# justinkay/aldi

Hardware: AMD Instinct MI355X
Metric: images/sec (student+teacher ALDI step), R50-FPN 1333x800 (higher is better)
Workload: dtype bf16

## Files before the change

### aldi_amd/csrc/bneck.hip

```cpp
#include "common.h"
#include "tile_prims.h"
#include <stdio.h>

namespace {

constexpr int MID = 64, CO = 256, TH = 8, TW = 16, HC = TW + 2, NHP = (TH + 2) * HC, CR = 192, A1P = 24;
constexpr int kRegA = 0;
constexpr int kRegB = 32768;
constexpr int kRegC = kRegB + (TH + 2) * A1P * 128;
constexpr int kLdsBytes = kRegC + 16384;
constexpr int kStgRow = CO * 2 + 16;
static_assert(TH * TW * kStgRow <= kLdsBytes && kLdsBytes <= 81920, "two workgroups per CU");

struct BneckDev {
    const bf16_t* x; const bf16_t* res; bf16_t* y;
    const bf16_t* w1; const bf16_t* w2; const bf16_t* w3;
    const float* b1; const float* b2; const float* b3;
    int N, H, W, th, tw, xcd;
    unsigned x_bytes, y_bytes;
};

__device__ __forceinline__ void lds_write_b64(unsigned addr, uint2 v) {
    asm volatile("ds_write_b64 %0, %1" ::"v"(addr), "v"(v) : "memory");
}
template <int N, int STEP, int I = 0>
__device__ __forceinline__ void stg_read_all(u32x4_t* f, unsigned addr) {
    if constexpr (I < N) {
        f[I] = frag_read<I * STEP>(addr);
        stg_read_all<N, STEP, I + 1>(f, addr);
    }
}
__device__ __forceinline__ uint2 relu_pack4(f32x4_t a, float4 sh, bool keep) {
    float v0 = fmaxf(a[0] + sh.x, 0.f), v1 = fmaxf(a[1] + sh.y, 0.f), v2 = fmaxf(a[2] + sh.z, 0.f), v3 = fmaxf(a[3] + sh.w, 0.f);
    uint2 t;
    t.x = keep ? pack2_bf16(v0, v1) : 0u;
    t.y = keep ? pack2_bf16(v2, v3) : 0u;
    return t;
}

template <int CX>
__global__ __launch_bounds__(256, 2) void bneck_kernel(BneckDev p) {
    static_assert(CX % 32 == 0, "x slabs of 32 channels");
    __shared__ __attribute__((aligned(128))) uint4 lds[kLdsBytes / 16];
    const int tid = threadIdx.x, lane = tid & 63, wave = __builtin_amdgcn_readfirstlane(tid >> 6);
    const int fr = lane & 15, fq = lane >> 4;
    int bid = blockIdx.x;
    if (p.xcd) {
        const int total = gridDim.x, q = total >> 3, r = total & 7, xcd = bid & 7, idx = bid >> 3;
        bid = (xcd < r ? xcd * (q + 1) : r * (q + 1) + (xcd - r) * q) + idx;
    }
    const int per_img = p.th * p.tw;
    const int n = bid / per_img, rem = bid - n * per_img;
    const int ty = rem / p.tw, tx = rem - ty * p.tw;
    const int h0 = ty * TH, w0 = tx * TW;
    constexpr unsigned OOB = 0x80000000u;
    const __amdgpu_buffer_rsrc_t rx = __builtin_amdgcn_make_buffer_rsrc(const_cast<bf16_t*>(p.x), 0, p.x_bytes, 0x00020000);
    const __amdgpu_buffer_rsrc_t rw1 = __builtin_amdgcn_make_buffer_rsrc(const_cast<bf16_t*>(p.w1), 0, MID * CX * 2, 0x00020000);
    const __amdgpu_buffer_rsrc_t rw2 = __builtin_amdgcn_make_buffer_rsrc(const_cast<bf16_t*>(p.w2), 0, MID * 9 * MID * 2, 0x00020000);
    const __amdgpu_buffer_rsrc_t rw3 = __builtin_amdgcn_make_buffer_rsrc(const_cast<bf16_t*>(p.w3), 0, CO * MID * 2, 0x00020000);
    const int wbase = __builtin_amdgcn_readfirstlane(tid & ~63);
    const unsigned lbase = lds_addr(&lds[0]);
    const long img_pix = (long)n * p.H * p.W;
    float4 sh1[4], sh2[4], sh3[4];
#pragma unroll
    for (int j = 0; j < 4; ++j) {
        sh1[j] = *reinterpret_cast<const float4*>(p.b1 + j * 16 + fq * 4);
        sh2[j] = *reinterpret_cast<const float4*>(p.b2 + j * 16 + fq * 4);
        sh3[j] = *reinterpret_cast<const float4*>(p.b3 + (wave * 4 + j) * 16 + fq * 4);
    }

    unsigned xoff[3];
#pragma unroll
    for (int it = 0; it < 3; ++it) {
        const int cr = (tid >> 2) + it * 64, kce = swz<4>(cr, tid & 3);
        const int hr = cr / HC, hc = cr - hr * HC;
        const int gh = h0 - 1 + hr, gw = w0 - 1 + hc;
        const bool ok = cr < NHP && (unsigned)gh < (unsigned)p.H && (unsigned)gw < (unsigned)p.W;
        xoff[it] = ok ? (unsigned)(((img_pix + (long)gh * p.W + gw) * CX + kce * 8) * 2) : OOB;
    }
    const unsigned w1off = (unsigned)(((tid >> 2) * CX + swz<4>(tid >> 2, tid & 3) * 8) * 2);
    constexpr int kStage1 = CR * 64 + MID * 64;
    auto issue1 = [&](int s) {
        const int st = s & 3;
#pragma unroll
        for (int it = 0; it < 3; ++it) glds16(rx, &lds[st * (kStage1 / 16) + wbase + it * 256], xoff[it] == OOB ? OOB : xoff[it] + (unsigned)(s * 64));
        glds16(rw1, &lds[st * (kStage1 / 16) + CR * 4 + wbase], w1off + (unsigned)(s * 64));
    };
    f32x4_t acc1[3][4];
#pragma unroll
    for (int i = 0; i < 3; ++i)
#pragma unroll
        for (int j = 0; j < 4; ++j) acc1[i][j] = f32x4_t{0.f, 0.f, 0.f, 0.f};
    {
        const int xrow = wave * 48 + fr;
        const unsigned x_rd = lbase + (unsigned)(xrow * 4 + swz<4>(xrow, fq)) * 16u;
        const unsigned w_rd = lbase + CR * 64 + (unsigned)(fr * 4 + swz<4>(fr, fq)) * 16u;
        constexpr int S = CX / 32;
#pragma unroll
        for (int s = 0; s < 3 && s < S; ++s) issue1(s);
#pragma unroll
        for (int s = 0; s < S; ++s) {
            constexpr int kPieces = 4;
            const int younger = (S - 1 - s < 2 ? S - 1 - s : 2) * kPieces;
            if (younger == 8) asm volatile("s_waitcnt vmcnt(8)" ::: "memory");
            else if (younger == 4) asm volatile("s_waitcnt vmcnt(4)" ::: "memory");
            else asm volatile("s_waitcnt vmcnt(0)" ::: "memory");
            __builtin_amdgcn_s_barrier();
            __builtin_amdgcn_sched_barrier(0);
            if (s + 3 < S) issue1(s + 3);
            u32x4_t xf[3], wf[4];
            frag_read_all<3, 64>(xf, x_rd + (unsigned)((s & 3) * kStage1));
            frag_read_all<4, 64>(wf, w_rd + (unsigned)((s & 3) * kStage1));
            frag_wait<3, 4>(xf, wf);
#pragma unroll
            for (int i = 0; i < 3; ++i)
#pragma unroll
                for (int j = 0; j < 4; ++j) acc1[i][j] = Mma<bf16_t>::run(wf[j], xf[i], acc1[i][j]);
        }
    }
    __builtin_amdgcn_s_barrier();
    __builtin_amdgcn_sched_barrier(0);
    unsigned w2off[2];
#pragma unroll
    for (int it = 0; it < 2; ++it) {
        const int c = tid + it * 256, row = c >> 3, q = c & 7;
        w2off[it] = (unsigned)(((row * 9) * MID + (q ^ ((row >> 1) & 7)) * 8) * 2);
    }
    auto issue_tap = [&](int t) {
#pragma unroll
        for (int it = 0; it < 2; ++it) glds16(rw2, &lds[kRegA / 16 + (t & 3) * 512 + wbase + it * 256], w2off[it] + (unsigned)(t * MID * 2));
    };
    issue_tap(0); issue_tap(1); issue_tap(2);
#pragma unroll
    for (int i = 0; i < 3; ++i) {
        const int cr = (wave * 3 + i) * 16 + fr;
        const int hr = cr / HC, hc = cr - hr * HC;
        const int gh = h0 - 1 + hr, gw = w0 - 1 + hc;
        const bool inside = (unsigned)gh < (unsigned)p.H && (unsigned)gw < (unsigned)p.W;
        const int ar = hr * A1P + hc;
        if (cr < NHP) {
#pragma unroll
            for (int j = 0; j < 4; ++j) {
                const int chunk = (j * 2 + (fq >> 1)) ^ ((ar >> 1) & 7);
                lds_write_b64(lbase + kRegB + (unsigned)(ar * 128 + chunk * 16 + (fq & 1) * 8), relu_pack4(acc1[i][j], sh1[j], inside));
            }
        }
    }
    f32x4_t acc2[2][4];
#pragma unroll
    for (int i = 0; i < 2; ++i)
#pragma unroll
        for (int j = 0; j < 4; ++j) acc2[i][j] = f32x4_t{0.f, 0.f, 0.f, 0.f};
    {
        unsigned a1b[2][3][2];
#pragma unroll
        for (int par = 0; par < 2; ++par)
#pragma unroll
            for (int kw = 0; kw < 3; ++kw)
#pragma unroll
                for (int ks = 0; ks < 2; ++ks) {
                    const int row = par * 8 + kw + fr;
                    a1b[par][kw][ks] = lbase + kRegB + (unsigned)(wave * 2 * A1P * 128) + (unsigned)(row * 128 + (((ks * 4 + fq) ^ ((row >> 1) & 7)) << 4));
                }
        unsigned wb[2];
#pragma unroll
        for (int ks = 0; ks < 2; ++ks) wb[ks] = lbase + kRegA + (unsigned)((fr * 8 + ((ks * 4 + fq) ^ ((fr >> 1) & 7))) * 16);
        asm volatile("s_waitcnt lgkmcnt(0)" ::: "memory");
#pragma unroll
        for (int t = 0; t < 9; ++t) {
            const int kh = t / 3, kw = t - kh * 3;
            if (t <= 6) asm volatile("s_waitcnt vmcnt(4)" ::: "memory");
            else if (t == 7) asm volatile("s_waitcnt vmcnt(2)" ::: "memory");
            else asm volatile("s_waitcnt vmcnt(0)" ::: "memory");
            __builtin_amdgcn_s_barrier();
            __builtin_amdgcn_sched_barrier(0);
            if (t + 3 < 9) issue_tap(t + 3);
            u32x4_t af[2][2], wf[2][4];
#pragma unroll
            for (int ks = 0; ks < 2; ++ks) {
                af[ks][0] = kh == 0 ? frag_read<0>(a1b[0][kw][ks]) : kh == 1 ? frag_read<16 * 128>(a1b[1][kw][ks]) : frag_read<48 * 128>(a1b[0][kw][ks]);
                af[ks][1] = kh == 0 ? frag_read<16 * 128>(a1b[1][kw][ks]) : kh == 1 ? frag_read<48 * 128>(a1b[0][kw][ks]) : frag_read<64 * 128>(a1b[1][kw][ks]);
                frag_read_all<4, 128>(wf[ks], wb[ks] + (unsigned)((t & 3) * 8192));
            }
            frag_wait<2, 4>(af[0], wf[0]);
            frag_wait<2, 4>(af[1], wf[1]);
#pragma unroll
            for (int ks = 0; ks < 2; ++ks)
#pragma unroll
                for (int i = 0; i < 2; ++i)
#pragma unroll
                    for (int j = 0; j < 4; ++j) acc2[i][j] = Mma<bf16_t>::run(wf[ks][j], af[ks][i], acc2[i][j]);
        }
    }
    __builtin_amdgcn_s_barrier();
    __builtin_amdgcn_sched_barrier(0);
#pragma unroll
    for (int it = 0; it < 8; ++it) {
        const int c = tid + it * 256, row = c >> 3, q = c & 7;
        glds16(rw3, &lds[kRegA / 16 + wbase + it * 256], (unsigned)((row * MID + (q ^ ((row >> 1) & 7)) * 8) * 2));
    }
#pragma unroll
    for (int i = 0; i < 2; ++i) {
        const int row = (wave * 2 + i) * 16 + fr;
#pragma unroll
        for (int j = 0; j < 4; ++j) {
            const int chunk = (j * 2 + (fq >> 1)) ^ ((row >> 1) & 7);
            lds_write_b64(lbase + kRegC + (unsigned)(row * 128 + chunk * 16 + (fq & 1) * 8), relu_pack4(acc2[i][j], sh2[j], true));
        }
    }
    asm volatile("s_waitcnt vmcnt(0) lgkmcnt(0)" ::: "memory");
    __builtin_amdgcn_s_barrier();
    __builtin_amdgcn_sched_barrier(0);
    f32x4_t acc3[8][4];
#pragma unroll
    for (int i = 0; i < 8; ++i)
#pragma unroll
        for (int j = 0; j < 4; ++j) acc3[i][j] = f32x4_t{0.f, 0.f, 0.f, 0.f};
#pragma unroll
    for (int ks = 0; ks < 2; ++ks) {
        const int sw = (ks * 4 + fq) ^ ((fr >> 1) & 7);
        const unsigned ab = lbase + kRegC + (unsigned)((fr * 8 + sw) * 16);
        const unsigned w3b = lbase + kRegA + (unsigned)(((wave * 64 + fr) * 8 + sw) * 16);
        u32x4_t af[8], wf[4];
        frag_read_all<8, 128>(af, ab);
        frag_read_all<4, 128>(wf, w3b);
        frag_wait<8, 4>(af, wf);
#pragma unroll
        for (int i = 0; i < 8; ++i)
#pragma unroll
            for (int j = 0; j < 4; ++j) acc3[i][j] = Mma<bf16_t>::run(wf[j], af[i], acc3[i][j]);
    }
    __builtin_amdgcn_s_barrier();
    __builtin_amdgcn_sched_barrier(0);
#pragma unroll
    for (int j = 0; j < 4; ++j) {
        const int co = (wave * 4 + j) * 16 + fq * 4;
        const float4 sh = sh3[j];
#pragma unroll
        for (int i = 0; i < 8; ++i) {
            uint2 t;
            t.x = pack2_bf16(acc3[i][j][0] + sh.x, acc3[i][j][1] + sh.y);
            t.y = pack2_bf16(acc3[i][j][2] + sh.z, acc3[i][j][3] + sh.w);
            lds_write_b64(lbase + (unsigned)((i * 16 + fr) * kStgRow + co * 2), t);
        }
    }
    asm volatile("s_waitcnt lgkmcnt(0)" ::: "memory");
    __builtin_amdgcn_s_barrier();
    __builtin_amdgcn_sched_barrier(0);
    {
        const __amdgpu_buffer_rsrc_t rr = make_rsrc_uniform(p.res, p.y_bytes);
        const __amdgpu_buffer_rsrc_t ry = make_rsrc_uniform(p.y, p.y_bytes);
        constexpr int NI = TH * TW * (CO / 8) / 256;
        unsigned goff[NI];
        u32x4_t rres[NI];
#pragma unroll
        for (int it = 0; it < NI; ++it) {
            const int c = tid + it * 256, row = c >> 5, ch = c & 31;
            const int gh = h0 + (row >> 4), gw = w0 + (row & 15);
            const bool ok = gh < p.H && gw < p.W;
            goff[it] = ok ? (unsigned)(((img_pix + (long)gh * p.W + gw) * CO + ch * 8) * 2) : OOB;
        }
#pragma unroll
        for (int it = 0; it < NI; ++it) rres[it] = __builtin_amdgcn_raw_buffer_load_b128(rr, goff[it], 0, 0);
        u32x4_t sv[NI];
        stg_read_all<NI, 8 * kStgRow>(sv, lbase + (unsigned)((tid >> 5) * kStgRow + (tid & 31) * 16));
        asm volatile("s_waitcnt lgkmcnt(0)" ::: "memory");
#pragma unroll
        for (int it = 0; it < NI; ++it) asm volatile("" : "+v"(sv[it]));
#pragma unroll
        for (int it = 0; it < NI; ++it) {
            u32x4_t ov;
#pragma unroll
            for (int q = 0; q < 4; ++q) {
                const float lo = fmaxf(__uint_as_float(sv[it][q] << 16) + __uint_as_float(rres[it][q] << 16), 0.f);
                const float hi = fmaxf(__uint_as_float(sv[it][q] & 0xffff0000u) + __uint_as_float(rres[it][q] & 0xffff0000u), 0.f);
                ov[q] = pack2_bf16(lo, hi);
            }
            __builtin_amdgcn_raw_buffer_store_b128(ov, ry, goff[it], 0, 0);
        }
    }
}

struct FoldItem { const float* w; const float* scale; bf16_t* out; int rows, cols, chunk_begin, reserved; };
__global__ __launch_bounds__(256) void fold_weights_kernel(const FoldItem* __restrict__ items, int n_items, int total_chunks) {
    const int c = blockIdx.x * blockDim.x + threadIdx.x;
    if (c >= total_chunks) return;
    int k = 0;
    for (int i = 1; i < n_items; ++i)
        if (c >= items[i].chunk_begin) k = i;
    const FoldItem it = items[k];
    const long e0 = (long)(c - it.chunk_begin) * 8;
    const int r = (int)(e0 / it.cols);
    const float s = it.scale ? it.scale[r] : 1.f;
    const float4 a = *reinterpret_cast<const float4*>(it.w + e0), b = *reinterpret_cast<const float4*>(it.w + e0 + 4);
    uint4 o;
    o.x = pack2_bf16(a.x * s, a.y * s); o.y = pack2_bf16(a.z * s, a.w * s);
    o.z = pack2_bf16(b.x * s, b.y * s); o.w = pack2_bf16(b.z * s, b.w * s);
    *reinterpret_cast<uint4*>(it.out + e0) = o;
}

}

extern "C" int aldi_fold_weights_batch(const aldi_fold_item* items, int n_items, int total_chunks, aldi_stream_t stream) {
    static_assert(sizeof(aldi_fold_item) == sizeof(FoldItem), "descriptor layout");
    if (!items || n_items < 1 || total_chunks < 1) return aldi_set_error_msg(ALDI_ERR_ARG, "fold_weights_batch: bad args");
    hipLaunchKernelGGL(fold_weights_kernel, dim3(cdiv(total_chunks, 256)), dim3(256), 0, static_cast<hipStream_t>(stream),
                       reinterpret_cast<const FoldItem*>(items), n_items, total_chunks);
    ALDI_CHECK_LAUNCH();
    return ALDI_OK;
}

extern "C" int aldi_bottleneck_fused(const aldi_bottleneck_args* a, aldi_stream_t stream) {
    if (!a || !a->x || !a->res || !a->y || !a->w1 || !a->w2 || !a->w3 || !a->b1 || !a->b2 || !a->b3)
        return aldi_set_error_msg(ALDI_ERR_ARG, "bottleneck_fused: null pointer");
    if (a->mid != MID || a->Cout != CO || (a->Cin != 64 && a->Cin != 256) || a->N < 1 || a->H < 1 || a->W < 1)
        return aldi_set_error_msg(ALDI_ERR_ARG, "bottleneck_fused: built for Cin in {64, 256}, 64 mid channels, 256 output channels (res2)");
    const size_t xb = (size_t)a->N * a->H * a->W * a->Cin * 2, yb = (size_t)a->N * a->H * a->W * CO * 2;
    if (xb >= 0x80000000ull || yb >= 0x80000000ull) return aldi_set_error_msg(ALDI_ERR_ARG, "bottleneck_fused: operand larger than 2 GiB (32-bit buffer offsets)");
    BneckDev d;
    d.x = static_cast<const bf16_t*>(a->x); d.res = static_cast<const bf16_t*>(a->res); d.y = static_cast<bf16_t*>(a->y);
    d.w1 = static_cast<const bf16_t*>(a->w1); d.w2 = static_cast<const bf16_t*>(a->w2); d.w3 = static_cast<const bf16_t*>(a->w3);
    d.b1 = a->b1; d.b2 = a->b2; d.b3 = a->b3;
    d.N = a->N; d.H = a->H; d.W = a->W; d.th = cdiv(a->H, TH); d.tw = cdiv(a->W, TW);
    d.xcd = aldi_tuning().igemm_xcd;
    d.x_bytes = (unsigned)xb; d.y_bytes = (unsigned)yb;
    const int tiles = a->N * d.th * d.tw;
    hipStream_t st = static_cast<hipStream_t>(stream);
    if (a->Cin == 64) hipLaunchKernelGGL(bneck_kernel<64>, dim3(tiles), dim3(256), 0, st, d);
    else hipLaunchKernelGGL(bneck_kernel<256>, dim3(tiles), dim3(256), 0, st, d);
    ALDI_CHECK_LAUNCH();
    char name[64];
    snprintf(name, sizeof(name), "bottleneck_fused<bf16,%d,64,256>", a->Cin);
    aldi_note_dispatch(name);
    return ALDI_OK;
}
```

### aldi_amd/csrc/elementwise.hip

```cpp
#include "common.h"
#include <stdlib.h>

namespace {

template <typename T>
__global__ void dgrad_weights_kernel(const float* __restrict__ w, const float* __restrict__ scale, T* __restrict__ wt,
                                     int Cout, int KH, int KW, int Cin) {
    long total = (long)Cout * KH * KW * Cin;
    for (long i = blockIdx.x * (long)blockDim.x + threadIdx.x; i < total; i += (long)gridDim.x * blockDim.x) {
        int co = (int)(i % Cout);
        long r = i / Cout;
        int kw = (int)(r % KW); r /= KW;
        int kh = (int)(r % KH);
        int ci = (int)(r / KH);
        float v = w[(((long)co * KH + (KH - 1 - kh)) * KW + (KW - 1 - kw)) * Cin + ci];
        if (scale) v *= scale[co];
        Elem<T>::st(wt + i, v);
    }
}

template <typename T>
__global__ __launch_bounds__(256) void dgrad_weights_batch_kernel(const aldi_dgw_item* __restrict__ items, int n_items) {
    __shared__ float tl[32][33];
    const int tile = blockIdx.x;
    int it = 0, hi = n_items - 1;
    while (it < hi) {
        const int mid = (it + hi + 1) >> 1;
        if (items[mid].tile_begin <= tile) it = mid;
        else hi = mid - 1;
    }
    const aldi_dgw_item d = items[it];
    const int Cout = d.Cout, KH = d.KH, KW = d.KW, Cin = d.Cin, T_ = KH * KW;
    const int nci = (Cin + 31) >> 5, nco = (Cout + 31) >> 5;
    int t = tile - d.tile_begin;
    const int cit = t % nci; t /= nci;
    const int cot = t % nco;
    const int tap = t / nco;
    const int kh = tap / KW, kw = tap - kh * KW;
    const int stap = (KH - 1 - kh) * KW + (KW - 1 - kw);
    const int tx = threadIdx.x & 31, ty = threadIdx.x >> 5;
#pragma unroll
    for (int k = 0; k < 4; ++k) {
        const int co = cot * 32 + ty + k * 8, ci = cit * 32 + tx;
        float v = 0.f;
        if (co < Cout && ci < Cin) {
            v = d.w_master[((long)co * T_ + stap) * Cin + ci];
            if (d.scale) v *= d.scale[co];
        }
        tl[ty + k * 8][tx] = v;
    }
    __syncthreads();
    T* __restrict__ wt = static_cast<T*>(d.wt);
#pragma unroll
    for (int k = 0; k < 4; ++k) {
        const int ci = cit * 32 + ty + k * 8, co = cot * 32 + tx;
        if (co < Cout && ci < Cin) Elem<T>::st(wt + ((long)ci * T_ + tap) * Cout + co, tl[tx][ty + k * 8]);
    }
}

struct StemDev {
    const uint8_t* img;
    const float* w;
    const float* scale; const float* shift;
    void* y;
    int N, Hs, Ws, Hc, Wc;
    int h[ALDI_MAX_IMAGES], wd[ALDI_MAX_IMAGES];
    float mean[3], inv_std[3];
};

template <typename T>
__global__ __launch_bounds__(256) void stem_kernel(StemDev p) {
    constexpr int TI = 16 * 2 + 5;
    __shared__ float ws[147 * 64];
    __shared__ float tile[3 * TI * TI];
    const int n = blockIdx.z;
    const int oy0 = blockIdx.y * 16, ox0 = blockIdx.x * 16;
    for (int i = threadIdx.x; i < 147 * 64; i += 256) {
        int co = i & 63, tap = i >> 6;
        ws[i] = p.w[co * 147 + tap];
    }
    const int iy0 = oy0 * 2 - 3, ix0 = ox0 * 2 - 3;
    const int h = p.h[n], w = p.wd[n];
    for (int i = threadIdx.x; i < 3 * TI * TI; i += 256) {
        int c = i / (TI * TI), r = i - c * TI * TI;
        int yy = r / TI, xx = r - yy * TI;
        int iy = iy0 + yy, ix = ix0 + xx;
        float v = 0.f;
        if (iy >= 0 && iy < h && ix >= 0 && ix < w)
            v = ((float)p.img[(((long)n * 3 + c) * p.Hs + iy) * p.Ws + ix] - p.mean[c]) * p.inv_std[c];
        tile[i] = v;
    }
    __syncthreads();
    const int ty = threadIdx.x >> 4, tx = threadIdx.x & 15;
    const int oy = oy0 + ty, ox = ox0 + tx;
    float acc[64];
#pragma unroll
    for (int i = 0; i < 64; ++i) acc[i] = 0.f;
    for (int kh = 0; kh < 7; ++kh)
        for (int kw = 0; kw < 7; ++kw)
#pragma unroll
            for (int c = 0; c < 3; ++c) {
                float xv = tile[(c * TI + ty * 2 + kh) * TI + tx * 2 + kw];
                const float4* wr = reinterpret_cast<const float4*>(&ws[((kh * 7 + kw) * 3 + c) * 64]);
#pragma unroll
                for (int q = 0; q < 16; ++q) {
                    float4 wv = wr[q];
                    acc[q * 4 + 0] = fmaf(xv, wv.x, acc[q * 4 + 0]);
                    acc[q * 4 + 1] = fmaf(xv, wv.y, acc[q * 4 + 1]);
                    acc[q * 4 + 2] = fmaf(xv, wv.z, acc[q * 4 + 2]);
                    acc[q * 4 + 3] = fmaf(xv, wv.w, acc[q * 4 + 3]);
                }
            }
    if (oy < p.Hc && ox < p.Wc) {
        T* out = static_cast<T*>(p.y) + (((long)n * p.Hc + oy) * p.Wc + ox) * 64;
#pragma unroll
        for (int q = 0; q < 16; ++q) {
            float v[4];
#pragma unroll
            for (int r = 0; r < 4; ++r) {
                float t = acc[q * 4 + r] * p.scale[q * 4 + r] + p.shift[q * 4 + r];
                v[r] = t > 0.f ? t : 0.f;
            }
            store4(out + q * 4, v);
        }
    }
}

__global__ __launch_bounds__(256) void stem_mfma_kernel(StemDev p) {
    constexpr int TH = 37, TW = 40, WK = 200;
    __shared__ __attribute__((aligned(16))) bf16_t wl[64 * WK];
    __shared__ __attribute__((aligned(16))) bf16_t tile[3 * TH * TW];
    const int n = blockIdx.z;
    const int oy0 = blockIdx.y * 16, ox0 = blockIdx.x * 16;
    for (int i = threadIdx.x; i < 64 * 192; i += 256) {
        const int co = i / 192, k = i - co * 192;
        const int idx = k >> 3, kw = k & 7;
        float v = 0.f;
        if (idx < 21 && kw < 7) {
            const int c = idx / 7, kh = idx - c * 7;
            v = p.w[co * 147 + (kh * 7 + kw) * 3 + c];
        }
        wl[co * WK + k] = f32_to_bf16(v);
    }
    const int iy0 = oy0 * 2 - 3, ix0 = ox0 * 2 - 3;
    const int h = p.h[n], w = p.wd[n];
    for (int i = threadIdx.x; i < 3 * TH * TW; i += 256) {
        const int c = i / (TH * TW), r = i - c * TH * TW;
        const int yy = r / TW, xx = r - yy * TW;
        const int iy = iy0 + yy, ix = ix0 + xx;
        float v = 0.f;
        if (xx < TH && iy >= 0 && iy < h && ix >= 0 && ix < w)
            v = ((float)p.img[(((long)n * 3 + c) * p.Hs + iy) * p.Ws + ix] - p.mean[c]) * p.inv_std[c];
        tile[i] = f32_to_bf16(v);
    }
    __syncthreads();
    const int lane = threadIdx.x & 63, wave = threadIdx.x >> 6;
    const int fr = lane & 15, fq = lane >> 4;
    f32x4_t acc[4][4];
#pragma unroll
    for (int i = 0; i < 4; ++i)
#pragma unroll
        for (int j = 0; j < 4; ++j) acc[i][j] = f32x4_t{0.f, 0.f, 0.f, 0.f};
    const uint32_t* tile32 = reinterpret_cast<const uint32_t*>(tile);
    const uint4* wl16 = reinterpret_cast<const uint4*>(wl);
#pragma unroll
    for (int s = 0; s < 6; ++s) {
        int idx = s * 4 + fq;
        idx = idx < 21 ? idx : 20;
        const int c = idx / 7, kh = idx - c * 7;
        uint4 xf[4], wf[4];
#pragma unroll
        for (int i = 0; i < 4; ++i) {
            const int ty = wave * 4 + i;
            const int e = ((c * TH + ty * 2 + kh) * TW + fr * 2) >> 1;
            xf[i] = make_uint4(tile32[e], tile32[e + 1], tile32[e + 2], tile32[e + 3]);
        }
#pragma unroll
        for (int j = 0; j < 4; ++j) wf[j] = wl16[((j * 16 + fr) * WK + (s * 4 + fq) * 8) >> 3];
#pragma unroll
        for (int i = 0; i < 4; ++i)
#pragma unroll
            for (int j = 0; j < 4; ++j)
                acc[i][j] = __builtin_amdgcn_mfma_f32_16x16x32_bf16(*reinterpret_cast<bf16x8_t*>(&wf[j]), *reinterpret_cast<bf16x8_t*>(&xf[i]),
                                                                     acc[i][j], 0, 0, 0);
    }
    bf16_t* Y = static_cast<bf16_t*>(p.y);
#pragma unroll
    for (int j = 0; j < 4; ++j) {
        const int ch = j * 16 + fq * 4;
        const float4 sc = *reinterpret_cast<const float4*>(p.scale + ch), sh = *reinterpret_cast<const float4*>(p.shift + ch);
#pragma unroll
        for (int i = 0; i < 4; ++i) {
            const int oy = oy0 + wave * 4 + i, ox = ox0 + fr;
            if (oy < p.Hc && ox < p.Wc) {
                uint2 o;
                o.x = pack2_bf16(fmaxf(acc[i][j][0] * sc.x + sh.x, 0.f), fmaxf(acc[i][j][1] * sc.y + sh.y, 0.f));
                o.y = pack2_bf16(fmaxf(acc[i][j][2] * sc.z + sh.z, 0.f), fmaxf(acc[i][j][3] * sc.w + sh.w, 0.f));
                *reinterpret_cast<uint2*>(Y + (((long)n * p.Hc + oy) * p.Wc + ox) * 64 + ch) = o;
            }
        }
    }
}

constexpr int kStemWK = 200;
__global__ void stem_pack_kernel(const float* __restrict__ w, bf16_t* __restrict__ wpk) {
    const int i = blockIdx.x * blockDim.x + threadIdx.x;
    if (i >= 64 * kStemWK) return;
    const int co = i / kStemWK, k = i - co * kStemWK;
    const int idx = k >> 3, kw = k & 7;
    float v = 0.f;
    if (k < 192 && idx < 21 && kw < 7) {
        const int c = idx / 7, kh = idx - c * 7;
        v = w[co * 147 + (kh * 7 + kw) * 3 + c];
    }
    wpk[i] = f32_to_bf16(v);
}

struct StemPoolDev {
    StemDev s;
    const bf16_t* wpk;
    bf16_t* yp;
    int Hp, Wp;
};

__global__ __launch_bounds__(256) void stem_pool_mfma_kernel(StemPoolDev q) {
    const StemDev& p = q.s;
    constexpr int TH = 37, TW = 40, WK = kStemWK, PT = 7, CS = 144;
    constexpr int kWlBytes = 64 * WK * 2, kTileBytes = 3 * TH * TW * 2, kCtBytes = 256 * CS;
    __shared__ __attribute__((aligned(16))) unsigned char smem[(kWlBytes + kTileBytes) > kCtBytes ? (kWlBytes + kTileBytes) : kCtBytes];
    bf16_t* wl = reinterpret_cast<bf16_t*>(smem);
    bf16_t* tile = reinterpret_cast<bf16_t*>(smem + kWlBytes);
    const int n = blockIdx.z;
    const int py0 = blockIdx.y * PT, px0 = blockIdx.x * PT;
    const int cy0 = 2 * py0 - 1, cx0 = 2 * px0 - 1;
    {
        const uint4* src = reinterpret_cast<const uint4*>(q.wpk);
        uint4* dst = reinterpret_cast<uint4*>(wl);
        for (int i = threadIdx.x; i < 64 * WK / 8; i += 256) dst[i] = src[i];
    }
    const int iy0 = cy0 * 2 - 3, ix0 = cx0 * 2 - 3;
    const int h = p.h[n], w = p.wd[n];
    {
        const int r = threadIdx.x >> 1, half = threadIdx.x & 1;
        if (r < 3 * TH) {
            const int c = r / TH, yy = r - c * TH;
            const int iy = iy0 + yy;
            const bool rok = iy >= 0 && iy < h;
            const uint8_t* row = p.img + (((long)n * 3 + c) * p.Hs + (rok ? iy : 0)) * p.Ws;
            const float mean = p.mean[c], inv = p.inv_std[c];
#pragma unroll
            for (int k = 0; k < 20; ++k) {
                const int xx = half * 20 + k, ix = ix0 + xx;
                float v = 0.f;
                if (rok && xx < TH && ix >= 0 && ix < w) v = ((float)row[ix] - mean) * inv;
                tile[(c * TH + yy) * TW + xx] = f32_to_bf16(v);
            }
        }
    }
    __syncthreads();
    const int lane = threadIdx.x & 63, wave = threadIdx.x >> 6;
    const int fr = lane & 15, fq = lane >> 4;
    f32x4_t acc[4][4];
#pragma unroll
    for (int i = 0; i < 4; ++i)
#pragma unroll
        for (int j = 0; j < 4; ++j) acc[i][j] = f32x4_t{0.f, 0.f, 0.f, 0.f};
    {
        const uint32_t* tile32 = reinterpret_cast<const uint32_t*>(tile);
        const uint4* wl16 = reinterpret_cast<const uint4*>(wl);
#pragma unroll
        for (int s = 0; s < 6; ++s) {
            int idx = s * 4 + fq;
            idx = idx < 21 ? idx : 20;
            const int c = idx / 7, kh = idx - c * 7;
            uint4 xf[4], wf[4];
#pragma unroll
            for (int i = 0; i < 4; ++i) {
                const int ty = wave * 4 + i;
                const int e = ((c * TH + ty * 2 + kh) * TW + fr * 2) >> 1;
                xf[i] = make_uint4(tile32[e], tile32[e + 1], tile32[e + 2], tile32[e + 3]);
            }
#pragma unroll
            for (int j = 0; j < 4; ++j) wf[j] = wl16[((j * 16 + fr) * WK + (s * 4 + fq) * 8) >> 3];
#pragma unroll
            for (int i = 0; i < 4; ++i)
#pragma unroll
                for (int j = 0; j < 4; ++j)
                    acc[i][j] = __builtin_amdgcn_mfma_f32_16x16x32_bf16(*reinterpret_cast<bf16x8_t*>(&wf[j]), *reinterpret_cast<bf16x8_t*>(&xf[i]),
                                                                         acc[i][j], 0, 0, 0);
        }
    }
    __syncthreads();
#pragma unroll
    for (int j = 0; j < 4; ++j) {
        const int ch = j * 16 + fq * 4;
        const float4 sc = *reinterpret_cast<const float4*>(p.scale + ch), sh = *reinterpret_cast<const float4*>(p.shift + ch);
#pragma unroll
        for (int i = 0; i < 4; ++i) {
            const int ry = wave * 4 + i, cy = cy0 + ry, cx = cx0 + fr;
            uint2 o;
            if (cy >= 0 && cy < p.Hc && cx >= 0 && cx < p.Wc) {
                o.x = pack2_bf16(fmaxf(acc[i][j][0] * sc.x + sh.x, 0.f), fmaxf(acc[i][j][1] * sc.y + sh.y, 0.f));
                o.y = pack2_bf16(fmaxf(acc[i][j][2] * sc.z + sh.z, 0.f), fmaxf(acc[i][j][3] * sc.w + sh.w, 0.f));
            } else {
                o.x = o.y = 0xff80ff80u;
            }
            *reinterpret_cast<uint2*>(smem + (ry * 16 + fr) * CS + ch * 2) = o;
        }
    }
    __syncthreads();
    typedef short s16x8_t __attribute__((ext_vector_type(8)));
    for (int item = threadIdx.x; item < PT * PT * 8; item += 256) {
        const int chunk = item & 7, pp = item >> 3;
        const int pi = pp / PT, pj = pp - pi * PT;
        const int py = py0 + pi, px = px0 + pj;
        if (py >= q.Hp || px >= q.Wp) continue;
        s16x8_t m = *reinterpret_cast<const s16x8_t*>(smem + ((2 * pi) * 16 + 2 * pj) * CS + chunk * 16);
#pragma unroll
        for (int d = 1; d < 9; ++d) {
            const s16x8_t v = *reinterpret_cast<const s16x8_t*>(smem + ((2 * pi + d / 3) * 16 + 2 * pj + d % 3) * CS + chunk * 16);
            m = __builtin_elementwise_max(m, v);
        }
        *reinterpret_cast<s16x8_t*>(q.yp + (((long)n * q.Hp + py) * q.Wp + px) * 64 + chunk * 8) = m;
    }
}

template <typename T>
__global__ void maxpool3s2_kernel(const T* __restrict__ x, T* __restrict__ y, int N, int H, int W, int C, int Ho, int Wo) {
    long total = (long)N * Ho * Wo * (C / 4);
    for (long i = blockIdx.x * (long)blockDim.x + threadIdx.x; i < total; i += (long)gridDim.x * blockDim.x) {
        int c4 = (int)(i % (C / 4));
        long r = i / (C / 4);
        int wo = (int)(r % Wo); r /= Wo;
        int ho = (int)(r % Ho);
        int n = (int)(r / Ho);
        float m[4] = {-INFINITY, -INFINITY, -INFINITY, -INFINITY};
        for (int dy = 0; dy < 3; ++dy) {
            int hi = ho * 2 - 1 + dy;
            if (hi < 0 || hi >= H) continue;
            for (int dx = 0; dx < 3; ++dx) {
                int wi = wo * 2 - 1 + dx;
                if (wi < 0 || wi >= W) continue;
                float v[4];
                load4(x + (((long)n * H + hi) * W + wi) * C + c4 * 4, v);
#pragma unroll
                for (int k = 0; k < 4; ++k) m[k] = fmaxf(m[k], v[k]);
            }
        }
        store4(y + i * 4, m);
    }
}

template <typename T>
__global__ void subsample2_kernel(const T* __restrict__ x, T* __restrict__ y, int N, int H, int W, int C, int Ho, int Wo) {
    long total = (long)N * Ho * Wo * (C / 4);
    for (long i = blockIdx.x * (long)blockDim.x + threadIdx.x; i < total; i += (long)gridDim.x * blockDim.x) {
        int c4 = (int)(i % (C / 4));
        long r = i / (C / 4);
        int wo = (int)(r % Wo); r /= Wo;
        int ho = (int)(r % Ho);
        int n = (int)(r / Ho);
        float v[4];
        load4(x + (((long)n * H + ho * 2) * W + wo * 2) * C + c4 * 4, v);
        store4(y + i * 4, v);
    }
}

template <typename T>
__global__ void subsample2_bwd_kernel(const T* __restrict__ gy, T* __restrict__ gx, int N, int H, int W, int C, int Ho, int Wo) {
    long total = (long)N * Ho * Wo * (C / 4);
    for (long i = blockIdx.x * (long)blockDim.x + threadIdx.x; i < total; i += (long)gridDim.x * blockDim.x) {
        int c4 = (int)(i % (C / 4));
        long r = i / (C / 4);
        int wo = (int)(r % Wo); r /= Wo;
        int ho = (int)(r % Ho);
        int n = (int)(r / Ho);
        float a[4], b[4];
        load4(gy + i * 4, a);
        T* dst = gx + (((long)n * H + ho * 2) * W + wo * 2) * C + c4 * 4;
        load4(dst, b);
#pragma unroll
        for (int k = 0; k < 4; ++k) b[k] += a[k];
        store4(dst, b);
    }
}

template <typename T>
__global__ void upsample2_bwd_kernel(const T* __restrict__ g, T* __restrict__ out, int N, int Hc, int Wc, int C, int accumulate) {
    long total = (long)N * Hc * Wc * (C / 4);
    const int H = Hc * 2, W = Wc * 2;
    for (long i = blockIdx.x * (long)blockDim.x + threadIdx.x; i < total; i += (long)gridDim.x * blockDim.x) {
        int c4 = (int)(i % (C / 4));
        long r = i / (C / 4);
        int w = (int)(r % Wc); r /= Wc;
        int h = (int)(r % Hc);
        int n = (int)(r / Hc);
        float s[4] = {0, 0, 0, 0};
#pragma unroll
        for (int dy = 0; dy < 2; ++dy)
#pragma unroll
            for (int dx = 0; dx < 2; ++dx) {
                float v[4];
                load4(g + (((long)n * H + h * 2 + dy) * W + w * 2 + dx) * C + c4 * 4, v);
#pragma unroll
                for (int k = 0; k < 4; ++k) s[k] += v[k];
            }
        if (accumulate) {
            float o[4];
            load4(out + i * 4, o);
#pragma unroll
            for (int k = 0; k < 4; ++k) s[k] += o[k];
        }
        store4(out + i * 4, s);
    }
}

template <typename T> __device__ __forceinline__ void through_storage(float v[4]);
template <> __device__ __forceinline__ void through_storage<float>(float v[4]) {}
template <> __device__ __forceinline__ void through_storage<bf16_t>(float v[4]) {
    bf16_t t[4];
    store4(t, v);
    load4(t, v);
}
template <typename T>
__global__ void upsample2_bwd_chain_kernel(const T* __restrict__ g2, T* __restrict__ o3, T* __restrict__ o4, T* __restrict__ o5, int N, int H5, int W5, int C) {
    const long total = (long)N * H5 * W5 * (C / 4);
    const int H4 = H5 * 2, W4 = W5 * 2, H3 = H5 * 4, W3 = W5 * 4, H2 = H5 * 8, W2 = W5 * 8;
    for (long i = blockIdx.x * (long)blockDim.x + threadIdx.x; i < total; i += (long)gridDim.x * blockDim.x) {
        const int c4 = (int)(i % (C / 4));
        long r = i / (C / 4);
        const int w5 = (int)(r % W5); r /= W5;
        const int h5 = (int)(r % H5);
        const int n = (int)(r / H5);
        float s5[4] = {0, 0, 0, 0};
        for (int a = 0; a < 4; ++a) {
            const int h4 = h5 * 2 + (a >> 1), w4 = w5 * 2 + (a & 1);
            float s4[4] = {0, 0, 0, 0};
            for (int b = 0; b < 4; ++b) {
                const int h3 = h4 * 2 + (b >> 1), w3 = w4 * 2 + (b & 1);
                float s3[4] = {0, 0, 0, 0};
#pragma unroll
                for (int dy = 0; dy < 2; ++dy)
#pragma unroll
                    for (int dx = 0; dx < 2; ++dx) {
                        float v[4];
                        load4(g2 + (((long)n * H2 + h3 * 2 + dy) * W2 + w3 * 2 + dx) * C + c4 * 4, v);
#pragma unroll
                        for (int k = 0; k < 4; ++k) s3[k] += v[k];
                    }
                T* p3 = o3 + (((long)n * H3 + h3) * W3 + w3) * C + c4 * 4;
                float o[4];
                load4(p3, o);
#pragma unroll
                for (int k = 0; k < 4; ++k) s3[k] += o[k];
                store4(p3, s3);
                through_storage<T>(s3);
#pragma unroll
                for (int k = 0; k < 4; ++k) s4[k] += s3[k];
            }
            T* p4 = o4 + (((long)n * H4 + h4) * W4 + w4) * C + c4 * 4;
            float o[4];
            load4(p4, o);
#pragma unroll
            for (int k = 0; k < 4; ++k) s4[k] += o[k];
            store4(p4, s4);
            through_storage<T>(s4);
#pragma unroll
            for (int k = 0; k < 4; ++k) s5[k] += s4[k];
        }
        T* p5 = o5 + i * 4;
        float o[4];
        load4(p5, o);
#pragma unroll
        for (int k = 0; k < 4; ++k) s5[k] += o[k];
        store4(p5, s5);
    }
}

template <typename T>
__global__ void add_f32_kernel(const T* __restrict__ a, const float* __restrict__ b, const T* __restrict__ relu_src, T* __restrict__ out, long n4) {
    for (long i = blockIdx.x * (long)blockDim.x + threadIdx.x; i < n4; i += (long)gridDim.x * blockDim.x) {
        float v[4] = {0, 0, 0, 0};
        if (a) load4(a + i * 4, v);
        if (b) {
            float4 t = *reinterpret_cast<const float4*>(b + i * 4);
            v[0] += t.x; v[1] += t.y; v[2] += t.z; v[3] += t.w;
        }
        if (relu_src) {
            float m[4];
            load4(relu_src + i * 4, m);
#pragma unroll
            for (int k = 0; k < 4; ++k) v[k] = m[k] > 0.f ? v[k] : 0.f;
        }
        store4(out + i * 4, v);
    }
}

template <typename T>
__global__ void cast_from_f32_kernel(const float* __restrict__ src, T* __restrict__ dst, long n) {
    for (long i = blockIdx.x * (long)blockDim.x + threadIdx.x; i < n; i += (long)gridDim.x * blockDim.x) Elem<T>::st(dst + i, src[i]);
}

template <typename T>
__global__ void sgd_kernel(float* __restrict__ p, const float* __restrict__ g, float* __restrict__ buf, T* __restrict__ pc,
                           long n, float lr, float mu, float wd, float gscale, int first) {
    for (long i = blockIdx.x * (long)blockDim.x + threadIdx.x; i < n; i += (long)gridDim.x * blockDim.x) {
        float w = p[i];
        float d = g[i] * gscale + wd * w;
        float b = first ? d : mu * buf[i] + d;
        buf[i] = b;
        w = w - lr * b;
        p[i] = w;
        if (pc) Elem<T>::st(pc + i, w);
    }
}

template <typename T>
__global__ void sgd_dev_kernel(float* __restrict__ p, const float* __restrict__ g, float* __restrict__ buf, T* __restrict__ pc,
                               long n, const float* __restrict__ hyper) {
    const float lr = hyper[0], mu = hyper[1], wd = hyper[2], gscale = hyper[3];
    for (long i = blockIdx.x * (long)blockDim.x + threadIdx.x; i < n; i += (long)gridDim.x * blockDim.x) {
        float w = p[i];
        const float d = g[i] * gscale + wd * w;
        const float b = mu * buf[i] + d;
        buf[i] = b;
        w = w - lr * b;
        p[i] = w;
        if (pc) Elem<T>::st(pc + i, w);
    }
}

template <typename T>
__global__ void ema_kernel(float* __restrict__ t, const float* __restrict__ s, T* __restrict__ tc, long n, long nc, float one_minus_alpha, float alpha,
                           int copy_only) {
    const long n4 = ((reinterpret_cast<uintptr_t>(t) | reinterpret_cast<uintptr_t>(s)) & 15) == 0 ? n >> 2 : 0;
    for (long q = blockIdx.x * (long)blockDim.x + threadIdx.x; q < n4; q += (long)gridDim.x * blockDim.x) {
        const float4 sv = reinterpret_cast<const float4*>(s)[q];
        float4 v = sv;
        if (!copy_only) {
            const float4 tv = reinterpret_cast<const float4*>(t)[q];
            v.x = sv.x * one_minus_alpha + tv.x * alpha; v.y = sv.y * one_minus_alpha + tv.y * alpha;
            v.z = sv.z * one_minus_alpha + tv.z * alpha; v.w = sv.w * one_minus_alpha + tv.w * alpha;
        }
        reinterpret_cast<float4*>(t)[q] = v;
        if (tc) {
            const long i = q << 2;
            if (i < nc) Elem<T>::st(tc + i, v.x);
            if (i + 1 < nc) Elem<T>::st(tc + i + 1, v.y);
            if (i + 2 < nc) Elem<T>::st(tc + i + 2, v.z);
            if (i + 3 < nc) Elem<T>::st(tc + i + 3, v.w);
        }
    }
    for (long i = (n4 << 2) + blockIdx.x * (long)blockDim.x + threadIdx.x; i < n; i += (long)gridDim.x * blockDim.x) {
        float v = copy_only ? s[i] : s[i] * one_minus_alpha + t[i] * alpha;
        t[i] = v;
        if (tc && i < nc) Elem<T>::st(tc + i, v);
    }
}

__global__ void bn_fold_kernel(const float* __restrict__ w, const float* __restrict__ b, const float* __restrict__ mean,
                               const float* __restrict__ var, float* __restrict__ scale, float* __restrict__ shift, int C, float eps) {
    int i = blockIdx.x * blockDim.x + threadIdx.x;
    if (i < C) {
        float sc = w[i] * (1.0f / sqrtf(var[i] + eps));
        scale[i] = sc;
        shift[i] = b[i] - mean[i] * sc;
    }
}

static inline int nblocks(long n, int per = 256, int cap = 16384) {
    long b = (n + per - 1) / per;
    return (int)(b < 1 ? 1 : (b > cap ? cap : b));
}

}

#define DISPATCH_T(dtype, KERNEL, grid, block, st, ...)                                              \
    do {                                                                                             \
        if ((dtype) == ALDI_BF16) hipLaunchKernelGGL(KERNEL<bf16_t>, grid, block, 0, st, __VA_ARGS__); \
        else if ((dtype) == ALDI_F32) hipLaunchKernelGGL(KERNEL<float>, grid, block, 0, st, __VA_ARGS__); \
        else return aldi_set_error_msg(ALDI_ERR_ARG, #KERNEL ": bad dtype");                         \
        ALDI_CHECK_LAUNCH();                                                                         \
    } while (0)

extern "C" int aldi_stem_forward(const aldi_stem_args* a, aldi_stream_t stream) {
    if (!a || !a->img || !a->w || !a->y || a->N < 1 || a->N > ALDI_MAX_IMAGES) return aldi_set_error_msg(ALDI_ERR_ARG, "stem_forward: bad args");
    StemDev d;
    d.img = a->img; d.w = a->w; d.scale = a->scale; d.shift = a->shift; d.y = a->y;
    d.N = a->N; d.Hs = a->Hs; d.Ws = a->Ws; d.Hc = a->Hc; d.Wc = a->Wc;
    for (int i = 0; i < a->N; ++i) { d.h[i] = a->h[i]; d.wd[i] = a->w_img[i]; }
    for (int c = 0; c < 3; ++c) { d.mean[c] = a->mean[c]; d.inv_std[c] = 1.0f / a->std[c]; }
    dim3 grid(cdiv(a->Wc, 16), cdiv(a->Hc, 16), a->N);
    hipStream_t st = static_cast<hipStream_t>(stream);
    const int mfma_env = aldi_tuning().stem_mfma;
    if (a->dtype == ALDI_BF16 && mfma_env && a->scale && a->shift) {
        hipLaunchKernelGGL(stem_mfma_kernel, grid, dim3(256), 0, st, d);
        ALDI_CHECK_LAUNCH();
        return ALDI_OK;
    }
    DISPATCH_T(a->dtype, stem_kernel, grid, dim3(256), st, d);
    return ALDI_OK;
}

extern "C" int aldi_stem_pack_weights(const float* w, void* w_packed, aldi_stream_t stream) {
    if (!w || !w_packed) return aldi_set_error_msg(ALDI_ERR_ARG, "stem_pack_weights: null pointer");
    hipLaunchKernelGGL(stem_pack_kernel, dim3(cdiv(64 * kStemWK, 256)), dim3(256), 0, static_cast<hipStream_t>(stream), w, (bf16_t*)w_packed);
    ALDI_CHECK_LAUNCH();
    return ALDI_OK;
}

extern "C" int aldi_stem_pool_forward(const aldi_stem_args* a, const void* w_packed, void* y_pool, aldi_stream_t stream) {
    if (!a || !a->img || !w_packed || !y_pool || !a->scale || !a->shift || a->N < 1 || a->N > ALDI_MAX_IMAGES || a->dtype != ALDI_BF16)
        return aldi_set_error_msg(ALDI_ERR_ARG, "stem_pool_forward: bad args (bf16 only)");
    StemPoolDev q;
    StemDev& d = q.s;
    d.img = a->img; d.w = a->w; d.scale = a->scale; d.shift = a->shift; d.y = nullptr;
    d.N = a->N; d.Hs = a->Hs; d.Ws = a->Ws; d.Hc = a->Hc; d.Wc = a->Wc;
    for (int i = 0; i < a->N; ++i) { d.h[i] = a->h[i]; d.wd[i] = a->w_img[i]; }
    for (int c = 0; c < 3; ++c) { d.mean[c] = a->mean[c]; d.inv_std[c] = 1.0f / a->std[c]; }
    q.wpk = static_cast<const bf16_t*>(w_packed);
    q.yp = static_cast<bf16_t*>(y_pool);
    q.Hp = (a->Hc - 1) / 2 + 1; q.Wp = (a->Wc - 1) / 2 + 1;
    dim3 grid(cdiv(q.Wp, 7), cdiv(q.Hp, 7), a->N);
    hipLaunchKernelGGL(stem_pool_mfma_kernel, grid, dim3(256), 0, static_cast<hipStream_t>(stream), q);
    ALDI_CHECK_LAUNCH();
    return ALDI_OK;
}

extern "C" int aldi_maxpool3s2(const void* x, void* y, int N, int H, int W, int C, int dtype, aldi_stream_t stream) {
    int Ho = (H + 2 - 3) / 2 + 1, Wo = (W + 2 - 3) / 2 + 1;
    long total = (long)N * Ho * Wo * (C / 4);
    hipStream_t st = static_cast<hipStream_t>(stream);
    if (dtype == ALDI_BF16) hipLaunchKernelGGL(maxpool3s2_kernel<bf16_t>, dim3(nblocks(total)), dim3(256), 0, st, (const bf16_t*)x, (bf16_t*)y, N, H, W, C, Ho, Wo);
    else hipLaunchKernelGGL(maxpool3s2_kernel<float>, dim3(nblocks(total)), dim3(256), 0, st, (const float*)x, (float*)y, N, H, W, C, Ho, Wo);
    ALDI_CHECK_LAUNCH();
    return ALDI_OK;
}

constexpr int kMaxStage = 16;
struct StageDev { const unsigned char* src[kMaxStage]; int h[kMaxStage], w[kMaxStage]; int n, C, Hs, Ws; };
__global__ __launch_bounds__(256) void stage_images_kernel(StageDev p, unsigned char* __restrict__ dst) {
    const int i = blockIdx.z, c = blockIdx.y;
    const int h = p.h[i], w = p.w[i];
    const unsigned char* s = p.src[i] + (long)c * h * w;
    unsigned char* d = dst + ((long)i * p.C + c) * p.Hs * p.Ws;
    for (int row = blockIdx.x; row < h; row += gridDim.x) {
        const unsigned char* sr = s + (long)row * w;
        unsigned char* dr = d + (long)row * p.Ws;
        if ((((uintptr_t)sr | (uintptr_t)dr) & 3) == 0) {
            const int w4 = w >> 2;
            for (int x = threadIdx.x; x < w4; x += blockDim.x) reinterpret_cast<unsigned*>(dr)[x] = reinterpret_cast<const unsigned*>(sr)[x];
            for (int x = (w4 << 2) + threadIdx.x; x < w; x += blockDim.x) dr[x] = sr[x];
        } else {
            for (int x = threadIdx.x; x < w; x += blockDim.x) dr[x] = sr[x];
        }
    }
}

extern "C" int aldi_stage_images(const void* const* images, const int* heights, const int* widths, int n, int C, int Hs, int Ws, void* batch,
                                 aldi_stream_t stream) {
    if (!images || !heights || !widths || !batch || n < 1 || n > kMaxStage || C < 1) return aldi_set_error_msg(ALDI_ERR_ARG, "stage_images: bad args (1..16 images)");
    StageDev p;
    p.n = n; p.C = C; p.Hs = Hs; p.Ws = Ws;
    int hmax = 1;
    for (int i = 0; i < kMaxStage; ++i) {
        p.src[i] = i < n ? static_cast<const unsigned char*>(images[i]) : nullptr;
        p.h[i] = i < n ? heights[i] : 0; p.w[i] = i < n ? widths[i] : 0;
        if (i < n && (!images[i] || heights[i] < 0 || widths[i] < 0 || heights[i] > Hs || widths[i] > Ws)) return aldi_set_error_msg(ALDI_ERR_ARG, "stage_images: image larger than the batch");
        if (p.h[i] > hmax) hmax = p.h[i];
    }
    hipLaunchKernelGGL(stage_images_kernel, dim3(hmax < 256 ? hmax : 256, C, n), dim3(256), 0, static_cast<hipStream_t>(stream), p, static_cast<unsigned char*>(batch));
    ALDI_CHECK_LAUNCH();
    return ALDI_OK;
}

extern "C" int aldi_subsample2(const void* x, void* y, int N, int H, int W, int C, int backward, int dtype, aldi_stream_t stream) {
    int Ho = (H - 1) / 2 + 1, Wo = (W - 1) / 2 + 1;
    long total = (long)N * Ho * Wo * (C / 4);
    hipStream_t st = static_cast<hipStream_t>(stream);
    if (!backward) {
        if (dtype == ALDI_BF16) hipLaunchKernelGGL(subsample2_kernel<bf16_t>, dim3(nblocks(total)), dim3(256), 0, st, (const bf16_t*)x, (bf16_t*)y, N, H, W, C, Ho, Wo);
        else hipLaunchKernelGGL(subsample2_kernel<float>, dim3(nblocks(total)), dim3(256), 0, st, (const float*)x, (float*)y, N, H, W, C, Ho, Wo);
    } else {
        if (dtype == ALDI_BF16) hipLaunchKernelGGL(subsample2_bwd_kernel<bf16_t>, dim3(nblocks(total)), dim3(256), 0, st, (const bf16_t*)x, (bf16_t*)y, N, H, W, C, Ho, Wo);
        else hipLaunchKernelGGL(subsample2_bwd_kernel<float>, dim3(nblocks(total)), dim3(256), 0, st, (const float*)x, (float*)y, N, H, W, C, Ho, Wo);
    }
    ALDI_CHECK_LAUNCH();
    return ALDI_OK;
}

extern "C" int aldi_upsample2_bwd(const void* g, void* out, int N, int Hc, int Wc, int C, int accumulate, int dtype, aldi_stream_t stream) {
    long total = (long)N * Hc * Wc * (C / 4);
    hipStream_t st = static_cast<hipStream_t>(stream);
    if (dtype == ALDI_BF16) hipLaunchKernelGGL(upsample2_bwd_kernel<bf16_t>, dim3(nblocks(total)), dim3(256), 0, st, (const bf16_t*)g, (bf16_t*)out, N, Hc, Wc, C, accumulate);
    else hipLaunchKernelGGL(upsample2_bwd_kernel<float>, dim3(nblocks(total)), dim3(256), 0, st, (const float*)g, (float*)out, N, Hc, Wc, C, accumulate);
    ALDI_CHECK_LAUNCH();
    return ALDI_OK;
}

extern "C" int aldi_upsample2_bwd_chain(const void* g2, void* o3, void* o4, void* o5, int N, int H5, int W5, int C, int dtype, aldi_stream_t stream) {
    if (!g2 || !o3 || !o4 || !o5 || N < 1 || H5 < 1 || W5 < 1 || (C & 3)) return aldi_set_error_msg(ALDI_ERR_ARG, "upsample2_bwd_chain: bad args");
    const long total = (long)N * H5 * W5 * (C / 4);
    hipStream_t st = static_cast<hipStream_t>(stream);
    if (dtype == ALDI_BF16) hipLaunchKernelGGL(upsample2_bwd_chain_kernel<bf16_t>, dim3(cdiv(total, 256)), dim3(256), 0, st, (const bf16_t*)g2, (bf16_t*)o3, (bf16_t*)o4, (bf16_t*)o5, N, H5, W5, C);
    else hipLaunchKernelGGL(upsample2_bwd_chain_kernel<float>, dim3(cdiv(total, 256)), dim3(256), 0, st, (const float*)g2, (float*)o3, (float*)o4, (float*)o5, N, H5, W5, C);
    ALDI_CHECK_LAUNCH();
    return ALDI_OK;
}

extern "C" int aldi_add_f32(const void* a, const float* b, const void* relu_src, void* out, long n, int dtype, aldi_stream_t stream) {
    if (n % 4) return aldi_set_error_msg(ALDI_ERR_ARG, "add_f32: n must be a multiple of 4");
    hipStream_t st = static_cast<hipStream_t>(stream);
    if (dtype == ALDI_BF16) hipLaunchKernelGGL(add_f32_kernel<bf16_t>, dim3(nblocks(n / 4)), dim3(256), 0, st, (const bf16_t*)a, b, (const bf16_t*)relu_src, (bf16_t*)out, n / 4);
    else hipLaunchKernelGGL(add_f32_kernel<float>, dim3(nblocks(n / 4)), dim3(256), 0, st, (const float*)a, b, (const float*)relu_src, (float*)out, n / 4);
    ALDI_CHECK_LAUNCH();
    return ALDI_OK;
}

extern "C" int aldi_cast_from_f32(const float* src, void* dst, long n, int dtype, aldi_stream_t stream) {
    hipStream_t st = static_cast<hipStream_t>(stream);
    if (dtype == ALDI_BF16) hipLaunchKernelGGL(cast_from_f32_kernel<bf16_t>, dim3(nblocks(n)), dim3(256), 0, st, src, (bf16_t*)dst, n);
    else hipLaunchKernelGGL(cast_from_f32_kernel<float>, dim3(nblocks(n)), dim3(256), 0, st, src, (float*)dst, n);
    ALDI_CHECK_LAUNCH();
    return ALDI_OK;
}

extern "C" int aldi_sgd_step(float* p, const float* g, float* buf, void* p_compute, long n, float lr, float momentum, float weight_decay,
                             float grad_scale, int first_step, int dtype, aldi_stream_t stream) {
    if (!p || !g || !buf) return aldi_set_error_msg(ALDI_ERR_ARG, "sgd_step: null pointer");
    hipStream_t st = static_cast<hipStream_t>(stream);
    if (dtype == ALDI_BF16) hipLaunchKernelGGL(sgd_kernel<bf16_t>, dim3(nblocks(n)), dim3(256), 0, st, p, g, buf, (bf16_t*)p_compute, n, lr, momentum, weight_decay, grad_scale, first_step);
    else hipLaunchKernelGGL(sgd_kernel<float>, dim3(nblocks(n)), dim3(256), 0, st, p, g, buf, (float*)nullptr, n, lr, momentum, weight_decay, grad_scale, first_step);
    ALDI_CHECK_LAUNCH();
    return ALDI_OK;
}

extern "C" int aldi_sgd_step_dev(float* p, const float* g, float* buf, void* p_compute, long n, const float* hyper, int dtype, aldi_stream_t stream) {
    if (!p || !g || !buf || !hyper || n <= 0) return aldi_set_error_msg(ALDI_ERR_ARG, "sgd_step_dev: bad args");
    hipStream_t st = static_cast<hipStream_t>(stream);
    if (dtype == ALDI_BF16) hipLaunchKernelGGL(sgd_dev_kernel<bf16_t>, dim3(nblocks(n)), dim3(256), 0, st, p, g, buf, (bf16_t*)p_compute, n, hyper);
    else hipLaunchKernelGGL(sgd_dev_kernel<float>, dim3(nblocks(n)), dim3(256), 0, st, p, g, buf, (float*)nullptr, n, hyper);
    ALDI_CHECK_LAUNCH();
    return ALDI_OK;
}

extern "C" int aldi_ema_update(float* teacher, const float* student, void* teacher_compute, long n, long n_compute, double alpha, int copy_only, int dtype,
                               aldi_stream_t stream) {
    if (!teacher || !student) return aldi_set_error_msg(ALDI_ERR_ARG, "ema_update: null pointer");
    hipStream_t st = static_cast<hipStream_t>(stream);
    const float oma = (float)(1.0 - alpha);
    const float alpha_f = (float)alpha;
    const long nc = teacher_compute ? (n_compute < n ? n_compute : n) : 0;
    const int cap = aldi_tuning().ema_blocks > 0 ? aldi_tuning().ema_blocks : 16384;
    if (dtype == ALDI_BF16) hipLaunchKernelGGL(ema_kernel<bf16_t>, dim3(nblocks(n / 4 + 1, 256, cap)), dim3(256), 0, st, teacher, student, (bf16_t*)teacher_compute, n, nc, oma, alpha_f, copy_only);
    else hipLaunchKernelGGL(ema_kernel<float>, dim3(nblocks(n / 4 + 1, 256, cap)), dim3(256), 0, st, teacher, student, (float*)nullptr, n, 0L, oma, alpha_f, copy_only);
    ALDI_CHECK_LAUNCH();
    return ALDI_OK;
}

extern "C" int aldi_bn_fold(const float* w, const float* b, const float* mean, const float* var, float* scale, float* shift, int C, aldi_stream_t stream) {
    hipLaunchKernelGGL(bn_fold_kernel, dim3(cdiv(C, 256)), dim3(256), 0, static_cast<hipStream_t>(stream), w, b, mean, var, scale, shift, C, 1e-5f);
    ALDI_CHECK_LAUNCH();
    return ALDI_OK;
}

extern "C" int aldi_dgrad_weights_batch(const aldi_dgw_item* items, int n_items, int total_tiles, int dtype, aldi_stream_t stream) {
    if (!items || n_items <= 0 || total_tiles <= 0) return aldi_set_error_msg(ALDI_ERR_ARG, "dgrad_weights_batch: bad args");
    hipStream_t st = static_cast<hipStream_t>(stream);
    if (dtype == ALDI_BF16) hipLaunchKernelGGL(dgrad_weights_batch_kernel<bf16_t>, dim3(total_tiles), dim3(256), 0, st, items, n_items);
    else if (dtype == ALDI_F32) hipLaunchKernelGGL(dgrad_weights_batch_kernel<float>, dim3(total_tiles), dim3(256), 0, st, items, n_items);
    else return aldi_set_error_msg(ALDI_ERR_ARG, "dgrad_weights_batch: bad dtype");
    ALDI_CHECK_LAUNCH();
    return ALDI_OK;
}

extern "C" int aldi_dgrad_weights(const float* w_master, const float* scale, void* wt, int Cout, int KH, int KW, int Cin,
                                  int dtype, aldi_stream_t stream) {
    if (!w_master || !wt) return aldi_set_error_msg(ALDI_ERR_ARG, "dgrad_weights: null pointer");
    long total = (long)Cout * KH * KW * Cin;
    int blocks = (int)((total + 255) / 256);
    if (blocks > 8192) blocks = 8192;
    hipStream_t st = static_cast<hipStream_t>(stream);
    if (dtype == ALDI_BF16) hipLaunchKernelGGL(dgrad_weights_kernel<bf16_t>, dim3(blocks), dim3(256), 0, st, w_master, scale, (bf16_t*)wt, Cout, KH, KW, Cin);
    else hipLaunchKernelGGL(dgrad_weights_kernel<float>, dim3(blocks), dim3(256), 0, st, w_master, scale, (float*)wt, Cout, KH, KW, Cin);
    ALDI_CHECK_LAUNCH();
    return ALDI_OK;
}
```

### aldi_amd/csrc/host.h

```cpp
#pragma once
#include "../../include/aldi_hip.h"

int aldi_set_error_msg(int code, const char* msg);

typedef uint16_t bf16_t;

#define ALDI_KNOBS(X) \
    X(igemm_xcd, 1) X(igemm_tile, 0) X(igemm_dbg, 0) X(igemm_bigtile_min, 1024) X(igemm_bigtile, 64) X(igemm_bigtile_k, 768) X(igemm_lintile_min, 768) \
    X(igemm_halo, 1) X(igemm_force, 0) X(igemm_k64_min, 1024) X(igemm_group, 1) X(igemm_narrow_k, 512) X(igemm_splitk_tile, 2) X(igemm_halo_f32, 0) \
    X(igemm_f32_tile64_max, 4096) X(igemm_direct, 15) X(igemm_lean, 1) X(igemm_halo64_mid, 0) X(igemm_ws, 1) X(igemm_ws_wgs, 512) X(igemm_ws_min, 40000) \
    X(wgrad_lean, 1) X(wgrad_big_min, 28) X(wgrad_big_slots, 256) X(wgrad_slots, 384) X(wgrad_xcd, 1) \
    X(igemm_halo_ilv, 1) X(igemm_halo_small, 0) X(igemm_halo96, 0) \
    X(wgrad_dma, 0) X(wgrad_dbg, 0) X(wgrad_group_slots, 0) X(wgrad_group_epi, 24) X(wgrad_db, 0) X(wgrad_ordered, 1) X(wgrad_big_group, 1) X(wgrad_big_epi, 12) \
    X(wgrad_big_group_min, 64) X(wgrad_lds_pad_kb, 0) X(wgrad_f32_tile128, 1) X(wgrad_dma64, 3) X(wgrad_ilv, 0) \
    X(msda_gather, 7) X(msda_gather_list, 1500) X(msda_bin, 1) X(msda_bin_list, 512) X(roialign_sep, 1) X(roialign_bwd_rows, 2) \
    X(colsum_blocks, 256) X(colsum_minrows, 16) X(colsum_nt, 1024) X(colsum_block_kb, 384) \
    X(stem_mfma, 1) X(sab_blocks, 512) X(ln_bwd_blocks, 512) X(ln_bwd_blocks_narrow, 1024) X(rpn_topk_fused, 1) X(ema_blocks, 2048) X(nms_mask_tri, 1) X(match_wave, 1)

struct AldiTuning {
#define ALDI_KNOB_FIELD(name, dflt) int name;
    ALDI_KNOBS(ALDI_KNOB_FIELD)
#undef ALDI_KNOB_FIELD
};
AldiTuning& aldi_tuning();
void aldi_note_dispatch(const char* kernel);

static inline int cdiv(long a, long b) { return (int)((a + b - 1) / b); }
```

### aldi_amd/engine.py

```python
from __future__ import annotations

import contextlib
import dataclasses
import inspect
import math
import os
from collections import OrderedDict
from typing import Dict, List, Optional, Sequence, Tuple

import torch

from . import ops
from .arch import FC_DIM, FPN_C, NUM_ANCHORS, POOL, STAGE_BLOCKS, Packed, ParamLayout, pad_to

PIXEL_MEAN = (103.530, 116.280, 123.675)
PIXEL_STD = (1.0, 1.0, 1.0)
ANCHOR_SIZES = (32, 64, 128, 256, 512)
ANCHOR_RATIOS = (0.5, 1.0, 2.0)
STRIDES = (4, 8, 16, 32, 64)
GMAX = 128
RPN_BATCH, RPN_POS_FRAC = 256, 0.5
ROI_BATCH, ROI_POS_FRAC = 512, 0.25
RPN_PRE = (2000, 1000)
RPN_POST = (1000, 1000)
# ... 42 lines not shown
        self.bn_shift = torch.zeros(max(L.bn_channels, 1), dtype=torch.float32, device=device)
        self._grad = None
        self._mom = None
        self.first_step = True
        self._wt: Dict[str, torch.Tensor] = {}
        self._wt_keys: List[str] = []
        self._wt_plan = None
        self.wt_epoch = 0
        self._neg1: Dict[int, torch.Tensor] = {}
        self._stem_pk, self._stem_name = None, None
        self.lazy_wt = False
        self._wt_dirty = False
        self._fold_names: List[str] = []
        self._fold_plan = None

    @property
    def grad(self) -> torch.Tensor:
        if self._grad is None:
            self._grad = torch.zeros(self.layout.n_train, dtype=torch.float32, device=self.device)
        return self._grad

    @property
    def mom(self) -> torch.Tensor:
        if self._mom is None:
            self._mom = torch.zeros(self.layout.n_train, dtype=torch.float32, device=self.device)
        return self._mom

    def w(self, name: str) -> torch.Tensor:
        p = self.layout.t[name]
        n = p.rows * p.kk * p.kk * p.cin
        return self.compute[p.w_off: p.w_off + n].view(p.wshape)

    def w_master(self, name: str) -> torch.Tensor:
        p = self.layout.t[name]
        n = p.rows * p.kk * p.kk * p.cin
        return self.master[p.w_off: p.w_off + n].view(p.wshape)

    def b(self, name: str) -> Optional[torch.Tensor]:
        p = self.layout.t[name]
        return self.master[p.b_off: p.b_off + p.rows] if p.bias else None

    def scale(self, name: str) -> Optional[torch.Tensor]:
        p = self.layout.t[name]
        return self.bn_scale[p.bn_off: p.bn_off + p.rows] if p.bn else None

    def shift(self, name: str) -> Optional[torch.Tensor]:
        p = self.layout.t[name]
        return self.bn_shift[p.bn_off: p.bn_off + p.rows] if p.bn else self.b(name)

    def gw(self, name: str) -> torch.Tensor:
        p = self.layout.t[name]
        n = p.rows * p.kk * p.kk * p.cin
        return self.grad[p.w_off: p.w_off + n]

    def gb(self, name: str) -> torch.Tensor:
        p = self.layout.t[name]
        return self.grad[p.b_off: p.b_off + p.rows]

    def wt(self, name: str, negate: bool = False) -> torch.Tensor:
        key = name + ("-" if negate else "")
        if self._wt_dirty:
            self._refresh_wt()
        if key not in self._wt:
            self._wt[key] = ops.dgrad_weights(*self._wt_source(key), self.dtype)
            if key not in self._wt_keys:
                self._wt_keys.append(key)
                if self._wt_plan is not None:
                    self.wt_epoch += 1
                self._wt_plan = None
        return self._wt[key]

    def wt_flat(self, name: str) -> torch.Tensor:
        return self.wt(name + "@flat")

    def folded(self, names: Sequence[str]) -> List[torch.Tensor]:
        if self._fold_plan is None:
            self._fold_names = list(names) if not self._fold_names else self._fold_names
            self._fold_plan = ops.FoldWeightsPlan([(self.w_master(n), self.scale(n)) for n in self._fold_names])
            self._fold_plan.run()
        idx = [self._fold_names.index(n) for n in names]
        return [self._fold_plan.out[i] for i in idx]

    def stem_packed(self, name: str) -> torch.Tensor:
        if self._stem_pk is None:
            self._stem_pk = ops.stem_pack_weights(self.w_master(name))
            self._stem_name = name
        return self._stem_pk

    def _wt_source(self, key: str):
        neg = key.endswith("-")
        key = key[:-1] if neg else key
        flat = key.endswith("@flat")
        name = key[:-len("@flat")] if flat else key
        w = self.w_master(name)
        if flat:
            w = w.view(w.shape[0], 1, 1, -1)
        return w, self._wt_scale(name, neg)

    def _wt_scale(self, name: str, negate: bool):
        if not negate:
            return self.scale(name)
        rows = self.layout.t[name].rows
        if rows not in self._neg1:
            self._neg1[rows] = torch.full((rows,), -1.0, dtype=torch.float32, device=self.device)
        return self._neg1[rows]

    def _refresh_wt(self):
        self._wt_dirty = False
        self._wt.clear()
        if not self._wt_keys:
            return
        if self._wt_plan is None:
            self._wt_plan = ops.DgradWeightsPlan([self._wt_source(key) for key in self._wt_keys], self.dtype)
        self._wt_plan.run()
        for key, o in zip(self._wt_keys, self._wt_plan.out):
            self._wt[key] = o

    def load_state_dict(self, sd: Dict[str, torch.Tensor]):
        missing = [k for k in self.layout.state_dict_keys() if k not in sd]
        if missing:
            raise KeyError(f"missing keys in state_dict: {missing[:5]}{'...' if len(missing) > 5 else ''}")
        self.master.copy_(self.layout.pack(sd).to(self.device))
        self.refresh()

    def state_dict(self) -> "OrderedDict[str, torch.Tensor]":
        return self.layout.unpack(self.master)

    def refresh(self, cast: bool = True):
        L = self.layout
        if L.bn_channels:
            b = L.bn_base
            c = L.bn_channels
            ops.bn_fold(self.master[b:b + c], self.master[b + c:b + 2 * c], self.master[b + 2 * c:b + 3 * c],
                        self.master[b + 3 * c:b + 4 * c], self.bn_scale, self.bn_shift, c)
        if self.dtype != torch.float32 and cast:
            ops.cast_from_f32(self.master[:L.n_weights], self.dtype, out=self.compute)
        if self._stem_pk is not None:
            ops.stem_pack_weights(self.w_master(self._stem_name), out=self._stem_pk)
        if self._fold_plan is not None:
            self._fold_plan.run()
        self._refresh_wt()

    def zero_grad(self):
        self.grad.zero_()
        self._gscale = 1.0

    def scale_grad(self, f: float):
        self._gscale = getattr(self, "_gscale", 1.0) * f

    def sgd_step(self, lr: float, momentum: float = 0.9, weight_decay: float = 1e-4, grad_scale: float = 1.0):
        n = self.layout.n_train
        ops.sgd_step(self.master, self.grad, self.mom, self.compute if self.dtype != torch.float32 else None, n, lr, momentum,
                     weight_decay, grad_scale * getattr(self, "_gscale", 1.0), self.first_step, self.dtype)
        self._after_sgd()

    def _after_sgd(self):
        self.first_step = False
        if self.lazy_wt:
            self._wt_dirty = True
        else:
            self._refresh_wt()

    def sgd_range_dev(self, lo: int, hi: int, hyper: torch.Tensor):
        hi = min(hi, self.layout.n_train)
        if hi > lo:
            ops.sgd_step_dev(self.master, self.grad, self.mom, self.compute if self.dtype != torch.float32 else None, lo, hi, hyper, self.dtype)

    def ema_from(self, student: "Weights", alpha: float, copy_only: bool):
        n = self.layout.n_total
        if self.dtype == torch.bfloat16:
            ops.ema_update(self.master, student.master, self.compute, n, alpha, copy_only, self.dtype, n_compute=self.layout.n_weights)
            self.refresh(cast=False)
        else:
            ops.ema_update(self.master, student.master, None, n, alpha, copy_only, torch.float32)
            self.refresh()


def make_anchors(shapes: Sequence[Tuple[int, int]], device, sizes: Sequence[float] = ANCHOR_SIZES) -> torch.Tensor:
    out = []
    for (h, w), size, stride in zip(shapes, sizes, STRIDES):
        cell = []
        for r in ANCHOR_RATIOS:
            area = size ** 2.0
            aw = math.sqrt(area / r)
            ah = r * aw
            cell.append([-aw / 2.0, -ah / 2.0, aw / 2.0, ah / 2.0])
        cell = torch.tensor(cell, dtype=torch.float32)
        sx = torch.arange(0, w * stride, step=stride, dtype=torch.float32)
        sy = torch.arange(0, h * stride, step=stride, dtype=torch.float32)
        yy, xx = torch.meshgrid(sy, sx, indexing="ij")
        shifts = torch.stack((xx.reshape(-1), yy.reshape(-1), xx.reshape(-1), yy.reshape(-1)), dim=1)
        out.append((shifts.view(-1, 1, 4) + cell.view(1, -1, 4)).reshape(-1, 4))
    return torch.cat(out).contiguous().to(device)


@dataclasses.dataclass(frozen=True)
class D2Params:
    pixel_mean: Tuple[float, ...] = PIXEL_MEAN
    pixel_std: Tuple[float, ...] = PIXEL_STD
    anchor_sizes: Tuple[float, ...] = ANCHOR_SIZES
    rpn_batch: int = RPN_BATCH
    rpn_pos_frac: float = RPN_POS_FRAC
    rpn_iou: Tuple[float, float] = (0.3, 0.7)
    rpn_pre: Tuple[int, int] = RPN_PRE
    rpn_post: Tuple[int, int] = RPN_POST
    rpn_nms: float = RPN_NMS
    roi_batch: int = ROI_BATCH
    roi_pos_frac: float = ROI_POS_FRAC
    roi_iou: float = 0.5
    roi_weights: Tuple[float, float, float, float] = ROI_WEIGHTS
    score_thresh: float = SCORE_THRESH
    nms_test: float = NMS_TEST
    dets: int = DETS

    @classmethod
    def from_cfg(cls, cfg) -> "D2Params":
        M = cfg.MODEL

        def get(node, key, default):
            return node.get(key, default) if hasattr(node, "get") else getattr(node, key, default)

        def need(cond, what):
            if not cond:
                raise ValueError(f"aldi_amd R50-FPN engine: unsupported config value: {what}")
        rpn, roi, box, ag = M.RPN, M.ROI_HEADS, get(M, "ROI_BOX_HEAD", {}), M.ANCHOR_GENERATOR
        sizes = [list(s_) for s_ in ag.SIZES]
        need(len(sizes) == 5 and all(len(s_) == 1 for s_ in sizes), f"ANCHOR_GENERATOR.SIZES {sizes} (one size per level p2..p6)")
        ratios = [list(r_) for r_ in ag.ASPECT_RATIOS]
        need(all(tuple(float(v) for v in r_) == ANCHOR_RATIOS for r_ in ratios), f"ANCHOR_GENERATOR.ASPECT_RATIOS {ratios} (kernels: {ANCHOR_RATIOS})")
        need(len(M.PIXEL_MEAN) == 3 and len(M.PIXEL_STD) == 3, "PIXEL_MEAN / PIXEL_STD must have 3 entries")
        need(list(get(rpn, "IN_FEATURES", ["p2", "p3", "p4", "p5", "p6"])) == ["p2", "p3", "p4", "p5", "p6"], "RPN.IN_FEATURES")
        need(list(get(roi, "IN_FEATURES", ["p2", "p3", "p4", "p5"])) == ["p2", "p3", "p4", "p5"], "ROI_HEADS.IN_FEATURES")
        need(tuple(get(rpn, "BBOX_REG_WEIGHTS", (1.0, 1.0, 1.0, 1.0))) == (1.0, 1.0, 1.0, 1.0), "RPN.BBOX_REG_WEIGHTS != (1, 1, 1, 1)")
        need(float(get(rpn, "SMOOTH_L1_BETA", 0.0)) == 0.0 and float(get(box, "SMOOTH_L1_BETA", 0.0)) == 0.0, "SMOOTH_L1_BETA != 0 (the losses are pure L1)")
        need(get(rpn, "BBOX_REG_LOSS_TYPE", "smooth_l1") == "smooth_l1" and get(box, "BBOX_REG_LOSS_TYPE", "smooth_l1") == "smooth_l1", "BBOX_REG_LOSS_TYPE")
        need(float(get(rpn, "LOSS_WEIGHT", 1.0)) == 1.0 and float(get(rpn, "BBOX_REG_LOSS_WEIGHT", 1.0)) == 1.0, "RPN loss weights != 1")
        need(int(get(box, "POOLER_RESOLUTION", POOL)) == POOL and int(get(box, "POOLER_SAMPLING_RATIO", 0)) == 0 and
             get(box, "POOLER_TYPE", "ROIAlignV2") == "ROIAlignV2", "ROI_BOX_HEAD pooler (kernels: ROIAlignV2, 7x7, adaptive sampling)")
        need(not get(box, "CLS_AGNOSTIC_BBOX_REG", False), "CLS_AGNOSTIC_BBOX_REG")
        need(get(roi, "PROPOSAL_APPEND_GT", True), "ROI_HEADS.PROPOSAL_APPEND_GT False")
        need(len(rpn.IOU_THRESHOLDS) == 2 and len(roi.IOU_THRESHOLDS) == 1, "IOU_THRESHOLDS (RPN: two, ROI heads: one)")
        pre = (int(rpn.PRE_NMS_TOPK_TRAIN), int(rpn.PRE_NMS_TOPK_TEST))
        post = (int(rpn.POST_NMS_TOPK_TRAIN), int(rpn.POST_NMS_TOPK_TEST))
        need(max(pre) <= 2048 and min(pre + post) >= 1, f"RPN.PRE_NMS_TOPK {pre} (the NMS workspace holds 2048 boxes per level and image)")
        dets = int(get(get(cfg, "TEST", {}), "DETECTIONS_PER_IMAGE", DETS))
        need(1 <= dets <= GMAX, f"TEST.DETECTIONS_PER_IMAGE {dets} (<= {GMAX}: pseudo-label rows)")
        need(int(rpn.BATCH_SIZE_PER_IMAGE) >= 1 and int(roi.BATCH_SIZE_PER_IMAGE) >= 1, "BATCH_SIZE_PER_IMAGE")
        return cls(pixel_mean=tuple(float(v) for v in M.PIXEL_MEAN), pixel_std=tuple(float(v) for v in M.PIXEL_STD),
                   anchor_sizes=tuple(float(s_[0]) for s_ in sizes), rpn_batch=int(rpn.BATCH_SIZE_PER_IMAGE), rpn_pos_frac=float(rpn.POSITIVE_FRACTION),
                   rpn_iou=(float(rpn.IOU_THRESHOLDS[0]), float(rpn.IOU_THRESHOLDS[1])), rpn_pre=pre, rpn_post=post, rpn_nms=float(rpn.NMS_THRESH),
                   roi_batch=int(roi.BATCH_SIZE_PER_IMAGE), roi_pos_frac=float(roi.POSITIVE_FRACTION), roi_iou=float(roi.IOU_THRESHOLDS[0]),
                   roi_weights=tuple(float(v) for v in get(box, "BBOX_REG_WEIGHTS", ROI_WEIGHTS)), score_thresh=float(roi.SCORE_THRESH_TEST),
                   nms_test=float(roi.NMS_THRESH_TEST), dets=dets)


def raise_on_error(code: int, who: str = "engine"):
    if code & 1:
        raise FloatingPointError(f"{who}: predicted boxes or scores contain Inf/NaN. Training has diverged.")
    if code & 2:
        raise RuntimeError(f"{who}: sparse RPN-head backward: more active pixels than (2 * BATCH_SIZE_PER_IMAGE + 4 * positives) per image; "
                           "the excess was dropped, gradients of this step are wrong -- or, from the detection post-processing: a row of class "
                           "scores contains Inf/NaN; the row was dropped")
    if code & 4:
        raise RuntimeError(f"{who}: detection post-processing: more than 8192 candidates above SCORE_THRESH_TEST in one image; the excess was dropped")
    if code & 8:
        raise RuntimeError(f"{who}: RPN top-k: the group barrier of `topk_fused_kernel` timed out (its workgroups were not co-resident); the candidates "
                           "of this step are wrong.  Set ALDI_RPN_TOPK_FUSED=0 for the five-launch path")
    if code:
        raise RuntimeError(f"{who}: device error word {code}")


class Ctx(dict):
    __getattr__ = dict.__getitem__
    __setattr__ = dict.__setitem__


class RCNN:
    p = D2Params()

    def __init__(self, weights: Weights, num_classes: int, params: Optional[D2Params] = None):
        self.wts = weights
        if params is not None:
            self.p = params
        self.K = num_classes
        self.device, self.dtype = weights.device, weights.dtype
        self.Cp = weights.layout.t["box_pred"].rows
        self.Ch = weights.layout.t["rpn_head_out"].rows
        self._anchor_cache: Dict[tuple, tuple] = {}
        self._ws: Dict[str, torch.Tensor] = {}
        self.err = torch.zeros(1, dtype=torch.int32, device=self.device)
        torch.set_num_threads(1)
        idx = lambda n: int(n.rsplit(".", 1)[1])
        names = list(getattr(weights.layout, "t", {}))
        self.img_da_layers = sorted((n for n in names if n.startswith("img_align.model.")), key=idx)
        self.ins_da_layers = sorted((n for n in names if n.startswith("ins_align.model.")), key=idx)
        self.has_img_da, self.has_ins_da = bool(self.img_da_layers), bool(self.ins_da_layers)
        self.fused_stem = os.environ.get("ALDI_FUSED_STEM", "1") == "1"
        self.wgrad_tail_split = int(os.environ.get("ALDI_WGRAD_TAIL_SPLIT", "2"))
        self.group_wgrad = os.environ.get("ALDI_WGRAD_GROUP", "1") == "1"
        self.mask_bits = os.environ.get("ALDI_MASK_BITS", "1") == "1"
        self.mask_bits_inner = os.environ.get("ALDI_MASK_BITS_INNER", "1") == "1"
        self.level_groups = os.environ.get("ALDI_LEVEL_GROUPS", "1") == "1"
        self.fused_res2 = os.environ.get("ALDI_FUSED_RES2", "1") == "1"
        self._wg_queue: list = []
        self.sparse_rpn_backward = os.environ.get("ALDI_RPN_SPARSE_BWD", "1") == "1"
        spec = getattr(weights.layout, "img_da", None)
        self.img_da_level = ("p2", "p3", "p4", "p5", "p6").index(spec["layer"]) if spec else 0

    def stage_images(self, images: Sequence[torch.Tensor]):
        sizes = [(int(im.shape[1]), int(im.shape[2])) for im in images]
        Hs = pad_to(max(s[0] for s in sizes), 32)
        Ws = pad_to(max(s[1] for s in sizes), 32)
        N = len(images)
        if all(im.is_cuda for im in images):
            st = torch.zeros((N, 3, Hs, Ws), dtype=torch.uint8, device=self.device)
            for i, im in enumerate(images):
                st[i, :, : sizes[i][0], : sizes[i][1]] = im
        else:
            host = torch.zeros((N, 3, Hs, Ws), dtype=torch.uint8).pin_memory()
            for i, im in enumerate(images):
                host[i, :, : sizes[i][0], : sizes[i][1]] = im
            st = host.to(self.device, non_blocking=True)
        hw = torch.tensor(sizes, dtype=torch.int32).to(self.device)
        return st, sizes, hw

    def stage_gt(self, instances: Sequence[dict]):
        N = len(instances)
        gb = torch.zeros((N, GMAX, 4), dtype=torch.float32)
        gc = torch.zeros((N, GMAX), dtype=torch.int32)
        cnt = torch.zeros((N,), dtype=torch.int32)
        on_dev = []
        for i, inst in enumerate(instances):
            b = inst["gt_boxes"]
            b = b.tensor if hasattr(b, "tensor") else b
            g = int(b.shape[0])
            if g > GMAX:
                raise ValueError(f"more than {GMAX} GT boxes in one image")
            if g:
                if b.is_cuda:
                    on_dev.append((i, g, b, inst["gt_classes"]))
                else:
                    gb[i, :g] = b.reshape(-1, 4).to(torch.float32)
                    gc[i, :g] = inst["gt_classes"].to(torch.int32)
            cnt[i] = g
        gbd, gcd, cntd = ops.upload_packed([gb, gc, cnt], self.device)
        for i, g, b, cl in on_dev:
            gbd[i, :g] = b.reshape(-1, 4).to(torch.float32)
            gcd[i, :g] = cl.to(torch.int32)
        return {"boxes": gbd, "classes": gcd, "count": cntd, "host_count": cnt.tolist()}

    def geometry(self, Hs: int, Ws: int):
        key = (Hs, Ws)
        if key not in self._anchor_cache:
            shapes = []
            h, w = Hs // 4, Ws // 4
            for l in range(4):
                shapes.append((h, w))
                if l < 3:
                    h, w = h // 2, w // 2
            shapes.append(((shapes[3][0] - 1) // 2 + 1, (shapes[3][1] - 1) // 2 + 1))
            geom = ops.make_geom(shapes, NUM_ANCHORS, self.Ch)
            anchors = make_anchors(shapes, self.device, getattr(self, "anchor_sizes", self.p.anchor_sizes))
            self._anchor_cache[key] = (shapes, geom, anchors)
            while len(self._anchor_cache) > 16:
                self._anchor_cache.pop(next(iter(self._anchor_cache)))
        else:
            self._anchor_cache[key] = self._anchor_cache.pop(key)
        return self._anchor_cache[key]

    def workspace(self, name: str, nbytes: int) -> torch.Tensor:
        t = self._ws.get(name)
        if t is None or t.numel() < nbytes:
            t = torch.empty(nbytes, dtype=torch.uint8, device=self.device)
            self._ws[name] = t
        return t

    def _conv_call(self, x, name, *, relu=False, res=None, res_mode=0, want_f32=False, out=None, bits_out=None):
        W = self.wts
        p = W.layout.t[name]
        return x, W.w(name), dict(stride=p.stride, pad=p.pad, scale=W.scale(name), shift=W.shift(name), res=res, res_mode=res_mode, relu=relu,
                                  want_f32=want_f32, out=out, bits_out=bits_out)

    def conv(self, x, name, **kw):
        x, w, kw = self._conv_call(x, name, **kw)
        return ops.conv2d(x, w, **kw)

    def _serve(self, req):
        if isinstance(req, list):
            return ops.conv2d_group([self._conv_call(r[0], r[1], **r[2]) for r in req])
        return self.conv(req[0], req[1], **req[2])

    def _drive(self, gen):
        try:
            req = next(gen)
            while True:
                req = gen.send(self._serve(req))
        except StopIteration as e:
            return e.value

    @staticmethod
    def drive_pair(eng_a, gen_a, eng_b, gen_b, streams=None):
        res = [None, None]
        ctx_a = torch.cuda.stream(streams[0]) if streams else contextlib.nullcontext()
        ctx_b = torch.cuda.stream(streams[1]) if streams else contextlib.nullcontext()
        try:
            with ctx_a:
                ra = next(gen_a)
        except StopIteration as e:
            ra, res[0] = None, e.value
        try:
            with ctx_b:
                rb = next(gen_b)
        except StopIteration as e:
            rb, res[1] = None, e.value
        while ra is not None or rb is not None:
            if streams:
                if ra is not None:
                    with ctx_a:
                        ya = eng_a._serve(ra)
                        try:
                            ra = gen_a.send(ya)
                        except StopIteration as e:
                            ra, res[0] = None, e.value
                if rb is not None:
                    with ctx_b:
                        yb = eng_b._serve(rb)
                        try:
                            rb = gen_b.send(yb)
                        except StopIteration as e:
                            rb, res[1] = None, e.value
                continue
            if ra is not None and rb is not None:
                la, lb = (ra if isinstance(ra, list) else [ra]), (rb if isinstance(rb, list) else [rb])
                ys = ops.conv2d_group([eng_a._conv_call(r[0], r[1], **r[2]) for r in la] + [eng_b._conv_call(r[0], r[1], **r[2]) for r in lb])
                ya = ys[:len(la)] if isinstance(ra, list) else ys[0]
                yb = ys[len(la):] if isinstance(rb, list) else ys[len(la)]
            elif ra is not None:
                ya = eng_a._serve(ra)
            else:
                yb = eng_b._serve(rb)
            if ra is not None:
                try:
                    ra = gen_a.send(ya)
                except StopIteration as e:
                    ra, res[0] = None, e.value
            if rb is not None:
                try:
                    rb = gen_b.send(yb)
                except StopIteration as e:
                    rb, res[1] = None, e.value
        return res[0], res[1]

    def trunk(self, st_u8: torch.Tensor, sizes, save: bool) -> Ctx:
        return self._drive(self.trunk_steps(st_u8, sizes, save))

    def prefix_pipelinable(self) -> bool:
        return type(self) is RCNN and self.dtype == torch.bfloat16 and self.fused_stem and self.fused_res2

    def trunk_steps(self, st_u8: torch.Tensor, sizes, save: bool, fpn: bool = True, pre: Optional[torch.Tensor] = None,
                    prefix_out: Optional[torch.Tensor] = None):
        W = self.wts
        c = Ctx()
        bu = "backbone.bottom_up."
        if pre is not None:
            x = pre
        elif self.dtype == torch.bfloat16 and self.fused_stem:
            x = ops.stem_pool_forward(st_u8, sizes, W.stem_packed(bu + "stem.conv1"), W.scale(bu + "stem.conv1"), W.shift(bu + "stem.conv1"),
                                      self.p.pixel_mean, self.p.pixel_std)
        else:
            stem = ops.stem_forward(st_u8, sizes, W.w_master(bu + "stem.conv1"), W.scale(bu + "stem.conv1"), W.shift(bu + "stem.conv1"),
                                    self.p.pixel_mean, self.p.pixel_std, self.dtype)
            x = ops.maxpool3s2(stem)
            del stem
        blocks = []
        cs = []
        out_bits = {}
        fuse2 = self.dtype == torch.bfloat16 and self.fused_res2
        if fuse2:
            res2 = [f"{bu}res2.{b}.conv{k}" for b in range(STAGE_BLOCKS[0]) for k in (1, 2, 3)]
            fw = dict(zip(res2, W.folded(res2)))
        assert prefix_out is None or (fuse2 and pre is None)
        for si, nb in enumerate(STAGE_BLOCKS):
            if si == 0 and pre is not None:
                cs.append(x)
                continue
            for b in range(nb):
                p = f"{bu}res{si + 2}.{b}."
                sc = (yield x, p + "shortcut", {}) if b == 0 else x
                if si == 0 and fuse2:
                    x = ops.bottleneck_fused(x, sc, fw[p + "conv1"], fw[p + "conv2"], fw[p + "conv3"], W.shift(p + "conv1"), W.shift(p + "conv2"),
                                             W.shift(p + "conv3"), out=prefix_out if (prefix_out is not None and b == nb - 1) else None)
                    continue
                want_bits = save and si > 0 and self.mask_bits and self.dtype == torch.bfloat16

                def bits_for(inp, name):
                    if not want_bits:
                        return None
                    lt = W.layout.t[name]
                    ho = (inp.shape[1] + 2 * lt.pad - lt.kk) // lt.stride + 1
                    wo = (inp.shape[2] + 2 * lt.pad - lt.kk) // lt.stride + 1
                    return torch.empty(inp.shape[0] * ho * wo * (lt.wshape[0] // 8), dtype=torch.uint8, device=self.device)
                b1 = bits_for(x, p + "conv1") if self.mask_bits_inner else None
                h1 = yield x, p + "conv1", dict(relu=True, bits_out=b1)
                b2 = bits_for(h1, p + "conv2") if self.mask_bits_inner else None
                h2 = yield h1, p + "conv2", dict(relu=True, bits_out=b2)
                bits = bits_for(h2, p + "conv3")
                out = yield h2, p + "conv3", dict(relu=True, res=sc, res_mode=1, bits_out=bits)
                if save and si > 0:
                    blocks.append((p, x, h1, h2, out, b == 0))
                    if bits is not None:
                        out_bits[out.data_ptr()] = bits
                        if b1 is not None:
                            out_bits[h1.data_ptr()], out_bits[h2.data_ptr()] = b1, b2
                x = out
            cs.append(x)
            if prefix_out is not None:
                return x
        if not fpn:
            if save:
                c.blocks, c.cs, c.out_bits = blocks, cs, out_bits
            else:
                c.cs = cs
            return c
        prev = {}
        P = {}
        prev[5] = yield cs[3], "backbone.fpn_lateral5", {}
        if self.level_groups:
            for lvl in (4, 3, 2):
                prev[lvl] = yield cs[lvl - 2], f"backbone.fpn_lateral{lvl}", dict(res=prev[lvl + 1], res_mode=2)
            outs = yield [(prev[lvl], f"backbone.fpn_output{lvl}", {}) for lvl in (2, 3, 4, 5)]
            P.update(zip((2, 3, 4, 5), outs))
        else:
            P[5] = yield prev[5], "backbone.fpn_output5", {}
            for lvl in (4, 3, 2):
                prev[lvl] = yield cs[lvl - 2], f"backbone.fpn_lateral{lvl}", dict(res=prev[lvl + 1], res_mode=2)
                P[lvl] = yield prev[lvl], f"backbone.fpn_output{lvl}", {}
        P[6] = ops.subsample2(P[5])
        c.P = [P[2], P[3], P[4], P[5], P[6]]
        if save:
            c.blocks, c.cs, c.prev, c.out_bits = blocks, cs, prev, out_bits
        return c

    def rpn_head(self, c: Ctx, save: bool):
        self._drive(self.rpn_head_steps(c, save))

    def rpn_head_steps(self, c: Ctx, save: bool):
        px = [f.shape[0] * f.shape[1] * f.shape[2] for f in c.P]
        flat = torch.empty((1, sum(px), 1, FPN_C), dtype=self.dtype, device=self.device)
        ts, o, reqs = [], 0, []
        for f, n in zip(c.P, px):
            view = flat[0, o:o + n, 0].view(f.shape[0], f.shape[1], f.shape[2], FPN_C)
            reqs.append((f, "proposal_generator.rpn_head.conv", dict(relu=True, out=view)))
            o += n
        if self.level_groups:
            ts = yield reqs
        else:
            for r in reqs:
                ts.append((yield r))
        hf = yield flat, "rpn_head_out", dict(want_f32=True)
        heads, o = [], 0
        for f, n in zip(c.P, px):
            heads.append(hf[0, o:o + n, 0].view(f.shape[0], f.shape[1], f.shape[2], hf.shape[3]))
            o += n
        c.head, c.head_flat = heads, hf
        if save:
            c.rpn_t = ts

    def box_head(self, pooled: torch.Tensor, c: Optional[Ctx] = None):
        R = pooled.shape[0]
        x = pooled.view(R, 1, 1, POOL * POOL * FPN_C)
        fc1 = self.conv(x, "roi_heads.box_head.fc1", relu=True)
        bits2 = None
        if c is not None and self.mask_bits and self.dtype == torch.bfloat16 and R > 0 and os.environ.get("ALDI_MASK_BITS_FC", "1") == "1":
            bits2 = torch.empty(R * (FC_DIM // 8), dtype=torch.uint8, device=self.device)
        fc2 = self.conv(fc1, "roi_heads.box_head.fc2", relu=True, bits_out=bits2)
        pred = self.conv(fc2, "box_pred", want_f32=True).view(R, self.Cp)
        if c is not None:
            c.pooled, c.fc1, c.fc2 = pooled, fc1, fc2
            if bits2 is not None:
                if c.get("out_bits") is None:
                    c.out_bits = {}
                c.out_bits[fc2.data_ptr()] = bits2
        return pred, fc2

    def roi_feats(self, c: Ctx, grads=None):
        return ops.make_roi_feats(c.P[:4], grads, [1.0 / s for s in STRIDES[:4]])

    def _sample_host(self, counts: List[List[int]], batch: int, frac: float):
        N = len(counts)
        S = batch
        sel = torch.zeros((N, 2, S), dtype=torch.int32)
        nsel = torch.zeros((N, 2), dtype=torch.int32)
        for n, (npos, nneg) in enumerate(counts):
            num_pos = min(npos, int(batch * frac))
            num_neg = min(nneg, batch - num_pos)
            perm1 = randperm_prefix(npos, num_pos)
            perm2 = randperm_prefix(nneg, num_neg)
            sel[n, 0, :num_pos] = perm1.to(torch.int32)
            sel[n, 1, :num_neg] = perm2.to(torch.int32)
            nsel[n, 0], nsel[n, 1] = num_pos, num_neg
        return sel, nsel, nsel.tolist()

    def _sample(self, counts: List[List[int]], batch: int, frac: float):
        sel, nsel, h = self._sample_host(counts, batch, frac)
        sel_d, nsel_d = ops.upload_packed([sel, nsel], self.device)
        return sel_d, nsel_d, h

    def rpn_match(self, geom, anchors, gt, N):
        sumA = anchors.shape[0]
        dev = self.device
        best_iou = torch.empty((N, sumA), dtype=torch.float32, device=dev)
        best_idx = torch.empty((N, sumA), dtype=torch.int32, device=dev)
        labels = torch.empty((N, sumA), dtype=torch.int32, device=dev)
        scratch = ops.box_match_scratch(N, GMAX, dev)
        ops.box_match(anchors, 0, None, sumA, gt["boxes"], gt["count"], GMAX, N, self.p.rpn_iou[0], self.p.rpn_iou[1], True, best_iou, best_idx, scratch, labels)
        lists = torch.empty((N, 2, sumA), dtype=torch.int32, device=dev)
        counts = torch.empty((N, 2), dtype=torch.int32, device=dev)
        ops.compact_labels(labels, sumA, N, 0, lists, counts)
        return labels, best_idx, lists, counts

    def rpn_sample(self, lists, counts, N, host_counts=None):
        if host_counts is None:
            both = torch.cat([counts.view(-1), self.err.view(-1)]).cpu().tolist()
            raise_on_error(both[-1])
            host_counts = [both[2 * i: 2 * i + 2] for i in range(N)]
        lists = lists.contiguous()
        sel, nsel, nsel_h = self._sample(host_counts, self.p.rpn_batch, self.p.rpn_pos_frac)
        L_ = lists.shape[2]
        labels = torch.empty((N, L_), dtype=torch.int32, device=self.device)
        ops.rpn_apply_sample(labels, L_, N, lists, sel, nsel, self.p.rpn_batch)
        n_fg = sum(a for a, _ in nsel_h)
        n_valid = sum(a + b for a, b in nsel_h)
        return labels, n_valid, n_fg, host_counts

    def proposals(self, c: Ctx, geom, anchors, hw, N, training: bool):
        nl = 5
        ws = self.workspace("rpn", ops.rpn_proposals_workspace(N, nl))
        post = self.p.rpn_post[0 if training else 1]
        boxes = torch.empty((N, post, 4), dtype=torch.float32, device=self.device)
        scores = torch.empty((N, post), dtype=torch.float32, device=self.device)
        count = torch.empty((N,), dtype=torch.int32, device=self.device)
        ops.rpn_proposals(geom, c.head, anchors, hw, N, self.p.rpn_pre[0 if training else 1], post, self.p.rpn_nms, ws, boxes, scores, count, self.err)
        return boxes, scores, count

    def forward_train(self, images, instances, *, roi_seed: Optional[int] = None, pre_roi_hook=None,
                      gt_dev: Optional[dict] = None, do_align: bool = False, labeled: bool = True,
                      da_weights: Tuple[float, float] = (0.0, 0.0)) -> Ctx:
        N = len(images)
        st, sizes, hw = self.stage_images(images)
        shapes, geom, anchors = self.geometry(st.shape[2], st.shape[3])
        gt = gt_dev if gt_dev is not None else self.stage_gt(instances)
        c = self.trunk(st, sizes, save=True)
        c.N, c.sizes, c.hw, c.geom, c.anchors, c.gt, c.shapes = N, sizes, hw, geom, anchors, gt, shapes
        self.rpn_head(c, save=True)
        dev = self.device
        _, matched, lists, counts = self.rpn_match(geom, anchors, gt, N)
        labels, _, _, c.rpn_host_counts = self.rpn_sample(lists, counts, N)
        c.rpn_labels, c.rpn_matched, c.rpn_lists, c.rpn_counts = labels, matched, lists, counts
        c.loss_rpn = torch.zeros(2, dtype=torch.float32, device=dev)
        ops.rpn_loss(geom, c.head, None, anchors, labels, matched, gt["boxes"], gt["count"], GMAX, N, 1.0 / (self.p.rpn_batch * N), 0.0, 0.0, c.loss_rpn)
        c.props, c.prop_scores, c.prop_count = self.proposals(c, geom, anchors, hw, N, training=True)
        if pre_roi_hook is not None:
            pre_roi_hook()
        if roi_seed is not None:
            torch.manual_seed(roi_seed)
        self.roi_sample(c, c.props, c.prop_count, gt, N)
        self.roi_forward(c)
        c.loss_box = torch.zeros(2, dtype=torch.float32, device=dev)
        ops.box_loss(c.pred, self.Cp, self.K, c.R, c.rois, c.r_cls, c.r_gt, self.p.roi_weights, 0.0, 0.0, None, c.loss_box)
        c.align = {}
        c.distill = None
        c.labeled, c.da_weights = labeled, da_weights
        if do_align:
            self.align_forward(c, labeled, da_weights)
        return c

    def forward_train_fused(self, specs: List[dict]) -> Ctx:
        dev = self.device
        images = [im for sp in specs for im in sp["images"]]
        N = len(images)
        st, sizes, hw = self.stage_images(images)
        shapes, geom, anchors = self.geometry(st.shape[2], st.shape[3])
        c = self.trunk(st, sizes, save=True)
        c.N, c.sizes, c.hw, c.geom, c.anchors, c.shapes = N, sizes, hw, geom, anchors, shapes
        self.rpn_head(c, save=True)
        side = self._wgrad_stream()
        if side is not None:
            side.wait_stream(torch.cuda.current_stream())
            with torch.cuda.stream(side):
                c.props, c.prop_scores, c.prop_count = self.proposals(c, geom, anchors, hw, N, training=True)
        else:
            c.props, c.prop_scores, c.prop_count = self.proposals(c, geom, anchors, hw, N, training=True)
        for sp in specs:
            if sp.get("gt_lazy") is not None:
                sp["gt_dev"] = sp["gt_lazy"]()
        for sp in specs:
            if sp.get("gt_wait") is not None:
                sp["gt_wait"]()
        gts = [sp["gt_dev"] if sp.get("gt_dev") is not None else self.stage_gt(sp["instances"]) for sp in specs]
        gt = {k: torch.cat([g[k] for g in gts]) for k in ("boxes", "classes", "count")}
        c.gt = gt
        _, matched, lists, counts = self.rpn_match(geom, anchors, gt, N)
        if side is not None:
            torch.cuda.current_stream().wait_stream(side)
        prep = self._roi_prepare(c.props, c.prop_count, gt, N)
        both = torch.cat([counts.view(-1), prep["counts"].view(-1), self.err.view(-1)]).cpu().tolist()
        raise_on_error(both[-1], "student")
        rpn_counts = [both[2 * i: 2 * i + 2] for i in range(N)]
        roi_counts = [both[2 * N + 2 * i: 2 * N + 2 * i + 2] for i in range(N)]
        rsel, rnsel, rh, osel, onsel, oh = [], [], [], [], [], []
        n0 = 0
        chunks = []
        for sp in specs:
            n1 = n0 + len(sp["images"])
            if sp.get("pre_rpn"):
                sp["pre_rpn"]()
            a, b, h_ = self._sample_host(rpn_counts[n0:n1], self.p.rpn_batch, self.p.rpn_pos_frac)
            rsel.append(a); rnsel.append(b); rh += h_
            if sp.get("pre_roi"):
                sp["pre_roi"]()
            a, b, h2 = self._sample_host(roi_counts[n0:n1], self.p.roi_batch, self.p.roi_pos_frac)
            osel.append(a); onsel.append(b); oh += h2
            chunks.append(dict(n0=n0, n1=n1, labeled=sp.get("labeled", True), do_align=sp.get("do_align", False),
                               da_weights=sp.get("da_weights", (0.0, 0.0)), rpn_counts=rpn_counts[n0:n1], roi_counts=roi_counts[n0:n1]))
            n0 = n1
        labels = torch.empty((N, anchors.shape[0]), dtype=torch.int32, device=dev)
        rsel_d, rnsel_d, osel_d, onsel_d = ops.upload_packed([torch.cat(rsel), torch.cat(rnsel), torch.cat(osel), torch.cat(onsel)], dev)
        ops.rpn_apply_sample(labels, anchors.shape[0], N, lists, rsel_d, rnsel_d, self.p.rpn_batch)
        c.rpn_labels, c.rpn_matched, c.rpn_lists, c.rpn_counts = labels, matched, lists, counts
        self._roi_gather(c, prep, osel_d, onsel_d, oh, gt, N)
        r0 = 0
        for ch, sp in zip(chunks, specs):
            r1 = r0 + sum(c.rows[ch["n0"]:ch["n1"]])
            if sp.get("post_rois") is not None:
                sp["post_rois"](c, ch["n0"], r0, r1)
            r0 = r1
        self.roi_forward(c)
        r0 = 0
        for ch in chunks:
            n0, n1 = ch["n0"], ch["n1"]
            r1 = r0 + sum(c.rows[n0:n1])
            ch["r0"], ch["r1"] = r0, r1
            ch["loss_rpn"] = torch.zeros(2, dtype=torch.float32, device=dev)
            ch["loss_box"] = torch.zeros(2, dtype=torch.float32, device=dev)
            nc = n1 - n0
            ops.rpn_loss(geom, [h[n0:n1] for h in c.head], None, anchors, labels[n0:n1], matched[n0:n1], gt["boxes"][n0:n1], gt["count"][n0:n1],
                         GMAX, nc, 1.0 / (self.p.rpn_batch * nc), 0.0, 0.0, ch["loss_rpn"])
            ops.box_loss(c.pred[r0:r1], self.Cp, self.K, r1 - r0, c.rois[r0:r1], c.r_cls[r0:r1], c.r_gt[r0:r1], self.p.roi_weights, 0.0, 0.0, None, ch["loss_box"])
            ch["align"] = {}
            ch["distill"] = None
            if ch["do_align"]:
                self._align_forward_chunk(c, ch)
            r0 = r1
        c.chunks = chunks
        c.align = {}
        c.distill = None
        return c

    def _align_forward_chunk(self, c: Ctx, ch: dict):
        dev = self.device
        label = 1.0 if ch["labeled"] else 0.0
        n0, n1, r0, r1 = ch["n0"], ch["n1"], ch["r0"], ch["r1"]
        if self.has_img_da:
            acts, pooled, logit = self._img_disc_forward(c.P[self.img_da_level][n0:n1])
            ch["loss_da_img"] = torch.zeros(1, dtype=torch.float32, device=dev)
            ops.domain_bce(logit, logit.shape[-1], n1 - n0, label, ch["da_weights"][0], 0.0, None, ch["loss_da_img"])
            ch["align"]["img"] = (acts, pooled, logit)
        if self.has_ins_da and r1 > r0:
            acts, logit = self._ins_disc_forward(c.fc2[r0:r1])
            ch["loss_da_ins"] = torch.zeros(1, dtype=torch.float32, device=dev)
            ops.domain_bce(logit, logit.shape[-1], r1 - r0, label, ch["da_weights"][1], 0.0, None, ch["loss_da_ins"])
            ch["align"]["ins"] = (acts, logit)

    def _img_disc_forward(self, feat: torch.Tensor):
        acts = [feat]
        for name in self.img_da_layers[:-1]:
            acts.append(self.conv(acts[-1], name, relu=True))
        pooled = ops.avgpool(acts[-1])
        return acts, pooled, self.conv(pooled, self.img_da_layers[-1], want_f32=True)

    def _ins_disc_forward(self, feat: torch.Tensor):
        acts = [feat]
        for name in self.ins_da_layers[:-1]:
            acts.append(self.conv(acts[-1], name, relu=True))
        return acts, self.conv(acts[-1], self.ins_da_layers[-1], want_f32=True)

    def distill_forward_chunk(self, c: Ctx, ch: dict, teacher_head, teacher_pred, labels, n_valid, n_fg, values=True, **kw):
        dev = self.device
        n0, n1, r0, r1 = ch["n0"], ch["n1"], ch["r0"], ch["r1"]
        ch["distill"] = dict(t_head=teacher_head, t_pred=teacher_pred, labels=labels, n_valid=n_valid, n_fg=n_fg, **kw)
        if not values:
            return
        ch["loss_dist_rpn"] = torch.zeros(2, dtype=torch.float32, device=dev)
        ch["loss_dist_roi"] = torch.zeros(2, dtype=torch.float32, device=dev)
        ops.rpn_distill_loss(c.geom, [h[n0:n1] for h in c.head], teacher_head, None, labels, n1 - n0, kw["obj_T"], n_valid, n_fg,
# ... 676 lines not shown
```

### aldi_amd/ops.py

```python
from __future__ import annotations

import ctypes as C
import os
from typing import List, Optional, Sequence

import torch

from . import _lib as L


def dtype_code(t: torch.dtype) -> int:
    if t == torch.float32:
        return L.F32
    if t == torch.bfloat16:
        return L.BF16
    raise TypeError(f"unsupported dtype {t}")


def _p(t: Optional[torch.Tensor]):
    return None if t is None else t.data_ptr()


_RAW_STREAM = getattr(torch._C, "_cuda_getCurrentRawStream", None)


def stream_ptr() -> int:
    if _RAW_STREAM is not None:
        return _RAW_STREAM(torch.cuda.current_device())
    return torch.cuda.current_stream().cuda_stream


def upload_packed(tensors, device):
    metas, off = [], 0
    for t in tensors:
        nb = t.numel() * t.element_size()
        metas.append((off, nb))
        off += (nb + 15) // 16 * 16
    host = torch.empty(max(off, 16), dtype=torch.uint8).pin_memory()
    for t, (o, nb) in zip(tensors, metas):
        if nb:
            host[o:o + nb] = t.contiguous().view(-1).view(torch.uint8)
    dev = host.to(device, non_blocking=True)
    return [dev[o:o + nb].view(t.dtype).view(t.shape) for t, (o, nb) in zip(tensors, metas)]


def conv2d(x: torch.Tensor, w: torch.Tensor, *, stride: int = 1, pad: int = 0,
           scale: Optional[torch.Tensor] = None, shift: Optional[torch.Tensor] = None,
           res: Optional[torch.Tensor] = None, res_mode: int = 0, relu: bool = False,
           mask: Optional[torch.Tensor] = None, out: Optional[torch.Tensor] = None,
           out_f32: Optional[torch.Tensor] = None, want_f32: bool = False,
           out_scale: int = 1, out_hw=None, ksplit: Optional[int] = None, mask_bits: Optional[torch.Tensor] = None,
           bits_out: Optional[torch.Tensor] = None) -> torch.Tensor:
    N, H, W_, Cin = x.shape
    Cout, KH, KW, Cin2 = w.shape
    assert Cin == Cin2 and x.is_contiguous() and w.is_contiguous() and x.dtype == w.dtype, (x.shape, w.shape, x.dtype, w.dtype)
    Ho = (H + 2 * pad - KH) // stride + 1
    Wo = (W_ + 2 * pad - KW) // stride + 1
    if out_scale > 1:
        OH, OW = out_hw
        shape = (N, OH, OW, Cout)
    else:
        OH = OW = 0
        shape = (N, Ho, Wo, Cout)
    if out is None and not want_f32:
        out = torch.empty(shape, dtype=x.dtype, device=x.device)
    if want_f32 and out_f32 is None:
        out_f32 = torch.empty(shape, dtype=torch.float32, device=x.device)
    ws = None
    if ksplit is None:
        ksplit = _auto_ksplit(x, N * Ho * Wo, Cout, KH * KW * Cin, KH * KW == 1 and stride == 1 and pad == 0 and res is None and mask is None
                              and not want_f32 and out_f32 is None and out_scale == 1 and mask_bits is None and bits_out is None)
    if ksplit and ksplit > 1:
        ws = torch.empty(ksplit * N * Ho * Wo * Cout, dtype=torch.float32, device=x.device)
    a = L.ConvArgs(_p(x), _p(w), _p(out), _p(out_f32), _p(scale), _p(shift), _p(res), _p(mask),
                   N, H, W_, Cin, Cout, KH, KW, stride, pad, Ho, Wo,
                   int(relu), res_mode, out_scale, OH, OW, dtype_code(x.dtype), _p(ws), int(ksplit or 0), _p(mask_bits), _p(bits_out))
    L.call("aldi_conv_igemm", C.byref(a), stream_ptr())
    return out_f32 if want_f32 and out is None else out


def _auto_ksplit(x, M, Cout, K, plain: bool) -> int:
    if not plain or x.dtype != torch.bfloat16 or K < 4096 or K % 256 or os.environ.get("ALDI_SPLITK", "1") != "1":
        return 0
    tiles = ((M + 127) // 128) * ((Cout + 127) // 128)
    if not (16 <= tiles <= 160) or Cout % 4:
        return 0
    tiles256 = ((M + 255) // 256) * ((Cout + 127) // 128)
    for ks in (2, 4, 7, 8, 14, 16):
        if K % (64 * ks) == 0 and tiles256 * ks >= 216:
            return ks
    return 4 if K % 256 == 0 else 0


def _conv_args(x, w, *, stride=1, pad=0, scale=None, shift=None, res=None, res_mode=0, relu=False, mask=None, out=None, out_f32=None,
               want_f32=False, out_scale=1, out_hw=None, mask_bits=None, bits_out=None):
    N, H, W_, Cin = x.shape
    Cout, KH, KW, Cin2 = w.shape
    assert Cin == Cin2 and x.is_contiguous() and w.is_contiguous() and x.dtype == w.dtype, (x.shape, w.shape, x.dtype, w.dtype)
    Ho = (H + 2 * pad - KH) // stride + 1
    Wo = (W_ + 2 * pad - KW) // stride + 1
    if out_scale > 1:
        OH, OW = out_hw
        shape = (N, OH, OW, Cout)
    else:
        OH = OW = 0
        shape = (N, Ho, Wo, Cout)
    if out is None and not want_f32:
        out = torch.empty(shape, dtype=x.dtype, device=x.device)
    if want_f32 and out_f32 is None:
        out_f32 = torch.empty(shape, dtype=torch.float32, device=x.device)
    a = L.ConvArgs(_p(x), _p(w), _p(out), _p(out_f32), _p(scale), _p(shift), _p(res), _p(mask),
                   N, H, W_, Cin, Cout, KH, KW, stride, pad, Ho, Wo,
                   int(relu), res_mode, out_scale, OH, OW, dtype_code(x.dtype), None, 0, _p(mask_bits), _p(bits_out))
    return a, (out_f32 if want_f32 and out is None else out)


def conv2d_group(calls) -> List[torch.Tensor]:
    arr = (L.ConvArgs * len(calls))()
    outs = []
    for i, (x, w, kw) in enumerate(calls):
        arr[i], y = _conv_args(x, w, **kw)
        outs.append(y)
    L.call("aldi_conv_igemm_group", arr, len(calls), stream_ptr())
    return outs


_WGRAD_WS = {}
WGRAD_WS_EPOCH = 0
WGRAD_ORDERED = os.environ.get("ALDI_WGRAD_ORDERED", "1") != "0"


def _wgrad_workspace(arr, n: int, device) -> None:
    if not WGRAD_ORDERED:
        return
    need = L.lib.aldi_conv_wgrad_group_workspace(arr, n)
    if need < 0:
        raise RuntimeError("aldi_conv_wgrad_group_workspace: " + L.lib.aldi_last_error().decode())
    if need == 0:
        need = 256
    key = (device, stream_ptr())
    buf = _WGRAD_WS.get(key)
    if buf is None or buf.numel() * 4 < need:
        global WGRAD_WS_EPOCH
        if buf is not None:
            WGRAD_WS_EPOCH += 1
            if torch.cuda.is_current_stream_capturing():
                raise RuntimeError("the weight-gradient workspace has to grow during a hipGraph capture: run the new shapes eagerly once first")
        else:
            need = max([need] + [b.numel() * 4 for (d_, _), b in _WGRAD_WS.items() if d_ == device])
        buf = torch.empty((need + (need >> 2) + 3) // 4, dtype=torch.float32, device=device)
        _WGRAD_WS[key] = buf
    arr[0].ws = buf.data_ptr()
    arr[0].ws_bytes = buf.numel() * 4


def conv_wgrad(x: torch.Tensor, g: torch.Tensor, dw: torch.Tensor, *, KH: int, KW: int, stride: int = 1, pad: int = 0,
               scale: Optional[torch.Tensor] = None, db: Optional[torch.Tensor] = None) -> None:
    N, H, W_, Cin = x.shape
    _, Ho, Wo, Cout = g.shape
    assert dw.dtype == torch.float32 and dw.numel() == Cout * KH * KW * Cin and x.dtype == g.dtype, (dw.shape, x.shape, g.shape)
    arr = (L.WgradArgs * 1)()
    arr[0] = L.WgradArgs(_p(x), _p(g), _p(dw), _p(scale), N, H, W_, Cin, Cout, KH, KW, stride, pad, Ho, Wo, dtype_code(x.dtype), _p(db), None, 0)
    if x.dtype == torch.bfloat16:
        _wgrad_workspace(arr, 1, x.device)
    L.call("aldi_conv_wgrad", arr, stream_ptr())


def conv_wgrad_group(problems) -> None:
    arr = (L.WgradArgs * len(problems))()
    for i, (x, g, dw, kw) in enumerate(problems):
        N, H, W_, Cin = x.shape
        _, Ho, Wo, Cout = g.shape
        KH, KW = kw["KH"], kw["KW"]
        assert dw.dtype == torch.float32 and dw.numel() == Cout * KH * KW * Cin and x.dtype == g.dtype, (dw.shape, x.shape, g.shape)
        arr[i] = L.WgradArgs(_p(x), _p(g), _p(dw), _p(kw.get("scale")), N, H, W_, Cin, Cout, KH, KW, kw.get("stride", 1), kw.get("pad", 0), Ho, Wo,
                             dtype_code(x.dtype), _p(kw.get("db")), None, 0)
    _wgrad_workspace(arr, len(problems), problems[0][0].device)
    L.call("aldi_conv_wgrad_group", arr, len(problems), stream_ptr())


def noop() -> None:
    L.call("aldi_noop", stream_ptr())


def bias_grad(g: torch.Tensor, db: torch.Tensor) -> None:
    Cc = g.shape[-1]
    L.call("aldi_bias_grad", _p(g), _p(db), g.numel() // Cc, Cc, dtype_code(g.dtype), stream_ptr())


def dgrad_weights(w_master: torch.Tensor, scale: Optional[torch.Tensor], dtype: torch.dtype,
                  out: Optional[torch.Tensor] = None) -> torch.Tensor:
    Cout, KH, KW, Cin = w_master.shape
    if out is None:
        out = torch.empty((Cin, KH, KW, Cout), dtype=dtype, device=w_master.device)
    L.call("aldi_dgrad_weights", _p(w_master), _p(scale), _p(out), Cout, KH, KW, Cin, dtype_code(dtype), stream_ptr())
    return out


class DgradWeightsPlan:

    def __init__(self, entries, dtype: torch.dtype):
        dev = entries[0][0].device
        self.dtype = dtype
        self.keep = list(entries)
        sizes = [w.numel() for w, _ in entries]
        offs, tot = [], 0
        for n in sizes:
            offs.append(tot)
            tot += (n + 63) // 64 * 64
        self.buf = torch.empty(tot, dtype=dtype, device=dev)
        self.out = []
        items = (L.DgwItem * len(entries))()
        tile = 0
        for i, (w, sc) in enumerate(entries):
            Cout, KH, KW, Cin = w.shape
            o = self.buf[offs[i]:offs[i] + sizes[i]].view(Cin, KH, KW, Cout)
            self.out.append(o)
            it = items[i]
            it.w_master, it.scale, it.wt = w.data_ptr(), (sc.data_ptr() if sc is not None else None), o.data_ptr()
            it.Cout, it.KH, it.KW, it.Cin, it.tile_begin, it.reserved = Cout, KH, KW, Cin, tile, 0
            tile += KH * KW * ((Cout + 31) // 32) * ((Cin + 31) // 32)
        self.total_tiles = tile
        self.n = len(entries)
        raw = torch.frombuffer(bytearray(bytes(items)), dtype=torch.uint8)
        self.items = raw.to(dev)

    def run(self):
        L.call("aldi_dgrad_weights_batch", _p(self.items), self.n, self.total_tiles, dtype_code(self.dtype), stream_ptr())


class FoldWeightsPlan:

    def __init__(self, entries):
        dev = entries[0][0].device
        self.keep = list(entries)
        sizes = [w.numel() for w, _ in entries]
        offs, tot = [], 0
        for n in sizes:
            assert n % 8 == 0
            offs.append(tot)
            tot += (n + 63) // 64 * 64
        self.buf = torch.empty(tot, dtype=torch.bfloat16, device=dev)
        self.out = []
        items = (L.FoldItem * len(entries))()
        chunk = 0
        for i, (w, sc) in enumerate(entries):
            assert w.dtype == torch.float32 and w.is_contiguous() and w.data_ptr() % 16 == 0, "fold_weights: fp32, contiguous, 16-byte aligned"
            o = self.buf[offs[i]:offs[i] + sizes[i]].view(w.shape)
            self.out.append(o)
            it = items[i]
            it.w, it.scale, it.out = w.data_ptr(), (sc.data_ptr() if sc is not None else None), o.data_ptr()
            it.rows, it.cols, it.chunk_begin, it.reserved = w.shape[0], sizes[i] // w.shape[0], chunk, 0
            chunk += sizes[i] // 8
        self.total_chunks, self.n = chunk, len(entries)
        self.items = torch.frombuffer(bytearray(bytes(items)), dtype=torch.uint8).to(dev)

    def run(self):
        L.call("aldi_fold_weights_batch", _p(self.items), self.n, self.total_chunks, stream_ptr())


def bottleneck_fused(x: torch.Tensor, res: torch.Tensor, w1, w2, w3, b1, b2, b3, out: Optional[torch.Tensor] = None) -> torch.Tensor:
    N, H, W_, Cin = x.shape
    mid, Cout = w1.shape[0], w3.shape[0]
    assert x.dtype == torch.bfloat16 and x.is_contiguous() and res.is_contiguous() and res.shape == (N, H, W_, Cout), (x.shape, res.shape)
    assert w1.numel() == mid * Cin and w2.numel() == mid * 9 * mid and w3.numel() == Cout * mid and w1.dtype == torch.bfloat16
    if out is None:
        out = torch.empty((N, H, W_, Cout), dtype=x.dtype, device=x.device)
    a = L.BottleneckArgs(_p(x), _p(res), _p(out), _p(w1), _p(w2), _p(w3), _p(b1), _p(b2), _p(b3), N, H, W_, Cin, mid, Cout)
    L.call("aldi_bottleneck_fused", C.byref(a), stream_ptr())
    return out


def stem_forward(img_u8: torch.Tensor, sizes: Sequence[Sequence[int]], w: torch.Tensor, scale: torch.Tensor, shift: torch.Tensor,
                 mean: Sequence[float], std: Sequence[float], dtype: torch.dtype) -> torch.Tensor:
    N, _, Hs, Ws = img_u8.shape
    Hc, Wc = Hs // 2, Ws // 2
    y = torch.empty((N, Hc, Wc, 64), dtype=dtype, device=img_u8.device)
    a = L.StemArgs()
    a.img, a.w, a.scale, a.shift, a.y = _p(img_u8), _p(w), _p(scale), _p(shift), _p(y)
    a.N, a.Hs, a.Ws, a.Hc, a.Wc = N, Hs, Ws, Hc, Wc
    for i, (h, w_) in enumerate(sizes):
        a.h[i], a.w_img[i] = int(h), int(w_)
    for c in range(3):
        a.mean[c], a.std[c] = float(mean[c]), float(std[c])
    a.dtype = dtype_code(dtype)
    L.call("aldi_stem_forward", C.byref(a), stream_ptr())
    return y


def stem_pack_weights(w: torch.Tensor, out: Optional[torch.Tensor] = None) -> torch.Tensor:
    if out is None:
        out = torch.empty((64, 200), dtype=torch.bfloat16, device=w.device)
    L.call("aldi_stem_pack_weights", _p(w), _p(out), stream_ptr())
    return out


def stem_pool_forward(img_u8: torch.Tensor, sizes: Sequence[Sequence[int]], w_packed: torch.Tensor, scale: torch.Tensor, shift: torch.Tensor,
                      mean: Sequence[float], std: Sequence[float]) -> torch.Tensor:
    N, _, Hs, Ws = img_u8.shape
    Hc, Wc = Hs // 2, Ws // 2
    y = torch.empty((N, (Hc - 1) // 2 + 1, (Wc - 1) // 2 + 1, 64), dtype=torch.bfloat16, device=img_u8.device)
    a = L.StemArgs()
    a.img, a.w, a.scale, a.shift, a.y = _p(img_u8), None, _p(scale), _p(shift), None
    a.N, a.Hs, a.Ws, a.Hc, a.Wc = N, Hs, Ws, Hc, Wc
    for i, (h, w_) in enumerate(sizes):
        a.h[i], a.w_img[i] = int(h), int(w_)
    for c in range(3):
        a.mean[c], a.std[c] = float(mean[c]), float(std[c])
    a.dtype = L.BF16
    L.call("aldi_stem_pool_forward", C.byref(a), _p(w_packed), _p(y), stream_ptr())
    return y


def maxpool3s2(x: torch.Tensor) -> torch.Tensor:
    N, H, W_, Cc = x.shape
    y = torch.empty((N, (H - 1) // 2 + 1, (W_ - 1) // 2 + 1, Cc), dtype=x.dtype, device=x.device)
    L.call("aldi_maxpool3s2", _p(x), _p(y), N, H, W_, Cc, dtype_code(x.dtype), stream_ptr())
    return y


def subsample2(x: torch.Tensor) -> torch.Tensor:
    N, H, W_, Cc = x.shape
    y = torch.empty((N, (H - 1) // 2 + 1, (W_ - 1) // 2 + 1, Cc), dtype=x.dtype, device=x.device)
    L.call("aldi_subsample2", _p(x), _p(y), N, H, W_, Cc, 0, dtype_code(x.dtype), stream_ptr())
    return y


def subsample2_bwd(g_small: torch.Tensor, g_big: torch.Tensor) -> None:
    N, H, W_, Cc = g_big.shape
    L.call("aldi_subsample2", _p(g_small), _p(g_big), N, H, W_, Cc, 1, dtype_code(g_big.dtype), stream_ptr())


def upsample2_bwd(g: torch.Tensor, out: torch.Tensor, accumulate: bool) -> None:
    N, Hc, Wc, Cc = out.shape
    assert g.shape == (N, Hc * 2, Wc * 2, Cc)
    L.call("aldi_upsample2_bwd", _p(g), _p(out), N, Hc, Wc, Cc, int(accumulate), dtype_code(g.dtype), stream_ptr())


def upsample2_bwd_chain(g2: torch.Tensor, o3: torch.Tensor, o4: torch.Tensor, o5: torch.Tensor) -> None:
    N, H5, W5, Cc = o5.shape
    assert o4.shape == (N, H5 * 2, W5 * 2, Cc) and o3.shape == (N, H5 * 4, W5 * 4, Cc) and g2.shape == (N, H5 * 8, W5 * 8, Cc)
    L.call("aldi_upsample2_bwd_chain", _p(g2), _p(o3), _p(o4), _p(o5), N, H5, W5, Cc, dtype_code(g2.dtype), stream_ptr())


def add_f32(a: Optional[torch.Tensor], b: Optional[torch.Tensor], out: torch.Tensor, relu_src: Optional[torch.Tensor] = None) -> torch.Tensor:
    L.call("aldi_add_f32", _p(a), _p(b), _p(relu_src), _p(out), out.numel(), dtype_code(out.dtype), stream_ptr())
    return out


def cast_from_f32(src: torch.Tensor, dtype: torch.dtype, out: Optional[torch.Tensor] = None) -> torch.Tensor:
    if out is None:
        out = torch.empty(src.shape, dtype=dtype, device=src.device)
    L.call("aldi_cast_from_f32", _p(src), _p(out), src.numel(), dtype_code(dtype), stream_ptr())
    return out


def sgd_step(p, g, buf, p_compute, n, lr, momentum, weight_decay, grad_scale, first_step, dtype) -> None:
    L.call("aldi_sgd_step", _p(p), _p(g), _p(buf), _p(p_compute), n, lr, momentum, weight_decay, grad_scale, int(first_step),
           dtype_code(dtype), stream_ptr())


def sgd_step_dev(p, g, buf, p_compute, lo: int, hi: int, hyper: torch.Tensor, dtype) -> None:
    pc = None if p_compute is None else p_compute.data_ptr() + lo * p_compute.element_size()
    L.call("aldi_sgd_step_dev", p.data_ptr() + 4 * lo, g.data_ptr() + 4 * lo, buf.data_ptr() + 4 * lo, pc, hi - lo, _p(hyper), dtype_code(dtype), stream_ptr())


def ema_update(teacher, student, teacher_compute, n, alpha, copy_only, dtype, n_compute=None) -> None:
    nc = 0 if teacher_compute is None else (teacher_compute.numel() if n_compute is None else n_compute)
    L.call("aldi_ema_update", _p(teacher), _p(student), _p(teacher_compute), n, nc, alpha, int(copy_only), dtype_code(dtype), stream_ptr())


def bn_fold(w, b, mean, var, scale, shift, Cc) -> None:
    L.call("aldi_bn_fold", _p(w), _p(b), _p(mean), _p(var), _p(scale), _p(shift), Cc, stream_ptr())


def make_geom(shapes: Sequence[Sequence[int]], A: int, Cc: int) -> L.RpnGeom:
    g = L.RpnGeom()
    g.num_levels, g.A, g.C = len(shapes), A, Cc
    off = 0
    for i, (h, w) in enumerate(shapes):
        g.H[i], g.W[i], g.off[i] = h, w, off
        off += h * w * A
    for i in range(len(shapes), L.MAX_LEVELS + 1):
        g.off[i] = off
    return g


def ptrs(ts: Optional[Sequence[Optional[torch.Tensor]]]):
    if ts is None:
        return None
    arr = L.PtrArray5()
    for i, t in enumerate(ts):
        arr[i] = _p(t)
    return arr


def box_match(boxes, box_stride_n, box_count, Lb, gt_boxes, gt_count, Gmax, N, lo, hi, lowq, best_iou, best_idx, scratch, labels):
    L.call("aldi_box_match", _p(boxes), box_stride_n, _p(box_count), Lb, _p(gt_boxes), _p(gt_count), Gmax, N, lo, hi, int(lowq),
           _p(best_iou), _p(best_idx), _p(scratch), scratch.numel() * scratch.element_size(), _p(labels), stream_ptr())


def box_match_scratch(N: int, Gmax: int, device) -> torch.Tensor:
    return torch.empty((N, Gmax * 32), dtype=torch.int32, device=device)


def stage_images(images, batch: torch.Tensor) -> None:
    n = len(images)
    ptr = (C.c_void_p * n)(*[_p(im) for im in images])
    hs = (C.c_int * n)(*[int(im.shape[1]) for im in images])
    ws = (C.c_int * n)(*[int(im.shape[2]) for im in images])
    L.call("aldi_stage_images", ptr, hs, ws, n, batch.shape[1], batch.shape[2], batch.shape[3], _p(batch), stream_ptr())


def compact_labels(labels, Lb, N, bg, lists, counts):
    ws = torch.empty(max(int(L.lib.aldi_compact_labels_workspace(Lb, N)), 16), dtype=torch.uint8, device=labels.device)
    L.call("aldi_compact_labels", _p(labels), Lb, N, bg, _p(lists), _p(counts), _p(ws), stream_ptr())


def rpn_apply_sample(labels, Lb, N, lists, sel, nsel, S):
    L.call("aldi_rpn_apply_sample", _p(labels), Lb, N, _p(lists), _p(sel), _p(nsel), S, stream_ptr())


def rpn_loss(geom, head, grad, anchors, labels, matched, gt_boxes, gt_count, Gmax, N, inv_norm, gs_cls, gs_loc, loss2):
    L.call("aldi_rpn_loss", C.byref(geom), ptrs(head), ptrs(grad), _p(anchors), _p(labels), _p(matched), _p(gt_boxes), _p(gt_count), Gmax, N,
           inv_norm, gs_cls, gs_loc, _p(loss2), stream_ptr())


def rpn_proposals_workspace(N, nl) -> int:
    return int(L.lib.aldi_rpn_proposals_workspace(N, nl))


def rpn_proposals(geom, head, anchors, img_hw, N, pre, post, thr, workspace, out_boxes, out_scores, out_count, err):
    L.call("aldi_rpn_proposals", C.byref(geom), ptrs(head), _p(anchors), _p(img_hw), N, pre, post, thr, _p(workspace),
           _p(out_boxes), _p(out_scores), _p(out_count), _p(err), stream_ptr())


def rpn_active_pixels_workspace(geom, N) -> int:
    return int(L.lib.aldi_rpn_active_pixels_workspace(C.byref(geom), N))


def rpn_active_pixels(geom, ghead, N, cap, idx, count, workspace, err):
    L.call("aldi_rpn_active_pixels", C.byref(geom), ptrs(ghead), N, cap, _p(idx), _p(count), _p(workspace), _p(err), stream_ptr())


def rpn_sparse_gather(geom, ghead, hidden, feat, N, Cf, cap, idx, count, G, Tm, X9):
    L.call("aldi_rpn_sparse_gather", C.byref(geom), ptrs(ghead), ptrs(hidden), ptrs(feat), N, Cf, cap, _p(idx), _p(count), _p(G), _p(Tm), _p(X9),
           dtype_code(G.dtype), stream_ptr())


def rpn_sparse_scatter(geom, gfeat, Y, N, Cf, cap, idx, count):
    L.call("aldi_rpn_sparse_scatter", C.byref(geom), ptrs(gfeat), _p(Y), N, Cf, cap, _p(idx), _p(count), dtype_code(Y.dtype),
           dtype_code(gfeat[0].dtype), stream_ptr())


def make_roi_feats(feats: Sequence[torch.Tensor], grads: Optional[Sequence[torch.Tensor]], scales: Sequence[float]) -> L.RoiFeats:
    f = L.RoiFeats()
    for i, t in enumerate(feats):
        f.feat[i] = _p(t)
        f.grad[i] = _p(grads[i]) if grads is not None else None
        f.H[i], f.W[i] = t.shape[1], t.shape[2]
        f.scale[i] = scales[i]
    f.C = feats[0].shape[3]
    return f


def roi_prepare(props, pcount, P, gt_boxes, gt_classes, gt_count, Gmax, N, K, thr, cand, ccount, best_iou, best_idx, scratch, labels, cls):
    L.call("aldi_roi_prepare", _p(props), _p(pcount), P, _p(gt_boxes), _p(gt_classes), _p(gt_count), Gmax, N, K, thr, _p(cand), _p(ccount),
           _p(best_iou), _p(best_idx), _p(scratch), _p(labels), _p(cls), stream_ptr())


def roi_prepare_lists(props, pcount, P, gt_boxes, gt_classes, gt_count, Gmax, N, K, thr, cand, ccount, best_iou, best_idx, labels, cls, lists, counts, tickets,
                      tail_a=None, tail_b=None):
    L.call("aldi_roi_prepare_lists", _p(props), _p(pcount), P, _p(gt_boxes), _p(gt_classes), _p(gt_count), Gmax, N, K, thr, _p(cand), _p(ccount),
           _p(best_iou), _p(best_idx), _p(labels), _p(cls), _p(lists), _p(counts), _p(tickets), _p(tail_a), _p(tail_b), stream_ptr())


def roi_gather(cand, cls, best_idx, Lb, lists, sel, nsel, S, row_off, gt_boxes, gt_count, Gmax, N, rois, r_cls, r_gt, r_idx):
    L.call("aldi_roi_gather", _p(cand), _p(cls), _p(best_idx), Lb, _p(lists), _p(sel), _p(nsel), S, _p(row_off), _p(gt_boxes), _p(gt_count),
           Gmax, N, _p(rois), _p(r_cls), _p(r_gt), _p(r_idx), stream_ptr())


def rois_from_proposals(props, pcount, P, N, rois):
    L.call("aldi_rois_from_proposals", _p(props), _p(pcount), P, N, _p(rois), stream_ptr())


def roialign(feats: L.RoiFeats, rois, R, P, pooled, backward: bool):
    L.call("aldi_roialign", C.byref(feats), _p(rois), R, P, _p(pooled), int(backward), dtype_code(pooled.dtype), stream_ptr())


def roialign_backward(feats: L.RoiFeats, rois, R, P, g_pooled, N, rois_sorted: bool = False, grad_dtype=torch.float32):
    L.call("aldi_roialign_backward", C.byref(feats), _p(rois), R, P, _p(g_pooled), N, int(rois_sorted), dtype_code(g_pooled.dtype),
           dtype_code(grad_dtype), stream_ptr())


def box_loss(pred, Cp, K, R, rois, cls, gt_boxes, weights4, gs_cls, gs_box, grad, loss2):
    w = (C.c_float * 4)(*weights4)
    L.call("aldi_box_loss", _p(pred), Cp, K, R, _p(rois), _p(cls), _p(gt_boxes), w, gs_cls, gs_box, _p(grad), _p(loss2), stream_ptr())


def detections_workspace(N) -> int:
    return int(L.lib.aldi_detections_workspace(N))


def detections(pred, Cp, K, props, pcount, P, N, img_hw, weights4, score_thresh, nms_thresh, topk, pl_thresh, workspace,
               det_boxes, det_scores, det_cls, det_count, pl_boxes, pl_cls, pl_scores, pl_count, err):
    w = (C.c_float * 4)(*weights4)
    L.call("aldi_detections", _p(pred), Cp, K, _p(props), _p(pcount), P, N, _p(img_hw), w, score_thresh, nms_thresh, topk, pl_thresh,
           _p(workspace), _p(det_boxes), _p(det_scores), _p(det_cls), _p(det_count), _p(pl_boxes), _p(pl_cls), _p(pl_scores), _p(pl_count),
           pl_boxes.shape[1], _p(err), stream_ptr())


def rpn_distill_loss(geom, s_head, t_head, grad, labels, N, obj_T, n_valid, n_fg, do_obj, do_reg, grad_scale, loss2, counts_dev=None):
    L.call("aldi_rpn_distill_loss", C.byref(geom), ptrs(s_head), ptrs(t_head), ptrs(grad), _p(labels), N, obj_T, int(n_valid), int(n_fg),
           _p(counts_dev), int(do_obj), int(do_reg), grad_scale, _p(loss2), stream_ptr())


def box_losses_fused(pred, Cp, K, rois, cls, gt_boxes, weights4, chunks, grad, grad_lo):
    arr = (L.BoxLossChunk * len(chunks))()
    for i, q in enumerate(chunks):
        arr[i] = L.BoxLossChunk(q["r0"], q["r1"], q["gs_cls"], q["gs_box"], _p(q["loss_box"]), _p(q.get("t_pred")), float(q.get("cls_T", 1.0)),
                                int(bool(q.get("kl"))), int(bool(q.get("do_cls"))), int(bool(q.get("do_reg"))), float(q.get("gs_dcls", 0.0)),
                                float(q.get("gs_dreg", 0.0)), _p(q.get("loss_d")))
    w = (C.c_float * 4)(*weights4)
    L.call("aldi_box_losses_fused", _p(pred), Cp, K, _p(rois), _p(cls), _p(gt_boxes), w, arr, len(chunks), _p(grad), _p(grad_lo), stream_ptr())


def roih_distill_loss(s_pred, t_pred, Cp, K, R, cls_T, kl, do_cls, do_reg, grad_scale, grad, loss2):
    L.call("aldi_roih_distill_loss", _p(s_pred), _p(t_pred), Cp, K, R, cls_T, int(kl), int(do_cls), int(do_reg), grad_scale, _p(grad),
           _p(loss2), stream_ptr())


def domain_bce(pred, ld, R, label, weight, grad_scale, grad, loss):
    L.call("aldi_domain_bce", _p(pred), ld, R, label, weight, grad_scale, _p(grad), _p(loss),
           dtype_code(grad.dtype) if grad is not None else L.F32, stream_ptr())


def avgpool(x: torch.Tensor) -> torch.Tensor:
    N, H, W_, Cc = x.shape
    y = torch.empty((N, 1, 1, Cc), dtype=x.dtype, device=x.device)
    ws = torch.empty(max(int(L.lib.aldi_avgpool_workspace(N, Cc)), 16), dtype=torch.uint8, device=x.device)
    L.call("aldi_avgpool", _p(x), _p(y), N, H * W_, Cc, dtype_code(x.dtype), _p(ws), stream_ptr())
    return y


def avgpool_bwd(gy: torch.Tensor, act: torch.Tensor) -> torch.Tensor:
    N, H, W_, Cc = act.shape
    gx = torch.empty_like(act)
    L.call("aldi_avgpool_bwd", _p(gy), _p(act), _p(gx), N, H * W_, Cc, dtype_code(act.dtype), stream_ptr())
    return gx


POOL_MODES = {"avg": 0, "max": 1}


def _pool_mode(mode: str) -> int:
    if mode not in POOL_MODES:
        raise ValueError(f"pooling must be one of {sorted(POOL_MODES)}, got {mode!r}")
    return POOL_MODES[mode]


def pool_rows(x: torch.Tensor, out: torch.Tensor, mode: str = "avg", row_off: int = 0) -> torch.Tensor:
    rows, S, Cc = x.shape
    assert x.is_contiguous() and out.is_contiguous() and out.dtype == torch.float32 and out.shape[1] == Cc, (x.shape, out.shape, out.dtype)
    L.call("aldi_pool_rows", _p(x), rows, S, Cc, dtype_code(x.dtype), _pool_mode(mode), _p(out), row_off, out.shape[0], stream_ptr())
    return out


def pool_rows_counted(x: torch.Tensor, count: torch.Tensor, out: torch.Tensor, total: torch.Tensor, mode: str = "avg", row_off: int = 0) -> torch.Tensor:
    N, P, S, Cc = x.shape
    assert x.is_contiguous() and out.is_contiguous() and out.dtype == torch.float32 and out.shape[1] == Cc, (x.shape, out.shape, out.dtype)
# ... 34 lines not shown
```

### include/aldi_hip.h

```cpp
#ifndef ALDI_HIP_H
#define ALDI_HIP_H
#include <stddef.h>
#include <stdint.h>

#ifdef __cplusplus
extern "C" {
#endif

typedef void* aldi_stream_t;

enum { ALDI_F32 = 0, ALDI_BF16 = 1 };
enum { ALDI_OK = 0, ALDI_ERR_HIP = -1, ALDI_ERR_ARG = -2 };

const char* aldi_last_error(void);
int aldi_version(void);
int aldi_noop(aldi_stream_t stream);

int aldi_set_tuning(const char* name, int value);
int aldi_get_tuning(const char* name, int* value);
int aldi_reset_tuning(void);
const char* aldi_last_dispatch(void);

typedef struct {
    const void* x;
    const void* w;
    void* y;
    float* y_f32;
    const float* scale;
    const float* shift;
    const void* res;
    const void* mask;
    int N, H, W, Cin;
    int Cout, KH, KW, stride, pad;
    int Ho, Wo;
    int relu;
    int res_mode;
    int out_scale;
    int OH, OW;
    int dtype;
    void* ws;
    int ksplit;
    const void* mask_bits;
    void* bits_out;
} aldi_conv_args;

int aldi_conv_igemm(const aldi_conv_args* a, aldi_stream_t stream);
int aldi_conv_igemm_group(const aldi_conv_args* args, int n, aldi_stream_t stream);
int aldi_conv_igemm_plan(const aldi_conv_args* args, int n, char* name, int cap);

typedef struct {
    const void* x;
    const void* g;
    float* dw;
    const float* scale;
    int N, H, W, Cin, Cout, KH, KW, stride, pad, Ho, Wo;
    int dtype;
    float* db;
    void* ws;
    long ws_bytes;
} aldi_wgrad_args;
int aldi_conv_wgrad(const aldi_wgrad_args* a, aldi_stream_t stream);

int aldi_conv_wgrad_group(const aldi_wgrad_args* args, int n, aldi_stream_t stream);
long aldi_conv_wgrad_group_workspace(const aldi_wgrad_args* args, int n);
int aldi_conv_wgrad_plan(const aldi_wgrad_args* args, int n, int group, char* name, int cap, long* ws_bytes);

int aldi_bias_grad(const void* g, float* db, int M, int C, int dtype, aldi_stream_t stream);

int aldi_dgrad_weights(const float* w_master, const float* scale, void* wt, int Cout, int KH, int KW, int Cin,
                       int dtype, aldi_stream_t stream);

typedef struct aldi_dgw_item {
    const float* w_master;
    const float* scale;
    void* wt;
    int Cout, KH, KW, Cin;
    int tile_begin, reserved;
} aldi_dgw_item;
int aldi_dgrad_weights_batch(const aldi_dgw_item* items, int n_items, int total_tiles, int dtype, aldi_stream_t stream);

typedef struct aldi_bottleneck_args {
    const void* x;
    const void* res;
    void* y;
    const void* w1; const void* w2; const void* w3;
    const float* b1; const float* b2; const float* b3;
    int N, H, W, Cin, mid, Cout;
} aldi_bottleneck_args;
int aldi_bottleneck_fused(const aldi_bottleneck_args* a, aldi_stream_t stream);
typedef struct aldi_fold_item {
    const float* w; const float* scale; void* out;
    int rows, cols, chunk_begin, reserved;
} aldi_fold_item;
int aldi_fold_weights_batch(const aldi_fold_item* items, int n_items, int total_chunks, aldi_stream_t stream);

#define ALDI_MAX_IMAGES 16

typedef struct {
    const uint8_t* img;
    const float* w;
    const float* scale; const float* shift;
    void* y;
    int N, Hs, Ws, Hc, Wc;
    int h[ALDI_MAX_IMAGES], w_img[ALDI_MAX_IMAGES];
    float mean[3], std[3];
    int dtype;
} aldi_stem_args;
int aldi_stem_forward(const aldi_stem_args* a, aldi_stream_t stream);
int aldi_stem_pack_weights(const float* w, void* w_packed, aldi_stream_t stream);
int aldi_stem_pool_forward(const aldi_stem_args* a, const void* w_packed, void* y_pool, aldi_stream_t stream);

int aldi_maxpool3s2(const void* x, void* y, int N, int H, int W, int C, int dtype, aldi_stream_t stream);
int aldi_stage_images(const void* const* images, const int* heights, const int* widths, int n, int C, int Hs, int Ws, void* batch,
                      aldi_stream_t stream);
int aldi_subsample2(const void* x, void* y, int N, int H, int W, int C, int backward, int dtype, aldi_stream_t stream);
int aldi_upsample2_bwd(const void* g, void* out, int N, int Hc, int Wc, int C, int accumulate, int dtype, aldi_stream_t stream);
int aldi_upsample2_bwd_chain(const void* g2, void* o3, void* o4, void* o5, int N, int H5, int W5, int C, int dtype, aldi_stream_t stream);
int aldi_add_f32(const void* a, const float* b, const void* relu_src, void* out, long n, int dtype, aldi_stream_t stream);
int aldi_cast_from_f32(const float* src, void* dst, long n, int dtype, aldi_stream_t stream);

int aldi_sgd_step(float* p, const float* g, float* buf, void* p_compute, long n, float lr, float momentum, float weight_decay,
                  float grad_scale, int first_step, int dtype, aldi_stream_t stream);
int aldi_sgd_step_dev(float* p, const float* g, float* buf, void* p_compute, long n, const float* hyper, int dtype, aldi_stream_t stream);
int aldi_ema_update(float* teacher, const float* student, void* teacher_compute, long n, long n_compute, double alpha, int copy_only, int dtype,
                    aldi_stream_t stream);
int aldi_bn_fold(const float* w, const float* b, const float* mean, const float* var, float* scale, float* shift, int C, aldi_stream_t stream);

#define ALDI_MAX_LEVELS 5
typedef struct {
    int num_levels;
    int A;
    int C;
    int H[ALDI_MAX_LEVELS], W[ALDI_MAX_LEVELS];
    int off[ALDI_MAX_LEVELS + 1];
} aldi_rpn_geom;

int aldi_box_match(const float* boxes, long box_stride_n, const int* box_count, int L,
                   const float* gt_boxes, const int* gt_count, int Gmax, int N,
                   float lo, float hi, int allow_low_quality,
                   float* best_iou, int* best_idx, unsigned* gt_best_scratch, size_t gt_best_bytes, int* labels, aldi_stream_t stream);
size_t aldi_compact_labels_workspace(int L, int N);
int aldi_compact_labels(const int* labels, int L, int N, int bg_label, int* lists, int* counts, void* workspace, aldi_stream_t stream);
int aldi_rpn_apply_sample(int* labels, int L, int N, const int* lists, const int* sel, const int* nsel, int S, aldi_stream_t stream);
int aldi_rpn_loss(const aldi_rpn_geom* gm, float* const* head, float* const* grad, const float* anchors, const int* labels, const int* matched,
                  const float* gt_boxes, const int* gt_count, int Gmax, int N, float inv_norm, float grad_scale_cls, float grad_scale_loc,
                  float* loss2, aldi_stream_t stream);
size_t aldi_rpn_proposals_workspace(int N, int num_levels);
int aldi_rpn_proposals(const aldi_rpn_geom* gm, float* const* head, const float* anchors, const int* img_hw, int N,
                       int pre_nms_topk, int post_nms_topk, float nms_thresh, void* workspace,
                       float* out_boxes, float* out_scores, int* out_count, int* err_flag, aldi_stream_t stream);

size_t aldi_rpn_active_pixels_workspace(const aldi_rpn_geom* gm, int N);
int aldi_rpn_active_pixels(const aldi_rpn_geom* gm, float* const* grad_head, int N, int cap, int* idx, int* count, void* workspace,
                           int* err_flag, aldi_stream_t stream);
int aldi_rpn_sparse_gather(const aldi_rpn_geom* gm, float* const* grad_head, const void* const* hidden, const void* const* feat, int N, int Cf,
                           int cap, const int* idx, const int* count, void* G, void* Tm, void* X9, int dtype, aldi_stream_t stream);
int aldi_rpn_sparse_scatter(const aldi_rpn_geom* gm, void* const* gfeat, const void* Y, int N, int Cf, int cap, const int* idx,
                            const int* count, int dtype, int grad_dtype, aldi_stream_t stream);

typedef struct {
    const void* feat[4];
    float* grad[4];
    int H[4], W[4];
    float scale[4];
    int C;
} aldi_roi_feats;

int aldi_roi_prepare(const float* props, const int* pcount, int P, const float* gt_boxes, const int* gt_classes, const int* gt_count,
                     int Gmax, int N, int K, float iou_thresh, float* cand, int* ccount, float* best_iou, int* best_idx,
                     unsigned* gt_best_scratch, int* labels, int* cls, aldi_stream_t stream);
int aldi_roi_prepare_lists(const float* props, const int* pcount, int P, const float* gt_boxes, const int* gt_classes, const int* gt_count,
                           int Gmax, int N, int K, float iou_thresh, float* cand, int* ccount, float* best_iou, int* best_idx, int* labels,
                           int* cls, int* lists, int* counts, unsigned* tickets, const int* tail_a, const int* tail_b, aldi_stream_t stream);
int aldi_roi_gather(const float* cand, const int* cls, const int* best_idx, int L, const int* lists, const int* sel, const int* nsel, int S,
                    const int* row_off, const float* gt_boxes, const int* gt_count, int Gmax, int N,
                    float* rois, int* r_cls, float* r_gt, int* r_idx, aldi_stream_t stream);
int aldi_rois_from_proposals(const float* props, const int* pcount, int P, int N, float* rois, aldi_stream_t stream);
int aldi_roialign(const aldi_roi_feats* f, const float* rois, int R, int P, void* pooled, int backward, int dtype, aldi_stream_t stream);
int aldi_roialign_backward(const aldi_roi_feats* f, const float* rois, int R, int P, const void* g_pooled, int N, int rois_sorted, int dtype,
                           int grad_dtype, aldi_stream_t stream);

int aldi_box_loss(const float* pred, int Cp, int K, int R, const float* rois, const int* cls, const float* gt_boxes,
                  const float* weights4, float grad_scale_cls, float grad_scale_box, float* grad, float* loss2, aldi_stream_t stream);
typedef struct {
    int r0, r1;
    float grad_scale_cls, grad_scale_box;
    float* loss_box;
    const float* teacher_pred;
    float cls_temperature;
    int kl, do_cls, do_reg;
    float grad_scale_distill_cls, grad_scale_distill_reg;
    float* loss_distill;
} aldi_box_loss_chunk;
int aldi_box_losses_fused(const float* pred, int Cp, int K, const float* rois, const int* cls, const float* gt_boxes, const float* weights4,
                          const aldi_box_loss_chunk* chunks, int nchunks, float* grad, void* grad_lo, aldi_stream_t stream);
size_t aldi_detections_workspace(int N);
int aldi_detections(const float* pred, int Cp, int K, const float* props, const int* pcount, int P, int N, const int* img_hw,
                    const float* weights4, float score_thresh, float nms_thresh, int topk, float pl_thresh, void* workspace,
                    float* det_boxes, float* det_scores, int* det_cls, int* det_count,
                    float* pl_boxes, int* pl_cls, float* pl_scores, int* pl_count, int pl_rows, int* err_flag, aldi_stream_t stream);

int aldi_rpn_distill_loss(const aldi_rpn_geom* gm, float* const* student_head, float* const* teacher_head, float* const* grad,
                          const int* labels, int N, float obj_temperature, int n_valid, int n_fg, const int* n_valid_fg_dev,
                          int do_obj, int do_reg, float grad_scale, float* loss2, aldi_stream_t stream);
int aldi_roih_distill_loss(const float* student_pred, const float* teacher_pred, int Cp, int K, int R, float cls_temperature,
                           int kl, int do_cls, int do_reg, float grad_scale, float* grad, float* loss2, aldi_stream_t stream);
int aldi_domain_bce(const float* pred, int ld, int R, float label, float weight, float grad_scale, void* grad, float* loss,
                    int dtype, aldi_stream_t stream);
size_t aldi_avgpool_workspace(int N, int C);
int aldi_avgpool(const void* x, void* y, int N, int HW, int C, int dtype, void* workspace, aldi_stream_t stream);
int aldi_avgpool_bwd(const void* gy, const void* act, void* gx, int N, int HW, int C, int dtype, aldi_stream_t stream);

int aldi_torch_randperm_prefix(unsigned char* state, long n, long k, long* out);
int aldi_torch_rng_script(unsigned char* state, const long* script, int nops, int* out, int threads);
int aldi_step_draws(unsigned char* state, const int* counts, int N, const int* chunks, int nch, const long* seeds, int nseeds,
                    int rpn_batch, int rpn_pos_cap, int roi_batch, int roi_pos_cap, int* words, const int* word0, int* rows_out, int threads);
int aldi_torch_rng_prefetch(const unsigned char* state, const long* seeds, int nseeds, long max_draws);
int aldi_torch_rng_prefetch_hits(void);
int aldi_torch_rng_prefetch_wait(void);

int aldi_aug_sum_u8(const unsigned char* img, long n, unsigned long long* sum, aldi_stream_t stream);
int aldi_aug_blend(unsigned char* img, int H, int W, int mode, double w, const unsigned long long* sum, aldi_stream_t stream);
int aldi_aug_blur(const unsigned char* img, unsigned char* out, float* tmp0, float* tmp1, int H, int W, const double* weights, int radius,
                  aldi_stream_t stream);
int aldi_aug_erase(unsigned char* img, int H, int W, int h0, int w0, int h, int w, const float* fill, aldi_stream_t stream);
int aldi_aug_mic(unsigned char* img, int H, int W, const unsigned char* mask, int mh, int mw, aldi_stream_t stream);
int aldi_aug_hwc_to_chw(const unsigned char* in, unsigned char* out, int H, int W, aldi_stream_t stream);

enum { ALDI_AUG_COLOUR = 1, ALDI_AUG_GRAY = 2, ALDI_AUG_BLUR = 4, ALDI_AUG_CHW_IN = 8, ALDI_AUG_CHW_OUT = 16 };
enum { ALDI_AUG_HALO = 8 };
typedef struct aldi_aug_desc {
    const unsigned char* src;
    unsigned char* dst;
    const unsigned char* mask;
    unsigned long long sum;
    double wc, wb, ws, wg;
    double taps[ALDI_AUG_HALO + 1];
    long fill_off[3];
    int H, W, flags, radius;
    int rect[3][4];
    int nerase, mh, mw;
    int tile_begin;
    int sum_begin, sum_blocks;
} aldi_aug_desc;
typedef struct aldi_aug_fill_job {
    const unsigned int* snap;
    long out_off;
    int pos, ndoubles;
} aldi_aug_fill_job;
int aldi_aug_batch_sums(aldi_aug_desc* desc, int n, int nblocks, aldi_stream_t stream);
int aldi_aug_batch_fills(const aldi_aug_fill_job* jobs, int njobs, unsigned char* arena, aldi_stream_t stream);
int aldi_aug_batch_view(const aldi_aug_desc* desc, int n, int ntiles, const unsigned char* arena, aldi_stream_t stream);
int aldi_np_mt_advance(unsigned int* key, int* pos, long n, long seg, unsigned int* snaps, int* snap_pos, long max_snaps);

enum { ALDI_COCO_AREAS = 4, ALDI_COCO_THRS = 10, ALDI_COCO_RECS = 101 };
int aldi_coco_postprocess(const float* boxes, const float* scores, const long* classes, const int* entry, const double* meta, long n,
                          int num_classes, double* out_boxes, double* out_scores, unsigned char* out_valid, aldi_stream_t stream);
size_t aldi_coco_match_workspace(long num_gt);
int aldi_coco_match(const double* det_boxes, const int* det_off, const double* gt_boxes, const double* gt_area, const unsigned char* gt_flags,
                    const int* gt_off, int num_segments, long num_gt, const double* area_rng, const double* iou_thrs, int max_det,
                    void* workspace, unsigned long long* matched, unsigned long long* dt_ignore, int* num_gt_out, aldi_stream_t stream);
int aldi_coco_accumulate(const long* perm, const int* cat_off, const unsigned long long* matched, const unsigned long long* dt_ignore,
                         const int* num_gt, int num_images, int num_classes, const double* rec_thrs, double* precision, double* recall,
                         int* valid, aldi_stream_t stream);


int aldi_layernorm_forward(const void* x, const int* map, const float* gamma, const float* beta, void* y, float* mean,
                           float* rstd, int rows, int C, float eps, int relu, int dtype, aldi_stream_t stream);
int aldi_layernorm_backward(const void* g, const void* x, const int* map, const float* gamma, const float* mean, const float* rstd,
                            const void* res, const void* mask, void* dx, float* dgamma, float* dbeta, int rows, int C, int dtype,
                            aldi_stream_t stream);
int aldi_gelu(const void* x, const void* g, void* out, long n, int dtype, aldi_stream_t stream);
int aldi_rows_add(const void* a, const void* b, const int* map, const float* scale, void* out, int rows, int C,
                  int rows_per_sample, int dtype, aldi_stream_t stream);
int aldi_patchify(const uint8_t* img, void* out, int N, int Hs, int Ws, int P, const int* hw, const float* mean, const float* std,
                  int dtype, aldi_stream_t stream);
int aldi_linear_resize(const float* in, float* out, int L0, int L1, int C, int backward, aldi_stream_t stream);
int aldi_bicubic_resize(const float* in, float* out, int S0h, int S0w, int gh, int gw, int C, int backward, aldi_stream_t stream);
int aldi_add_pos(const void* x, const float* pos, void* y, int N, long TC, int dtype, aldi_stream_t stream);
int aldi_sum_batch(const void* g, float* out, int N, long TC, int dtype, aldi_stream_t stream);
int aldi_maxpool2(const void* x, void* y, unsigned char* idx, int N, int H, int W, int C, int backward, int dtype, aldi_stream_t stream);
int aldi_adamw_step(float* p, const float* g, float* m, float* v, void* p_compute, long n, float lr, float beta1, float beta2,
                    float eps, float weight_decay, int step, float grad_scale, int dtype, aldi_stream_t stream);

typedef struct {
    const void* qkv;
    const float* rel_h;
    const float* rel_w;
    void *Qp, *Kp, *KpT, *VT, *QsT;
    void* O;
    float* lse;
    const void* dO;
    void *dOT, *dQp;
    float* delta;
    void* dqkv;
    float *drel_h, *drel_w;
    int nB, gh, gw, heads, Dq;
    float scale;
} aldi_attn_args;
int aldi_attn_layout(int gh, int gw, int rel, int* Dq, int* tiled, long* vt_cols);
int aldi_attn_prepare(const aldi_attn_args* a, aldi_stream_t stream);
int aldi_attn_forward(const aldi_attn_args* a, aldi_stream_t stream);
int aldi_attn_backward(const aldi_attn_args* a, aldi_stream_t stream);

int aldi_ms_deform_attn_forward(const float* value, const int* spatial_shapes, const int* level_start_index, const float* sampling_loc,
                                const float* attn_weight, float* out, int N, int S, int M, int D, int Lq, int L, int P, aldi_stream_t stream);
int aldi_ms_deform_attn_backward(const float* value, const int* spatial_shapes, const int* level_start_index, const float* sampling_loc,
                                 const float* attn_weight, const float* grad_out, float* grad_value, float* grad_sampling_loc,
                                 float* grad_attn_weight, int N, int S, int M, int D, int Lq, int L, int P, aldi_stream_t stream);

int aldi_ms_deform_attn_backward_self(const float* value, const int* spatial_shapes, const int* level_start_index, const int* spatial_shapes_host,
                                      const float* sampling_loc, const float* attn_weight, const float* grad_out, float* grad_value,
                                      float* grad_sampling_loc, float* grad_attn_weight, void* workspace, size_t workspace_bytes,
                                      int N, int S, int M, int D, int L, int P, aldi_stream_t stream);
size_t aldi_ms_deform_attn_backward_self_workspace(const int* spatial_shapes_host, int N, int S, int M, int L, int P);

size_t aldi_group_norm_workspace(int N, int HW, int G);
int aldi_group_norm_forward(const float* x, const float* gamma, const float* beta, float* y, float* mean, float* rstd, void* workspace, int N, int HW,
                            int C, int G, float eps, aldi_stream_t stream);
int aldi_msda_prepare(const float* raw, const float* ref, const int* spatial_shapes, float* sampling_loc, float* attn_weight, long T, int M, int L, int P,
                      aldi_stream_t stream);
int aldi_mha_small_forward(const float* q, const float* k, const float* v, float* out, float* lse, int B, int Q, int H, int D, int ldq, int ldk, int ldv,
                           float scale, float drop_p, unsigned long long seed, aldi_stream_t stream);
int aldi_dropout_add(const float* x, const float* res, float* out, long n, float p, unsigned long long seed, aldi_stream_t stream);
int aldi_msda_prepare_backward(const float* g_loc, const float* g_aw, const float* attn_weight, const int* spatial_shapes, float* g_raw, float* g_ref, long T,
                               int M, int L, int P, aldi_stream_t stream);
int aldi_mha_small_backward(const float* q, const float* k, const float* v, const float* out, const float* d_out, const float* lse, float* dq, float* dk,
                            float* dv, float* delta, int B, int Q, int H, int D, int ldq, int ldk, int ldv, int lddq, int lddk, int lddv, float scale,
                            float drop_p, unsigned long long seed, aldi_stream_t stream);
size_t aldi_group_norm_backward_workspace(int N, int HW, int C, int G);
int aldi_group_norm_backward(const float* g, const float* x, const float* gamma, const float* mean, const float* rstd, float* dx, float* dgamma,
                             float* dbeta, void* workspace, int N, int HW, int C, int G, aldi_stream_t stream);
int aldi_detr_box_finish_backward(const float* g_boxes, const float* boxes, const float* ref, float* g_t, float* g_ref, long R, long refs,
                                  aldi_stream_t stream);
int aldi_detr_match_cost(const float* logits, const float* boxes, const int* t_labels, const float* t_boxes, const int* t_count, float* cost, int LB, int B,
                         int Nq, int K, int Gmax, float w_class, float w_bbox, float w_giou, float alpha, aldi_stream_t stream);
int aldi_detr_set_loss(const float* logits, const float* boxes, const int* match, const int* t_labels, const float* t_boxes, float* rows, float* losses,
                       float* g_logits, float* g_boxes, int LB, int B, int Nq, int K, int Gmax, float alpha, float c_ce, float c_bbox, float c_giou,
                       float num_boxes, aldi_stream_t stream);
int aldi_mask_rows(float* x, const unsigned char* keep, long T, int C, aldi_stream_t stream);
int aldi_detr_box_finish(const float* t, const float* ref, float* boxes, long R, long refs, aldi_stream_t stream);

int aldi_dwconv7(const void* x, const void* wt, const float* bias, void* y, int N, int H, int W, int C, int flip, int dtype, aldi_stream_t stream);
int aldi_dwconv7_wgrad(const void* x, const void* g, float* dw, int N, int H, int W, int C, int dtype, aldi_stream_t stream);
int aldi_scale_add(const void* x, const void* y, const float* gamma, const float* scale, void* out, long rows, int C, int rows_per_sample,
                   int dtype, aldi_stream_t stream);
int aldi_scale_add_backward(const void* g, const void* y, const float* gamma, const float* scale, void* dy, float* dgamma, long rows, int C,
                            int rows_per_sample, int dtype, aldi_stream_t stream);

enum { ALDI_POOL_AVG = 0, ALDI_POOL_MAX = 1 };
int aldi_pool_rows(const void* x, long rows, int S, int C, int dtype, int mode, float* out, long row_off, long out_rows, aldi_stream_t stream);
int aldi_pool_rows_counted(const void* x, int N, int P, int S, int C, int dtype, int mode, const int* count, float* out, long row_off,
                           long out_rows, int* total, aldi_stream_t stream);
size_t aldi_moments_workspace(int C);
int aldi_moments_accum(const float* X, int n, const int* n_dev, int n_cap, int C, double* sum, double* gram, double* count, void* workspace,
                       aldi_stream_t stream);
int aldi_project2(const float* X, long n, int C, const double* mean, const double* comp, float* Y, aldi_stream_t stream);

#ifdef __cplusplus
}
#endif
#endif
```

Before: 503.1.

## Fold res2.0 shortcut conv into fused bottleneck; persistent double-buffered stem-pool kernel

```diff
diff --git a/aldi_amd/csrc/bneck.hip b/aldi_amd/csrc/bneck.hip
--- a/aldi_amd/csrc/bneck.hip
+++ b/aldi_amd/csrc/bneck.hip
@@ -16,6 +16,7 @@
     const bf16_t* x; const bf16_t* res; bf16_t* y;
     const bf16_t* w1; const bf16_t* w2; const bf16_t* w3;
     const float* b1; const float* b2; const float* b3;
+    const bf16_t* wsc; const float* ssc; const float* bsc;
     int N, H, W, th, tw, xcd;
     unsigned x_bytes, y_bytes;
 };
@@ -38,9 +39,10 @@
     return t;
 }
 
-template <int CX>
+template <int CX, bool SC>
 __global__ __launch_bounds__(256, 2) void bneck_kernel(BneckDev p) {
     static_assert(CX % 32 == 0, "x slabs of 32 channels");
+    static_assert(!SC || CX == 64, "the shortcut's x tile is one 128-byte row per pixel");
     __shared__ __attribute__((aligned(128))) uint4 lds[kLdsBytes / 16];
     const int tid = threadIdx.x, lane = tid & 63, wave = __builtin_amdgcn_readfirstlane(tid >> 6);
     const int fr = lane & 15, fq = lane >> 4;
@@ -68,6 +70,18 @@
         sh2[j] = *reinterpret_cast<const float4*>(p.b2 + j * 16 + fq * 4);
         sh3[j] = *reinterpret_cast<const float4*>(p.b3 + (wave * 4 + j) * 16 + fq * 4);
     }
+    u32x4_t wscf[SC ? 4 : 1][2];
+    float4 ssc[SC ? 4 : 1], bsc[SC ? 4 : 1];
+    if constexpr (SC) {
+#pragma unroll
+        for (int j = 0; j < 4; ++j) {
+#pragma unroll
+            for (int ks = 0; ks < 2; ++ks)
+                wscf[j][ks] = *reinterpret_cast<const u32x4_t*>(p.wsc + ((wave * 4 + j) * 16 + fr) * MID + ks * 32 + fq * 8);
+            ssc[j] = *reinterpret_cast<const float4*>(p.ssc + (wave * 4 + j) * 16 + fq * 4);
+            bsc[j] = *reinterpret_cast<const float4*>(p.bsc + (wave * 4 + j) * 16 + fq * 4);
+        }
+    }
 
     unsigned xoff[3];
 #pragma unroll
@@ -199,6 +213,15 @@
         const int c = tid + it * 256, row = c >> 3, q = c & 7;
         glds16(rw3, &lds[kRegA / 16 + wbase + it * 256], (unsigned)((row * MID + (q ^ ((row >> 1) & 7)) * 8) * 2));
     }
+    if constexpr (SC) {
+#pragma unroll
+        for (int it = 0; it < 4; ++it) {
+            const int c = tid + it * 256, row = c >> 3, q = c & 7;
+            const int gh = h0 + (row >> 4), gw = w0 + (row & 15);
+            const bool ok = gh < p.H && gw < p.W;
+            glds16(rx, &lds[kRegB / 16 + wbase + it * 256], ok ? (unsigned)(((img_pix + (long)gh * p.W + gw) * CX + (q ^ ((row >> 1) & 7)) * 8) * 2) : OOB);
+        }
+    }
 #pragma unroll
     for (int i = 0; i < 2; ++i) {
         const int row = (wave * 2 + i) * 16 + fr;
@@ -211,42 +234,111 @@
     asm volatile("s_waitcnt vmcnt(0) lgkmcnt(0)" ::: "memory");
     __builtin_amdgcn_s_barrier();
     __builtin_amdgcn_sched_barrier(0);
-    f32x4_t acc3[8][4];
-#pragma unroll
-    for (int i = 0; i < 8; ++i)
-#pragma unroll
-        for (int j = 0; j < 4; ++j) acc3[i][j] = f32x4_t{0.f, 0.f, 0.f, 0.f};
-#pragma unroll
-    for (int ks = 0; ks < 2; ++ks) {
-        const int sw = (ks * 4 + fq) ^ ((fr >> 1) & 7);
-        const unsigned ab = lbase + kRegC + (unsigned)((fr * 8 + sw) * 16);
-        const unsigned w3b = lbase + kRegA + (unsigned)(((wave * 64 + fr) * 8 + sw) * 16);
-        u32x4_t af[8], wf[4];
-        frag_read_all<8, 128>(af, ab);
-        frag_read_all<4, 128>(wf, w3b);
-        frag_wait<8, 4>(af, wf);
-#pragma unroll
+    if constexpr (!SC) {
+        f32x4_t acc3[8][4];
+    #pragma unroll
         for (int i = 0; i < 8; ++i)
-#pragma unroll
-            for (int j = 0; j < 4; ++j) acc3[i][j] = Mma<bf16_t>::run(wf[j], af[i], acc3[i][j]);
-    }
-    __builtin_amdgcn_s_barrier();
-    __builtin_amdgcn_sched_barrier(0);
-#pragma unroll
-    for (int j = 0; j < 4; ++j) {
-        const int co = (wave * 4 + j) * 16 + fq * 4;
-        const float4 sh = sh3[j];
-#pragma unroll
-        for (int i = 0; i < 8; ++i) {
-            uint2 t;
-            t.x = pack2_bf16(acc3[i][j][0] + sh.x, acc3[i][j][1] + sh.y);
-            t.y = pack2_bf16(acc3[i][j][2] + sh.z, acc3[i][j][3] + sh.w);
-            lds_write_b64(lbase + (unsigned)((i * 16 + fr) * kStgRow + co * 2), t);
-        }
-    }
-    asm volatile("s_waitcnt lgkmcnt(0)" ::: "memory");
-    __builtin_amdgcn_s_barrier();
-    __builtin_amdgcn_sched_barrier(0);
+    #pragma unroll
+            for (int j = 0; j < 4; ++j) acc3[i][j] = f32x4_t{0.f, 0.f, 0.f, 0.f};
+    #pragma unroll
+        for (int ks = 0; ks < 2; ++ks) {
+            const int sw = (ks * 4 + fq) ^ ((fr >> 1) & 7);
+            const unsigned ab = lbase + kRegC + (unsigned)((fr * 8 + sw) * 16);
+            const unsigned w3b = lbase + kRegA + (unsigned)(((wave * 64 + fr) * 8 + sw) * 16);
+            u32x4_t af[8], wf[4];
+            frag_read_all<8, 128>(af, ab);
+            frag_read_all<4, 128>(wf, w3b);
+            frag_wait<8, 4>(af, wf);
+    #pragma unroll
+            for (int i = 0; i < 8; ++i)
+    #pragma unroll
+                for (int j = 0; j < 4; ++j) acc3[i][j] = Mma<bf16_t>::run(wf[j], af[i], acc3[i][j]);
+        }
+        __builtin_amdgcn_s_barrier();
+        __builtin_amdgcn_sched_barrier(0);
+    #pragma unroll
+        for (int j = 0; j < 4; ++j) {
+            const int co = (wave * 4 + j) * 16 + fq * 4;
+            const float4 sh = sh3[j];
+    #pragma unroll
+            for (int i = 0; i < 8; ++i) {
+                uint2 t;
+                t.x = pack2_bf16(acc3[i][j][0] + sh.x, acc3[i][j][1] + sh.y);
+                t.y = pack2_bf16(acc3[i][j][2] + sh.z, acc3[i][j][3] + sh.w);
+                lds_write_b64(lbase + (unsigned)((i * 16 + fr) * kStgRow + co * 2), t);
+            }
+        }
+        asm volatile("s_waitcnt lgkmcnt(0)" ::: "memory");
+        __builtin_amdgcn_s_barrier();
+        __builtin_amdgcn_sched_barrier(0);
+    } else {
+        uint2 outp[8][4];
+#pragma unroll
+        for (int hf = 0; hf < 2; ++hf) {
+            f32x4_t acc[8][2];
+            uint2 scp[8][2];
+#pragma unroll
+            for (int ks = 0; ks < 2; ++ks) {
+                const int sw = (ks * 4 + fq) ^ ((fr >> 1) & 7);
+                u32x4_t xf[8];
+                frag_read_all<8, 128>(xf, lbase + kRegB + (unsigned)((fr * 8 + sw) * 16));
+                frag_wait<8, 0>(xf, xf);
+#pragma unroll
+                for (int i = 0; i < 8; ++i)
+#pragma unroll
+                    for (int jj = 0; jj < 2; ++jj)
+                        acc[i][jj] = Mma<bf16_t>::run(wscf[hf * 2 + jj][ks], xf[i], ks == 0 ? f32x4_t{0.f, 0.f, 0.f, 0.f} : acc[i][jj]);
+            }
+#pragma unroll
+            for (int jj = 0; jj < 2; ++jj) {
+                const float4 sc = ssc[hf * 2 + jj], sh = bsc[hf * 2 + jj];
+#pragma unroll
+                for (int i = 0; i < 8; ++i) {
+                    float v0 = acc[i][jj][0] * sc.x, v1 = acc[i][jj][1] * sc.y, v2 = acc[i][jj][2] * sc.z, v3 = acc[i][jj][3] * sc.w;
+                    v0 += sh.x; v1 += sh.y; v2 += sh.z; v3 += sh.w;
+                    scp[i][jj].x = pack2_bf16(v0, v1);
+                    scp[i][jj].y = pack2_bf16(v2, v3);
+                }
+            }
+#pragma unroll
+            for (int ks = 0; ks < 2; ++ks) {
+                const int sw = (ks * 4 + fq) ^ ((fr >> 1) & 7);
+                u32x4_t af[8], wf[2];
+                frag_read_all<8, 128>(af, lbase + kRegC + (unsigned)((fr * 8 + sw) * 16));
+                frag_read_all<2, 128>(wf, lbase + kRegA + (unsigned)(((wave * 64 + hf * 32 + fr) * 8 + sw) * 16));
+                frag_wait<8, 2>(af, wf);
+#pragma unroll
+                for (int i = 0; i < 8; ++i)
+#pragma unroll
+                    for (int jj = 0; jj < 2; ++jj)
+                        acc[i][jj] = Mma<bf16_t>::run(wf[jj], af[i], ks == 0 ? f32x4_t{0.f, 0.f, 0.f, 0.f} : acc[i][jj]);
+            }
+#pragma unroll
+            for (int jj = 0; jj < 2; ++jj) {
+                const float4 sh = sh3[hf * 2 + jj];
+#pragma unroll
+                for (int i = 0; i < 8; ++i) {
+                    const unsigned s0 = pack2_bf16(acc[i][jj][0] + sh.x, acc[i][jj][1] + sh.y), s1 = pack2_bf16(acc[i][jj][2] + sh.z, acc[i][jj][3] + sh.w);
+                    const unsigned r0 = scp[i][jj].x, r1 = scp[i][jj].y;
+                    outp[i][hf * 2 + jj].x = pack2_bf16(fmaxf(__uint_as_float(s0 << 16) + __uint_as_float(r0 << 16), 0.f),
+                                                        fmaxf(__uint_as_float(s0 & 0xffff0000u) + __uint_as_float(r0 & 0xffff0000u), 0.f));
+                    outp[i][hf * 2 + jj].y = pack2_bf16(fmaxf(__uint_as_float(s1 << 16) + __uint_as_float(r1 << 16), 0.f),
+                                                        fmaxf(__uint_as_float(s1 & 0xffff0000u) + __uint_as_float(r1 & 0xffff0000u), 0.f));
+                }
+            }
+        }
+        __builtin_amdgcn_s_barrier();
+        __builtin_amdgcn_sched_barrier(0);
+#pragma unroll
+        for (int j = 0; j < 4; ++j) {
+            const int co = (wave * 4 + j) * 16 + fq * 4;
+#pragma unroll
+            for (int i = 0; i < 8; ++i) lds_write_b64(lbase + (unsigned)((i * 16 + fr) * kStgRow + co * 2), outp[i][j]);
+        }
+        asm volatile("s_waitcnt lgkmcnt(0)" ::: "memory");
+        __builtin_amdgcn_s_barrier();
+        __builtin_amdgcn_sched_barrier(0);
+    }
     {
         const __amdgpu_buffer_rsrc_t rr = make_rsrc_uniform(p.res, p.y_bytes);
         const __amdgpu_buffer_rsrc_t ry = make_rsrc_uniform(p.y, p.y_bytes);
@@ -260,8 +352,10 @@
             const bool ok = gh < p.H && gw < p.W;
             goff[it] = ok ? (unsigned)(((img_pix + (long)gh * p.W + gw) * CO + ch * 8) * 2) : OOB;
         }
-#pragma unroll
-        for (int it = 0; it < NI; ++it) rres[it] = __builtin_amdgcn_raw_buffer_load_b128(rr, goff[it], 0, 0);
+        if constexpr (!SC) {
+#pragma unroll
+            for (int it = 0; it < NI; ++it) rres[it] = __builtin_amdgcn_raw_buffer_load_b128(rr, goff[it], 0, 0);
+        }
         u32x4_t sv[NI];
         stg_read_all<NI, 8 * kStgRow>(sv, lbase + (unsigned)((tid >> 5) * kStgRow + (tid & 31) * 16));
         asm volatile("s_waitcnt lgkmcnt(0)" ::: "memory");
@@ -269,12 +363,14 @@
         for (int it = 0; it < NI; ++it) asm volatile("" : "+v"(sv[it]));
 #pragma unroll
         for (int it = 0; it < NI; ++it) {
-            u32x4_t ov;
-#pragma unroll
-            for (int q = 0; q < 4; ++q) {
-                const float lo = fmaxf(__uint_as_float(sv[it][q] << 16) + __uint_as_float(rres[it][q] << 16), 0.f);
-                const float hi = fmaxf(__uint_as_float(sv[it][q] & 0xffff0000u) + __uint_as_float(rres[it][q] & 0xffff0000u), 0.f);
-                ov[q] = pack2_bf16(lo, hi);
+            u32x4_t ov = sv[it];
+            if constexpr (!SC) {
+#pragma unroll
+                for (int q = 0; q < 4; ++q) {
+                    const float lo = fmaxf(__uint_as_float(sv[it][q] << 16) + __uint_as_float(rres[it][q] << 16), 0.f);
+                    const float hi = fmaxf(__uint_as_float(sv[it][q] & 0xffff0000u) + __uint_as_float(rres[it][q] & 0xffff0000u), 0.f);
+                    ov[q] = pack2_bf16(lo, hi);
+                }
             }
             __builtin_amdgcn_raw_buffer_store_b128(ov, ry, goff[it], 0, 0);
         }
@@ -310,27 +406,38 @@
     return ALDI_OK;
 }
 
-extern "C" int aldi_bottleneck_fused(const aldi_bottleneck_args* a, aldi_stream_t stream) {
-    if (!a || !a->x || !a->res || !a->y || !a->w1 || !a->w2 || !a->w3 || !a->b1 || !a->b2 || !a->b3)
+static int launch_bneck(const aldi_bottleneck_args* a, const void* wsc, const float* ssc, const float* bsc, aldi_stream_t stream) {
+    const bool sc = wsc != nullptr;
+    if (!a || !a->x || (!sc && !a->res) || !a->y || !a->w1 || !a->w2 || !a->w3 || !a->b1 || !a->b2 || !a->b3)
         return aldi_set_error_msg(ALDI_ERR_ARG, "bottleneck_fused: null pointer");
-    if (a->mid != MID || a->Cout != CO || (a->Cin != 64 && a->Cin != 256) || a->N < 1 || a->H < 1 || a->W < 1)
-        return aldi_set_error_msg(ALDI_ERR_ARG, "bottleneck_fused: built for Cin in {64, 256}, 64 mid channels, 256 output channels (res2)");
+    if (a->mid != MID || a->Cout != CO || (a->Cin != 64 && (sc || a->Cin != 256)) || a->N < 1 || a->H < 1 || a->W < 1)
+        return aldi_set_error_msg(ALDI_ERR_ARG, sc ? "bottleneck_fused_sc: built for 64 input, 64 mid and 256 output channels (res2.0)"
+                                                   : "bottleneck_fused: built for Cin in {64, 256}, 64 mid channels, 256 output channels (res2)");
     const size_t xb = (size_t)a->N * a->H * a->W * a->Cin * 2, yb = (size_t)a->N * a->H * a->W * CO * 2;
     if (xb >= 0x80000000ull || yb >= 0x80000000ull) return aldi_set_error_msg(ALDI_ERR_ARG, "bottleneck_fused: operand larger than 2 GiB (32-bit buffer offsets)");
     BneckDev d;
     d.x = static_cast<const bf16_t*>(a->x); d.res = static_cast<const bf16_t*>(a->res); d.y = static_cast<bf16_t*>(a->y);
     d.w1 = static_cast<const bf16_t*>(a->w1); d.w2 = static_cast<const bf16_t*>(a->w2); d.w3 = static_cast<const bf16_t*>(a->w3);
     d.b1 = a->b1; d.b2 = a->b2; d.b3 = a->b3;
+    d.wsc = static_cast<const bf16_t*>(wsc); d.ssc = ssc; d.bsc = bsc;
     d.N = a->N; d.H = a->H; d.W = a->W; d.th = cdiv(a->H, TH); d.tw = cdiv(a->W, TW);
     d.xcd = aldi_tuning().igemm_xcd;
     d.x_bytes = (unsigned)xb; d.y_bytes = (unsigned)yb;
     const int tiles = a->N * d.th * d.tw;
     hipStream_t st = static_cast<hipStream_t>(stream);
-    if (a->Cin == 64) hipLaunchKernelGGL(bneck_kernel<64>, dim3(tiles), dim3(256), 0, st, d);
-    else hipLaunchKernelGGL(bneck_kernel<256>, dim3(tiles), dim3(256), 0, st, d);
+    if (sc) hipLaunchKernelGGL((bneck_kernel<64, true>), dim3(tiles), dim3(256), 0, st, d);
+    else if (a->Cin == 64) hipLaunchKernelGGL((bneck_kernel<64, false>), dim3(tiles), dim3(256), 0, st, d);
+    else hipLaunchKernelGGL((bneck_kernel<256, false>), dim3(tiles), dim3(256), 0, st, d);
     ALDI_CHECK_LAUNCH();
     char name[64];
-    snprintf(name, sizeof(name), "bottleneck_fused<bf16,%d,64,256>", a->Cin);
+    snprintf(name, sizeof(name), "bottleneck_fused<bf16,%d,64,256%s>", a->Cin, sc ? ",shortcut" : "");
     aldi_note_dispatch(name);
     return ALDI_OK;
 }
+
+extern "C" int aldi_bottleneck_fused(const aldi_bottleneck_args* a, aldi_stream_t stream) { return launch_bneck(a, nullptr, nullptr, nullptr, stream); }
+
+extern "C" int aldi_bottleneck_fused_sc(const aldi_bottleneck_args* a, const void* wsc, const float* sc_scale, const float* sc_shift, aldi_stream_t stream) {
+    if (!wsc || !sc_scale || !sc_shift) return aldi_set_error_msg(ALDI_ERR_ARG, "bottleneck_fused_sc: null pointer");
+    return launch_bneck(a, wsc, sc_scale, sc_shift, stream);
+}
diff --git a/aldi_amd/csrc/elementwise.hip b/aldi_amd/csrc/elementwise.hip
--- a/aldi_amd/csrc/elementwise.hip
+++ b/aldi_amd/csrc/elementwise.hip
@@ -221,107 +221,181 @@
     const bf16_t* wpk;
     bf16_t* yp;
     int Hp, Wp;
+    int tiles_x, tiles_y, n_tiles;
 };
 
-__global__ __launch_bounds__(256) void stem_pool_mfma_kernel(StemPoolDev q) {
+constexpr int kStemPoolTH = 37, kStemPoolTW = 40, kStemPoolPT = 7;
+
+struct StemTile { int n, ty, tx; };
+__device__ __forceinline__ StemTile stem_tile(const StemPoolDev& q, int t) {
+    const int per = q.tiles_x * q.tiles_y;
+    StemTile r;
+    r.n = t / per;
+    const int rem = t - r.n * per;
+    r.ty = rem / q.tiles_x; r.tx = rem - r.ty * q.tiles_x;
+    r.n = __builtin_amdgcn_readfirstlane(r.n); r.ty = __builtin_amdgcn_readfirstlane(r.ty); r.tx = __builtin_amdgcn_readfirstlane(r.tx);
+    return r;
+}
+__device__ __forceinline__ StemTile stem_tile_advance(const StemPoolDev& q, StemTile a, const StemTile d) {
+    a.tx += d.tx;
+    if (a.tx >= q.tiles_x) { a.tx -= q.tiles_x; ++a.ty; }
+    a.ty += d.ty;
+    if (a.ty >= q.tiles_y) { a.ty -= q.tiles_y; ++a.n; }
+    a.n += d.n;
+    return a;
+}
+__device__ __forceinline__ void stem_fetch(const StemPoolDev& q, const StemTile tl, const int tid, uint32_t (&raw)[6]) {
+    constexpr int TH = kStemPoolTH;
     const StemDev& p = q.s;
-    constexpr int TH = 37, TW = 40, WK = kStemWK, PT = 7, CS = 144;
-    constexpr int kWlBytes = 64 * WK * 2, kTileBytes = 3 * TH * TW * 2, kCtBytes = 256 * CS;
-    __shared__ __attribute__((aligned(16))) unsigned char smem[(kWlBytes + kTileBytes) > kCtBytes ? (kWlBytes + kTileBytes) : kCtBytes];
-    bf16_t* wl = reinterpret_cast<bf16_t*>(smem);
-    bf16_t* tile = reinterpret_cast<bf16_t*>(smem + kWlBytes);
-    const int n = blockIdx.z;
-    const int py0 = blockIdx.y * PT, px0 = blockIdx.x * PT;
-    const int cy0 = 2 * py0 - 1, cx0 = 2 * px0 - 1;
+    const int r = tid >> 1, half = tid & 1;
+    const int c = r / TH, yy = r - c * TH;
+    const int iy = tl.ty * (4 * kStemPoolPT) - 5 + yy, x0 = tl.tx * (4 * kStemPoolPT) - 5 + half * 20 - 3;
+    const bool rok = r < 3 * TH && iy >= 0 && iy < p.h[tl.n];
+    const uint8_t* row = p.img + (((long)tl.n * 3 + (rok ? c : 0)) * p.Hs + (rok ? iy : 0)) * p.Ws;
+#pragma unroll
+    for (int i = 0; i < 6; ++i) {
+        int x = x0 + 4 * i;
+        x = x < 0 ? 0 : (x > p.Ws - 4 ? p.Ws - 4 : x);
+        raw[i] = *reinterpret_cast<const uint32_t*>(row + x);
+    }
+}
+__device__ __forceinline__ void stem_convert(const StemPoolDev& q, const StemTile tl, const int tid, const uint32_t (&raw)[6], bf16_t* tile) {
+    constexpr int TH = kStemPoolTH, TW = kStemPoolTW;
+    const StemDev& p = q.s;
+    const int r = tid >> 1, half = tid & 1;
+    if (r >= 3 * TH) return;
+    const int c = r / TH, yy = r - c * TH;
+    const int iy = tl.ty * (4 * kStemPoolPT) - 5 + yy, ix0 = tl.tx * (4 * kStemPoolPT) - 5;
+    const bool rok = iy >= 0 && iy < p.h[tl.n];
+    const int xlim = p.wd[tl.n] - ix0 < TH ? p.wd[tl.n] - ix0 : TH;
+    const int klo = rok ? -ix0 - half * 20 : 20, khi = xlim - half * 20;
+    const float mean = p.mean[c], inv = p.inv_std[c];
+    uint2* dst = reinterpret_cast<uint2*>(tile + (c * TH + yy) * TW + half * 20);
+#pragma unroll
+    for (int g = 0; g < 5; ++g) {
+        bf16_t e[4];
+#pragma unroll
+        for (int k4 = 0; k4 < 4; ++k4) {
+            const int k = g * 4 + k4, b = 3 + k;
+            float v = 0.f;
+            if (k >= klo && k < khi) v = ((float)((raw[b >> 2] >> ((b & 3) * 8)) & 0xffu) - mean) * inv;
+            e[k4] = f32_to_bf16(v);
+        }
+        dst[g] = make_uint2((uint32_t)e[0] | ((uint32_t)e[1] << 16), (uint32_t)e[2] | ((uint32_t)e[3] << 16));
+    }
+}
+
+__global__ __launch_bounds__(256, 2) void stem_pool_mfma_kernel(StemPoolDev q) {
+    const StemDev& p = q.s;
+    constexpr int TH = kStemPoolTH, TW = kStemPoolTW, WK = kStemWK, PT = kStemPoolPT, CS = 144;
+    constexpr int kTileBytes = (3 * TH * TW * 2 + 15) & ~15, kCtBytes = 256 * CS;
+    __shared__ __attribute__((aligned(16))) unsigned char smem[2 * kTileBytes + kCtBytes + 512];
+    unsigned char* ct = smem + 2 * kTileBytes;
+    float* bn = reinterpret_cast<float*>(smem + 2 * kTileBytes + kCtBytes);
+    if (threadIdx.x < 128) bn[threadIdx.x] = threadIdx.x < 64 ? p.scale[threadIdx.x] : p.shift[threadIdx.x - 64];
+    const int lane = threadIdx.x & 63, wave = __builtin_amdgcn_readfirstlane(threadIdx.x >> 6);
+    const int fr = lane & 15, fq = lane >> 4;
+    int t = blockIdx.x, step = gridDim.x, t_end = q.n_tiles;
+    if ((gridDim.x & 7) == 0) {
+        const int chunk = (q.n_tiles + 7) >> 3, xcd = blockIdx.x & 7;
+        t = xcd * chunk + (blockIdx.x >> 3); step = gridDim.x >> 3;
+        t_end = (xcd + 1) * chunk < q.n_tiles ? (xcd + 1) * chunk : q.n_tiles;
+    }
+    if (t >= t_end) return;
+    uint4 wf[6][4];
     {
-        const uint4* src = reinterpret_cast<const uint4*>(q.wpk);
-        uint4* dst = reinterpret_cast<uint4*>(wl);
-        for (int i = threadIdx.x; i < 64 * WK / 8; i += 256) dst[i] = src[i];
-    }
-    const int iy0 = cy0 * 2 - 3, ix0 = cx0 * 2 - 3;
-    const int h = p.h[n], w = p.wd[n];
-    {
-        const int r = threadIdx.x >> 1, half = threadIdx.x & 1;
-        if (r < 3 * TH) {
-            const int c = r / TH, yy = r - c * TH;
-            const int iy = iy0 + yy;
-            const bool rok = iy >= 0 && iy < h;
-            const uint8_t* row = p.img + (((long)n * 3 + c) * p.Hs + (rok ? iy : 0)) * p.Ws;
-            const float mean = p.mean[c], inv = p.inv_std[c];
-#pragma unroll
-            for (int k = 0; k < 20; ++k) {
-                const int xx = half * 20 + k, ix = ix0 + xx;
-                float v = 0.f;
-                if (rok && xx < TH && ix >= 0 && ix < w) v = ((float)row[ix] - mean) * inv;
-                tile[(c * TH + yy) * TW + xx] = f32_to_bf16(v);
+        const uint4* wpk16 = reinterpret_cast<const uint4*>(q.wpk);
+#pragma unroll
+        for (int s = 0; s < 6; ++s)
+#pragma unroll
+            for (int j = 0; j < 4; ++j) wf[s][j] = wpk16[((j * 16 + fr) * WK + (s * 4 + fq) * 8) >> 3];
+    }
+    StemTile cur = stem_tile(q, t);
+    const StemTile stride = stem_tile(q, step);
+    uint32_t raw[6];
+    stem_fetch(q, cur, threadIdx.x, raw);
+    stem_convert(q, cur, threadIdx.x, raw, reinterpret_cast<bf16_t*>(smem));
+    __syncthreads();
+    int buf = 0;
+    for (; t < t_end; t += step, buf ^= 1) {
+        const bool more = t + step < t_end;
+        int tid_l = threadIdx.x, fr_l = fr, fq_l = fq;
+        asm volatile("" : "+v"(tid_l), "+v"(fr_l), "+v"(fq_l));
+        StemTile nxt = cur;
+        if (more) {
+            nxt = stem_tile_advance(q, cur, stride);
+            stem_fetch(q, nxt, tid_l, raw);
+        }
+        const int n = cur.n, py0 = cur.ty * PT, px0 = cur.tx * PT;
+        const int cy0 = 2 * py0 - 1, cx0 = 2 * px0 - 1;
+        f32x4_t acc[4][4];
+#pragma unroll
+        for (int i = 0; i < 4; ++i)
+#pragma unroll
+            for (int j = 0; j < 4; ++j) acc[i][j] = f32x4_t{0.f, 0.f, 0.f, 0.f};
+        {
+            const uint32_t* tile32 = reinterpret_cast<const uint32_t*>(smem + buf * kTileBytes);
+            auto read_x = [&](int s, uint4 (&xf)[4]) {
+                int idx = s * 4 + fq_l;
+                idx = idx < 21 ? idx : 20;
+                const int c = idx / 7, kh = idx - c * 7;
+#pragma unroll
+                for (int i = 0; i < 4; ++i) {
+                    const int ty = wave * 4 + i;
+                    const int e = (c * TH + ty * 2 + kh) * (TW / 2) + fr_l;
+                    xf[i] = make_uint4(tile32[e], tile32[e + 1], tile32[e + 2], tile32[e + 3]);
+                }
+            };
+            uint4 xa[4], xb[4];
+            read_x(0, xa);
+#pragma unroll
+            for (int s = 0; s < 6; ++s) {
+                uint4 (&xf)[4] = (s & 1) ? xb : xa;
+                if (s + 1 < 6) read_x(s + 1, (s & 1) ? xa : xb);
+#pragma unroll
+                for (int i = 0; i < 4; ++i)
+#pragma unroll
+                    for (int j = 0; j < 4; ++j)
+                        acc[i][j] = __builtin_amdgcn_mfma_f32_16x16x32_bf16(*reinterpret_cast<bf16x8_t*>(&wf[s][j]), *reinterpret_cast<bf16x8_t*>(&xf[i]),
+                                                                             acc[i][j], 0, 0, 0);
+                __builtin_amdgcn_sched_barrier(0);
             }
         }
-    }
-    __syncthreads();
-    const int lane = threadIdx.x & 63, wave = threadIdx.x >> 6;
-    const int fr = lane & 15, fq = lane >> 4;
-    f32x4_t acc[4][4];
-#pragma unroll
-    for (int i = 0; i < 4; ++i)
-#pragma unroll
-        for (int j = 0; j < 4; ++j) acc[i][j] = f32x4_t{0.f, 0.f, 0.f, 0.f};
-    {
-        const uint32_t* tile32 = reinterpret_cast<const uint32_t*>(tile);
-        const uint4* wl16 = reinterpret_cast<const uint4*>(wl);
-#pragma unroll
-        for (int s = 0; s < 6; ++s) {
-            int idx = s * 4 + fq;
-            idx = idx < 21 ? idx : 20;
-            const int c = idx / 7, kh = idx - c * 7;
-            uint4 xf[4], wf[4];
+#pragma unroll
+        for (int j = 0; j < 4; ++j) {
+            const int ch = j * 16 + fq_l * 4;
+            const float4 sc = *reinterpret_cast<const float4*>(bn + ch), sh = *reinterpret_cast<const float4*>(bn + 64 + ch);
 #pragma unroll
             for (int i = 0; i < 4; ++i) {
-                const int ty = wave * 4 + i;
-                const int e = ((c * TH + ty * 2 + kh) * TW + fr * 2) >> 1;
-                xf[i] = make_uint4(tile32[e], tile32[e + 1], tile32[e + 2], tile32[e + 3]);
+                const int ry = wave * 4 + i, cy = cy0 + ry, cx = cx0 + fr_l;
+                uint2 o;
+                if (cy >= 0 && cy < p.Hc && cx >= 0 && cx < p.Wc) {
+                    o.x = pack2_bf16(fmaxf(acc[i][j][0] * sc.x + sh.x, 0.f), fmaxf(acc[i][j][1] * sc.y + sh.y, 0.f));
+                    o.y = pack2_bf16(fmaxf(acc[i][j][2] * sc.z + sh.z, 0.f), fmaxf(acc[i][j][3] * sc.w + sh.w, 0.f));
+                } else {
+                    o.x = o.y = 0xff80ff80u;
+                }
+                *reinterpret_cast<uint2*>(ct + (ry * 16 + fr_l) * CS + ch * 2) = o;
             }
-#pragma unroll
-            for (int j = 0; j < 4; ++j) wf[j] = wl16[((j * 16 + fr) * WK + (s * 4 + fq) * 8) >> 3];
-#pragma unroll
-            for (int i = 0; i < 4; ++i)
-#pragma unroll
-                for (int j = 0; j < 4; ++j)
-                    acc[i][j] = __builtin_amdgcn_mfma_f32_16x16x32_bf16(*reinterpret_cast<bf16x8_t*>(&wf[j]), *reinterpret_cast<bf16x8_t*>(&xf[i]),
-                                                                         acc[i][j], 0, 0, 0);
-        }
-    }
-    __syncthreads();
-#pragma unroll
-    for (int j = 0; j < 4; ++j) {
-        const int ch = j * 16 + fq * 4;
-        const float4 sc = *reinterpret_cast<const float4*>(p.scale + ch), sh = *reinterpret_cast<const float4*>(p.shift + ch);
-#pragma unroll
-        for (int i = 0; i < 4; ++i) {
-            const int ry = wave * 4 + i, cy = cy0 + ry, cx = cx0 + fr;
-            uint2 o;
-            if (cy >= 0 && cy < p.Hc && cx >= 0 && cx < p.Wc) {
-                o.x = pack2_bf16(fmaxf(acc[i][j][0] * sc.x + sh.x, 0.f), fmaxf(acc[i][j][1] * sc.y + sh.y, 0.f));
-                o.y = pack2_bf16(fmaxf(acc[i][j][2] * sc.z + sh.z, 0.f), fmaxf(acc[i][j][3] * sc.w + sh.w, 0.f));
-            } else {
-                o.x = o.y = 0xff80ff80u;
+        }
+        if (more) stem_convert(q, nxt, tid_l, raw, reinterpret_cast<bf16_t*>(smem + (buf ^ 1) * kTileBytes));
+        __syncthreads();
+        typedef short s16x8_t __attribute__((ext_vector_type(8)));
+        for (int item = tid_l; item < PT * PT * 8; item += 256) {
+            const int chunk = item & 7, pp = item >> 3;
+            const int pi = pp / PT, pj = pp - pi * PT;
+            const int py = py0 + pi, px = px0 + pj;
+            if (py >= q.Hp || px >= q.Wp) continue;
+            s16x8_t m = *reinterpret_cast<const s16x8_t*>(ct + ((2 * pi) * 16 + 2 * pj) * CS + chunk * 16);
+#pragma unroll
+            for (int d = 1; d < 9; ++d) {
+                const s16x8_t v = *reinterpret_cast<const s16x8_t*>(ct + ((2 * pi + d / 3) * 16 + 2 * pj + d % 3) * CS + chunk * 16);
+                m = __builtin_elementwise_max(m, v);
             }
-            *reinterpret_cast<uint2*>(smem + (ry * 16 + fr) * CS + ch * 2) = o;
-        }
-    }
-    __syncthreads();
-    typedef short s16x8_t __attribute__((ext_vector_type(8)));
-    for (int item = threadIdx.x; item < PT * PT * 8; item += 256) {
-        const int chunk = item & 7, pp = item >> 3;
-        const int pi = pp / PT, pj = pp - pi * PT;
-        const int py = py0 + pi, px = px0 + pj;
-        if (py >= q.Hp || px >= q.Wp) continue;
-        s16x8_t m = *reinterpret_cast<const s16x8_t*>(smem + ((2 * pi) * 16 + 2 * pj) * CS + chunk * 16);
-#pragma unroll
-        for (int d = 1; d < 9; ++d) {
-            const s16x8_t v = *reinterpret_cast<const s16x8_t*>(smem + ((2 * pi + d / 3) * 16 + 2 * pj + d % 3) * CS + chunk * 16);
-            m = __builtin_elementwise_max(m, v);
-        }
-        *reinterpret_cast<s16x8_t*>(q.yp + (((long)n * q.Hp + py) * q.Wp + px) * 64 + chunk * 8) = m;
+            *reinterpret_cast<s16x8_t*>(q.yp + (((long)n * q.Hp + py) * q.Wp + px) * 64 + chunk * 8) = m;
+        }
+        __syncthreads();
+        cur = nxt;
     }
 }
 
@@ -620,9 +694,20 @@
     for (int c = 0; c < 3; ++c) { d.mean[c] = a->mean[c]; d.inv_std[c] = 1.0f / a->std[c]; }
     q.wpk = static_cast<const bf16_t*>(w_packed);
     q.yp = static_cast<bf16_t*>(y_pool);
+    if ((a->Ws & 3) || (reinterpret_cast<uintptr_t>(a->img) & 3))
+        return aldi_set_error_msg(ALDI_ERR_ARG, "stem_pool_forward: the staging rows must be 4-byte aligned (Ws % 4 == 0)");
     q.Hp = (a->Hc - 1) / 2 + 1; q.Wp = (a->Wc - 1) / 2 + 1;
-    dim3 grid(cdiv(q.Wp, 7), cdiv(q.Hp, 7), a->N);
-    hipLaunchKernelGGL(stem_pool_mfma_kernel, grid, dim3(256), 0, static_cast<hipStream_t>(stream), q);
+    q.tiles_x = cdiv(q.Wp, kStemPoolPT); q.tiles_y = cdiv(q.Hp, kStemPoolPT); q.n_tiles = q.tiles_x * q.tiles_y * a->N;
+    static int n_cu = 0;
+    if (!n_cu) {
+        int dev = 0, v = 0;
+        if (hipGetDevice(&dev) != hipSuccess || hipDeviceGetAttribute(&v, hipDeviceAttributeMultiprocessorCount, dev) != hipSuccess || v < 1)
+            return aldi_set_error_msg(ALDI_ERR_HIP, "stem_pool_forward: cannot read the compute-unit count");
+        n_cu = v;
+    }
+    int wgs = aldi_tuning().stem_pool_wgs > 0 ? aldi_tuning().stem_pool_wgs : 2 * n_cu;
+    if (wgs > q.n_tiles) wgs = q.n_tiles;
+    hipLaunchKernelGGL(stem_pool_mfma_kernel, dim3(wgs), dim3(256), 0, static_cast<hipStream_t>(stream), q);
     ALDI_CHECK_LAUNCH();
     return ALDI_OK;
 }
diff --git a/aldi_amd/csrc/host.h b/aldi_amd/csrc/host.h
--- a/aldi_amd/csrc/host.h
+++ b/aldi_amd/csrc/host.h
@@ -15,7 +15,7 @@
     X(wgrad_big_group_min, 64) X(wgrad_lds_pad_kb, 0) X(wgrad_f32_tile128, 1) X(wgrad_dma64, 3) X(wgrad_ilv, 0) \
     X(msda_gather, 7) X(msda_gather_list, 1500) X(msda_bin, 1) X(msda_bin_list, 512) X(roialign_sep, 1) X(roialign_bwd_rows, 2) \
     X(colsum_blocks, 256) X(colsum_minrows, 16) X(colsum_nt, 1024) X(colsum_block_kb, 384) \
-    X(stem_mfma, 1) X(sab_blocks, 512) X(ln_bwd_blocks, 512) X(ln_bwd_blocks_narrow, 1024) X(rpn_topk_fused, 1) X(ema_blocks, 2048) X(nms_mask_tri, 1) X(match_wave, 1)
+    X(stem_mfma, 1) X(stem_pool_wgs, 0) X(sab_blocks, 512) X(ln_bwd_blocks, 512) X(ln_bwd_blocks_narrow, 1024) X(rpn_topk_fused, 1) X(ema_blocks, 2048) X(nms_mask_tri, 1) X(match_wave, 1)
 
 struct AldiTuning {
 #define ALDI_KNOB_FIELD(name, dflt) int name;
diff --git a/aldi_amd/engine.py b/aldi_amd/engine.py
--- a/aldi_amd/engine.py
+++ b/aldi_amd/engine.py
@@ -368,6 +368,7 @@
         self.mask_bits_inner = os.environ.get("ALDI_MASK_BITS_INNER", "1") == "1"
         self.level_groups = os.environ.get("ALDI_LEVEL_GROUPS", "1") == "1"
         self.fused_res2 = os.environ.get("ALDI_FUSED_RES2", "1") == "1"
+        self.fused_res2_shortcut = os.environ.get("ALDI_FUSED_RES2_SHORTCUT", "1") == "1"
         self._wg_queue: list = []
         self.sparse_rpn_backward = os.environ.get("ALDI_RPN_SPARSE_BWD", "1") == "1"
         spec = getattr(weights.layout, "img_da", None)
@@ -552,11 +553,14 @@
                 continue
             for b in range(nb):
                 p = f"{bu}res{si + 2}.{b}."
+                if si == 0 and fuse2:
+                    fold_sc = b == 0 and self.fused_res2_shortcut
+                    sc = (yield x, p + "shortcut", {}) if b == 0 and not fold_sc else x
+                    x = ops.bottleneck_fused(x, sc, fw[p + "conv1"], fw[p + "conv2"], fw[p + "conv3"], W.shift(p + "conv1"), W.shift(p + "conv2"),
+                                             W.shift(p + "conv3"), out=prefix_out if (prefix_out is not None and b == nb - 1) else None,
+                                             shortcut=(W.w(p + "shortcut"), W.scale(p + "shortcut"), W.shift(p + "shortcut")) if fold_sc else None)
+                    continue
                 sc = (yield x, p + "shortcut", {}) if b == 0 else x
-                if si == 0 and fuse2:
-                    x = ops.bottleneck_fused(x, sc, fw[p + "conv1"], fw[p + "conv2"], fw[p + "conv3"], W.shift(p + "conv1"), W.shift(p + "conv2"),
-                                             W.shift(p + "conv3"), out=prefix_out if (prefix_out is not None and b == nb - 1) else None)
-                    continue
                 want_bits = save and si > 0 and self.mask_bits and self.dtype == torch.bfloat16
 
                 def bits_for(inp, name):
diff --git a/aldi_amd/ops.py b/aldi_amd/ops.py
--- a/aldi_amd/ops.py
+++ b/aldi_amd/ops.py
@@ -259,13 +259,22 @@
         L.call("aldi_fold_weights_batch", _p(self.items), self.n, self.total_chunks, stream_ptr())
 
 
-def bottleneck_fused(x: torch.Tensor, res: torch.Tensor, w1, w2, w3, b1, b2, b3, out: Optional[torch.Tensor] = None) -> torch.Tensor:
+def bottleneck_fused(x: torch.Tensor, res: torch.Tensor, w1, w2, w3, b1, b2, b3, out: Optional[torch.Tensor] = None, *,
+                     shortcut=None) -> torch.Tensor:
     N, H, W_, Cin = x.shape
     mid, Cout = w1.shape[0], w3.shape[0]
-    assert x.dtype == torch.bfloat16 and x.is_contiguous() and res.is_contiguous() and res.shape == (N, H, W_, Cout), (x.shape, res.shape)
+    assert x.dtype == torch.bfloat16 and x.is_contiguous()
     assert w1.numel() == mid * Cin and w2.numel() == mid * 9 * mid and w3.numel() == Cout * mid and w1.dtype == torch.bfloat16
     if out is None:
         out = torch.empty((N, H, W_, Cout), dtype=x.dtype, device=x.device)
+    if shortcut is not None:
+        wsc, ssc, bsc = shortcut
+        assert wsc.dtype == torch.bfloat16 and wsc.is_contiguous() and wsc.numel() == Cout * Cin, wsc.shape
+        assert ssc.dtype == bsc.dtype == torch.float32 and ssc.numel() == bsc.numel() == Cout
+        a = L.BottleneckArgs(_p(x), None, _p(out), _p(w1), _p(w2), _p(w3), _p(b1), _p(b2), _p(b3), N, H, W_, Cin, mid, Cout)
+        L.call("aldi_bottleneck_fused_sc", C.byref(a), _p(wsc), _p(ssc), _p(bsc), stream_ptr())
+        return out
+    assert res.is_contiguous() and res.shape == (N, H, W_, Cout), (x.shape, res.shape)
     a = L.BottleneckArgs(_p(x), _p(res), _p(out), _p(w1), _p(w2), _p(w3), _p(b1), _p(b2), _p(b3), N, H, W_, Cin, mid, Cout)
     L.call("aldi_bottleneck_fused", C.byref(a), stream_ptr())
     return out
diff --git a/include/aldi_hip.h b/include/aldi_hip.h
--- a/include/aldi_hip.h
+++ b/include/aldi_hip.h
@@ -88,6 +88,7 @@
     int N, H, W, Cin, mid, Cout;
 } aldi_bottleneck_args;
 int aldi_bottleneck_fused(const aldi_bottleneck_args* a, aldi_stream_t stream);
+int aldi_bottleneck_fused_sc(const aldi_bottleneck_args* a, const void* wsc, const float* sc_scale, const float* sc_shift, aldi_stream_t stream);
 typedef struct aldi_fold_item {
     const float* w; const float* scale; void* out;
     int rows, cols, chunk_begin, reserved;
```

After: 511.1 (median of 6 runs). 1.02x the previous value.
